# debbiemarkslab/BEAR

Measured on AMD Instinct MI355X. Metric: k-mer contexts/sec (DM-marginal+grad h), k=13, higher is better.
Workload: dtype f64

## Files before the change

### bear_amd/csrc/bear_common.h

```cpp
#pragma once
#include <hip/hip_runtime.h>
#include <math.h>
#include <stdint.h>
#include <string.h>

#include "../../include/bear_hip.h"
#include "bear_release_guard.h"
#include "bear_math.h"

#define BEAR_THREADS 256
#define BEAR_TILE_ROWS 1024
#define BEAR_ROWS_PER_THREAD (BEAR_TILE_ROWS / BEAR_THREADS)
#define BEAR_MAX_OUT 4

extern __attribute__((visibility("hidden"))) thread_local int g_last_hip_error;

#define HIP_TRY(expr)                      \
  do {                                     \
    hipError_t _e = (expr);                \
    if (_e != hipSuccess) {                \
      g_last_hip_error = (int)_e;          \
      return BEAR_ERR_HIP;                 \
    }                                      \
  } while (0)

struct bear_params;
struct bear_ws {
  int device;
  int num_cu;
  int max_blocks;
  double *partials;
  double *logtab;
  unsigned long long *dbg;
  double *eval_partials;
  double *eval_out;
  int eval_blocks;
  double *lin_partials;
  double *lin_accum;
  unsigned long long *arrive;
  unsigned epoch;
  double *cnn_partials;
  size_t cnn_partials_cap;
};

struct bear_params {
  double inv_h;
  double eps;
  double E;
  double tauE;
  double tau;
  double V;
  double nw;
};

__device__ __forceinline__ void bear_store_agent(double *p, double v) {
  __hip_atomic_store(p, v, __ATOMIC_RELAXED, __HIP_MEMORY_SCOPE_AGENT);
}

__device__ __forceinline__ void bear_wave_store_rows5(double *R, const double (&f)[5], double *__restrict__ dst, uint64_t i0,
                                                      uint32_t valid, uint32_t lane) {
#pragma unroll
  for (int b = 0; b < 5; ++b) R[lane * 5u + b] = f[b];
  __builtin_amdgcn_fence(__ATOMIC_RELEASE, "wavefront");
  __builtin_amdgcn_wave_barrier();
  const uint32_t n16 = (valid * 5u) >> 1;
  typedef double bear_v2d __attribute__((ext_vector_type(2)));
  bear_v2d *out = reinterpret_cast<bear_v2d *>(dst + i0 * 5u);
  const bear_v2d *src = reinterpret_cast<const bear_v2d *>(R);
  for (uint32_t k = lane; k < n16; k += 64u) __builtin_nontemporal_store(src[k], out + k);
  if ((valid & 1u) && lane == 0) dst[(i0 + valid) * 5u - 1u] = R[valid * 5u - 1u];
  __builtin_amdgcn_fence(__ATOMIC_ACQUIRE, "wavefront");
  __builtin_amdgcn_wave_barrier();
}

__device__ __forceinline__ void bear_wave_load_rows5(double *R, const double *__restrict__ src, uint64_t i0, uint32_t valid,
                                                     uint32_t lane, double (&f)[5]) {
  typedef double bear_v2d __attribute__((ext_vector_type(2)));
  const uint32_t n16 = (valid * 5u) >> 1;
  const bear_v2d *in = reinterpret_cast<const bear_v2d *>(src + i0 * 5u);
  bear_v2d *dst = reinterpret_cast<bear_v2d *>(R);
  for (uint32_t k = lane; k < n16; k += 64u) dst[k] = __builtin_nontemporal_load(in + k);
  if ((valid & 1u) && lane == 0) R[valid * 5u - 1u] = src[(i0 + valid) * 5u - 1u];
  __builtin_amdgcn_fence(__ATOMIC_RELEASE, "wavefront");
  __builtin_amdgcn_wave_barrier();
  const uint32_t row = lane < valid ? lane : valid - 1u;
#pragma unroll
  for (int b = 0; b < 5; ++b) f[b] = R[row * 5u + b];
  __builtin_amdgcn_fence(__ATOMIC_ACQUIRE, "wavefront");
  __builtin_amdgcn_wave_barrier();
}

template <int NOUT, bool AGENT = false>
__device__ __forceinline__ void block_store_partials(double (&acc)[NOUT], double *partials) {
  __shared__ double red[16][BEAR_MAX_OUT];
  const int lane = threadIdx.x & 63, wave = threadIdx.x >> 6;
#pragma unroll
  for (int k = 0; k < NOUT; ++k) {
    double v = bear_wave_sum(acc[k]);
    if (lane == 0) red[wave][k] = v;
  }
  __syncthreads();
  if (threadIdx.x < NOUT) {
    double s = 0.0;
#pragma unroll
    for (int w = 0; w < (int)(blockDim.x >> 6); ++w) s += red[w][threadIdx.x];
    if (AGENT) bear_store_agent(&partials[(size_t)blockIdx.x * BEAR_MAX_OUT + threadIdx.x], s);
    else partials[(size_t)blockIdx.x * BEAR_MAX_OUT + threadIdx.x] = s;
  }
}

#define BEAR_THETA_NET 1
#define BEAR_THETA_REF 2
struct bear_arrival {
  unsigned long long *word;
  unsigned epoch;
};
struct bear_step_io {
  const double *theta;
  int kind;
  unsigned epoch;
  double *out;
  unsigned long long *arrive_word;
  __host__ __device__ bear_arrival arrive() const { return bear_arrival{arrive_word, epoch}; }
};
static_assert(sizeof(bear_step_io) == 32, "bear_step_io: kernel-argument size");

__device__ __forceinline__ double bear_uniform_f64(double v) {
  const unsigned long long b = (unsigned long long)__double_as_longlong(v);
  const unsigned lo = (unsigned)__builtin_amdgcn_readfirstlane((int)(unsigned)b);
  const unsigned hi = (unsigned)__builtin_amdgcn_readfirstlane((int)(unsigned)(b >> 32));
  return __longlong_as_double((long long)(((unsigned long long)hi << 32) | lo));
}

__device__ __forceinline__ bear_params bear_params_of(const bear_params &arg, const bear_step_io &io) {
  if (!io.theta) return arg;
  bear_params p;
  p.eps = arg.eps;
  p.inv_h = bear_uniform_f64(1.0 / exp(io.theta[0]));
  p.E = p.tauE = p.tau = p.V = p.nw = 0.0;
  if (io.kind == BEAR_THETA_REF) {
    const double tau = exp(io.theta[1]), nw = exp(io.theta[2]);
    const double E = exp(-tau);
    p.E = bear_uniform_f64(E);
    p.tauE = bear_uniform_f64(tau * E);
    p.tau = bear_uniform_f64(tau);
    p.V = bear_uniform_f64(1.0 / (nw + 1.0));
    p.nw = bear_uniform_f64(nw);
  }
  return p;
}

#define BEAR_ARRIVE_SUBS 16
#define BEAR_ARRIVE_STRIDE 16
#define BEAR_ARRIVE_WORDS ((BEAR_ARRIVE_SUBS + 1) * BEAR_ARRIVE_STRIDE)
__device__ __forceinline__ bool bear_arrive_count(unsigned long long *word, unsigned long long tag, unsigned expected) {
  __hip_atomic_fetch_max(word, tag, __ATOMIC_RELAXED, __HIP_MEMORY_SCOPE_AGENT);
  return __hip_atomic_fetch_add(word, 1ull, __ATOMIC_RELAXED, __HIP_MEMORY_SCOPE_AGENT) == tag + (expected - 1u);
}
__device__ __forceinline__ bool bear_arrive_last(const bear_arrival &arrive) {
  __shared__ unsigned s_last;
  asm volatile("s_waitcnt vmcnt(0)" ::: "memory");
  __syncthreads();
  if (threadIdx.x == 0) {
    const unsigned long long tag = (unsigned long long)arrive.epoch << 24;
    const unsigned sub = blockIdx.x % BEAR_ARRIVE_SUBS, grid = gridDim.x;
    const unsigned in_sub = (grid - sub + BEAR_ARRIVE_SUBS - 1u) / BEAR_ARRIVE_SUBS;
    const unsigned subs = grid < BEAR_ARRIVE_SUBS ? grid : BEAR_ARRIVE_SUBS;
    bool last = bear_arrive_count(arrive.word + (1u + sub) * BEAR_ARRIVE_STRIDE, tag, in_sub);
    if (last) last = bear_arrive_count(arrive.word, tag, subs);
    s_last = last ? 1u : 0u;
  }
  __syncthreads();
  if (!s_last) return false;
  __builtin_amdgcn_fence(__ATOMIC_ACQUIRE, "agent");
  return true;
}

__device__ __forceinline__ void bear_arrive_reset(const bear_arrival &arrive) {
#pragma unroll
  for (int k = 0; k <= BEAR_ARRIVE_SUBS; ++k)
    __hip_atomic_store(arrive.word + k * BEAR_ARRIVE_STRIDE, 0ull, __ATOMIC_RELAXED, __HIP_MEMORY_SCOPE_AGENT);
}

__device__ __forceinline__ void bear_finalize_in_block(const double *partials, int n_out, double *out, const bear_arrival &arrive, bool accumulate = false) {
  __shared__ double fred[4][BEAR_MAX_OUT];
  const int n_blocks = (int)gridDim.x;
  if (threadIdx.x < 256) {
    double acc[BEAR_MAX_OUT] = {0.0, 0.0, 0.0, 0.0};
    for (int b = threadIdx.x; b < n_blocks; b += 256)
#pragma unroll
      for (int k = 0; k < BEAR_MAX_OUT; ++k)
        if (k < n_out) acc[k] += partials[(size_t)b * BEAR_MAX_OUT + k];
    const int lane = threadIdx.x & 63, wave = threadIdx.x >> 6;
#pragma unroll
    for (int k = 0; k < BEAR_MAX_OUT; ++k) {
      double v = bear_wave_sum(acc[k]);
      if (lane == 0) fred[wave][k] = v;
    }
  }
  __syncthreads();
  if ((int)threadIdx.x < n_out) {
    const double v = (fred[0][threadIdx.x] + fred[1][threadIdx.x]) + (fred[2][threadIdx.x] + fred[3][threadIdx.x]);
    out[threadIdx.x] = accumulate ? out[threadIdx.x] + v : v;
  }
  if (threadIdx.x == 0) bear_arrive_reset(arrive);
}

struct bear_apply_io {
  double *theta;
  double *m, *v;
  double *t_state;
  double *loss_buf;
  unsigned long long loss_cap;
  double lr, scale;
  int n_theta, train_ar;
};

__device__ __forceinline__ void bear_adam_update(const bear_apply_io &A, const double *packed, int tid, int n_threads) {
  const double t0 = A.t_state[0], t = t0 + 1.0;
  const double b1 = 0.9, b2 = 0.999, aeps = 1e-7;
  const double lr_t = A.lr * sqrt(1.0 - pow(b2, t)) / (1.0 - pow(b1, t));
  for (int k = tid; k < A.n_theta; k += n_threads) {
    if (A.train_ar && k == 0) continue;
    const double g = A.scale * packed[1 + k];
    const double mk = b1 * A.m[k] + (1.0 - b1) * g, vk = b2 * A.v[k] + (1.0 - b2) * g * g;
    A.m[k] = mk;
    A.v[k] = vk;
    A.theta[k] -= lr_t * mk / (sqrt(vk) + aeps);
  }
  if (tid == 0) {
    const unsigned long long step = (unsigned long long)t0;
    if (A.loss_buf && step < A.loss_cap) A.loss_buf[step] = -A.scale * packed[0];
  }
  __syncthreads();
  if (tid == 0) A.t_state[0] = t;
}

__device__ __forceinline__ void bear_apply_in_block(const bear_apply_io &A, const double *packed) {
  if (!A.theta) return;
  __threadfence_block();
  __syncthreads();
  bear_adam_update(A, packed, (int)threadIdx.x, (int)blockDim.x);
}

template <int NOUT>
__device__ __forceinline__ void block_finish(double (&acc)[NOUT], double *partials, const bear_step_io &io) {
  if (!io.out) {
    block_store_partials<NOUT>(acc, partials);
    return;
  }
  block_store_partials<NOUT, true>(acc, partials);
  if (bear_arrive_last(io.arrive())) bear_finalize_in_block(partials, NOUT, io.out, io.arrive());
}
template <int NOUT>
__device__ __forceinline__ void block_finish(double (&acc)[NOUT], double *partials, const bear_step_io &io, const bear_apply_io &apply) {
  if (!io.out) {
    block_store_partials<NOUT>(acc, partials);
    return;
  }
  block_store_partials<NOUT, true>(acc, partials);
  if (bear_arrive_last(io.arrive())) {
    bear_finalize_in_block(partials, NOUT, io.out, io.arrive());
    bear_apply_in_block(apply, io.out);
  }
}
```

### bear_amd/csrc/bear_hip.hip

```cpp
#include "bear_host.h"
#include "kernels_finalize.h"
#include "kernels_rows.h"
#include "kernels_sorted.h"
#include "kernels_plan.h"
#include "kernels_synth.h"
#include "kernels_refmix.h"
#include "kernels_mixplan.h"
#include "kernels_sample.h"
#include "kernels_shuffle.h"
#include "kernels_refplan.h"

#ifdef PLN_STAMPS
#define PLN_DBG_ARG , ws->dbg
#else
#define PLN_DBG_ARG
#endif

thread_local int g_last_hip_error = 0;

extern "C" {

int bear_abi_version(void) { return BEAR_ABI_VERSION; }

const char *bear_strerror(int status) {
  switch (status) {
    case BEAR_OK: return "ok";
    case BEAR_ERR_INVALID_ARG: return "invalid argument (null or misaligned pointer, bad flag)";
    case BEAR_ERR_NO_DEVICE: return "no usable HIP device";
    case BEAR_ERR_WRONG_DEVICE: return "current HIP device differs from the workspace device";
    case BEAR_ERR_HIP: return "HIP runtime call failed (see bear_last_hip_error)";
    case BEAR_ERR_NOMEM: return "out of memory";
    case BEAR_ERR_IO: return "file could not be opened or read";
    case BEAR_ERR_PARSE: return "malformed count-table row";
    default: return "unknown bear status";
  }
}

int bear_last_hip_error(void) { return g_last_hip_error; }

static int dm_kernels_setup() {
  int st = allow_dynamic_lds({BEAR_KFN(dm_prior_sorted_kernel<0>), BEAR_KFN(dm_prior_sorted_kernel<1>), BEAR_KFN(dm_prior_sorted_kernel<9>)},
                             sizeof(srt_lds_n));
  if (st == BEAR_OK) st = allow_dynamic_lds({BEAR_KFN(dm_ref_sorted_kernel)}, sizeof(srt_lds_r));
  if (st == BEAR_OK)
    st = allow_dynamic_lds({BEAR_KFN(dm_prior_plan_kernel<false, false>), BEAR_KFN(dm_prior_plan_kernel<true, false>),
                            BEAR_KFN(dm_prior_plan_kernel<true, true>)},
                           sizeof(pln_lds_n));
  if (st == BEAR_OK)
    st = allow_dynamic_lds({BEAR_KFN(dm_prior_plan_grad_kernel<false, false>), BEAR_KFN(dm_prior_plan_grad_kernel<true, true>),
                            BEAR_KFN(dm_refmix_plan_grad_kernel<false>), BEAR_KFN(dm_refmix_plan_grad_kernel<true>)},
                           sizeof(pln_lds_g));
  if (st == BEAR_OK) st = allow_dynamic_lds({BEAR_KFN(dm_prior_plan_grad_inplace_kernel)}, sizeof(pln_lds_gi));
  if (st == BEAR_OK) st = allow_dynamic_lds({BEAR_KFN(dm_ref_plan_kernel<false>), BEAR_KFN(dm_ref_plan_kernel<true>)}, sizeof(pln_lds_r));
  return st;
}

static void ws_release(bear_ws *ws) {
  (void)hipFree(ws->partials);
  (void)hipFree(ws->logtab);
  (void)hipFree(ws->dbg);
  (void)hipFree(ws->eval_partials);
  (void)hipFree(ws->eval_out);
  (void)hipFree(ws->lin_partials);
  (void)hipFree(ws->lin_accum);
  (void)hipFree(ws->cnn_partials);
  (void)hipFree(ws->arrive);
  delete ws;
}

static int ws_setup(bear_ws *ws) {
  HIP_TRY(hipMalloc(&ws->partials, sizeof(double) * BEAR_MAX_OUT * (size_t)ws->max_blocks));
  HIP_TRY(hipMalloc(&ws->logtab, sizeof(double) * 2 * BEAR_LOGTAB_N));
  HIP_TRY(hipMalloc(&ws->dbg, sizeof(unsigned long long) * 48 * (size_t)ws->max_blocks));
  HIP_TRY(hipMalloc(&ws->arrive, sizeof(unsigned long long) * BEAR_ARRIVE_WORDS));
  HIP_TRY(hipMemset(ws->arrive, 0, sizeof(unsigned long long) * BEAR_ARRIVE_WORDS));
  double tab[2 * BEAR_LOGTAB_N];
  for (int i = 0; i < BEAR_LOGTAB_N; ++i) {
    const double r = 1.0 / ((BEAR_LOGTAB_N + i + 0.5) / (2.0 * BEAR_LOGTAB_N));
    tab[2 * i] = r;
    tab[2 * i + 1] = -log(r);
  }
  HIP_TRY(hipMemcpy(ws->logtab, tab, sizeof(tab), hipMemcpyHostToDevice));
  int st = dm_kernels_setup();
  if (st == BEAR_OK) st = linear_ws_setup(ws);
  if (st == BEAR_OK) st = cnn_ws_setup(ws);
  if (st == BEAR_OK) st = eval_ws_setup(ws);
  return st;
}

int bear_ws_create(int device, bear_ws **out) {
  if (!out) return BEAR_ERR_INVALID_ARG;
  *out = nullptr;
  int count = 0;
  if (hipGetDeviceCount(&count) != hipSuccess || count <= 0) return BEAR_ERR_NO_DEVICE;
  if (device < 0 || device >= count) return BEAR_ERR_INVALID_ARG;
  int prev = 0;
  HIP_TRY(hipGetDevice(&prev));
  HIP_TRY(hipSetDevice(device));
  hipDeviceProp_t prop;
  const hipError_t e = hipGetDeviceProperties(&prop, device);
  bear_ws *ws = e == hipSuccess ? new (std::nothrow) bear_ws() : nullptr;
  int st = ws ? BEAR_OK : BEAR_ERR_NOMEM;
  if (e != hipSuccess) {
    g_last_hip_error = (int)e;
    st = BEAR_ERR_HIP;
  }
  if (ws) {
    ws->device = device;
    ws->num_cu = prop.multiProcessorCount;
    ws->max_blocks = ws->num_cu * 8;
    ws->eval_blocks = ws->num_cu * 8;
    st = ws_setup(ws);
    if (st != BEAR_OK) {
      ws_release(ws);
      ws = nullptr;
    }
  }
  (void)hipSetDevice(prev);
  *out = ws;
  return st;
}

int bear_ws_destroy(bear_ws *ws) {
  if (!ws) return BEAR_OK;
  int prev = 0;
  (void)hipGetDevice(&prev);
  (void)hipSetDevice(ws->device);
  ws_release(ws);
  (void)hipSetDevice(prev);
  return BEAR_OK;
}

int bear_deterministic_build(void) {
#ifdef BEAR_DET_BUILD
  return 1;
#else
  return 0;
#endif
}

static int grid_rows(const bear_ws *ws, uint64_t n_rows) { return grid_capped((n_rows + BEAR_TILE_ROWS - 1) / BEAR_TILE_ROWS, ws_blocks(ws, 2)); }
static int grid_sorted(const bear_ws *ws, uint64_t n_rows) { return grid_capped((n_rows + SRT_TILE - 1) / SRT_TILE, ws_blocks(ws, 2)); }
static int grid_dense(const bear_ws *ws, uint64_t n_rows) {
  return grid_capped((n_rows + DPR_TILE_ROWS - 1) / DPR_TILE_ROWS, ws_blocks(ws, DPR_BLOCKS_PER_CU));
}

int bear_dm_prior_f64(bear_ws *ws, const uint32_t *counts, const double *prior, uint64_t n_rows,
                      double h_signed, double eps, int train_ar, double *out, double *grad_prior,
                      void *stream) {
  int st = check_ws(ws);
  if (st != BEAR_OK) return st;
  if (!out || (n_rows && (!counts || !prior))) return BEAR_ERR_INVALID_ARG;
  if (misaligned(counts) || misaligned(prior) || misaligned(grad_prior) || (reinterpret_cast<uintptr_t>(out) & 7u))
    return BEAR_ERR_INVALID_ARG;
  hipStream_t s = static_cast<hipStream_t>(stream);
  bear_params prm;
  memset(&prm, 0, sizeof(prm));
  prm.inv_h = 1.0 / exp(h_signed);
  prm.eps = eps;
  int grid = grid_rows(ws, n_rows);
  if (!train_ar && !grad_prior) {
    grid = grid_sorted(ws, n_rows);
    const char *dbg = getenv("BEAR_DEBUG_STOP");
    const int stop = dbg ? atoi(dbg) : 0;
    const double2 *lt = reinterpret_cast<const double2 *>(ws->logtab);
    if (stop == 1)
      hipLaunchKernelGGL(dm_prior_sorted_kernel<1>, dim3(grid), dim3(SRT_THREADS), sizeof(srt_lds_n), s, counts, prior, n_rows, prm, lt, ws->partials, ws->dbg);
    else if (stop == 9)
      hipLaunchKernelGGL(dm_prior_sorted_kernel<9>, dim3(grid), dim3(SRT_THREADS), sizeof(srt_lds_n), s, counts, prior, n_rows, prm, lt, ws->partials, ws->dbg);
    else
      hipLaunchKernelGGL(dm_prior_sorted_kernel<0>, dim3(grid), dim3(SRT_THREADS), sizeof(srt_lds_n), s, counts, prior, n_rows, prm, lt, ws->partials, ws->dbg);
  } else {
#define PRIOR_LAUNCH(AR, GRAD)                                                                                                          \
  hipLaunchKernelGGL((dm_prior_kernel<AR, GRAD>), dim3(grid), dim3(BEAR_THREADS), 0, s, counts, prior, n_rows, prm, grad_prior, \
                     reinterpret_cast<const double2 *>(ws->logtab), ws->partials)
    BEAR_DISPATCH_2(train_ar, grad_prior, PRIOR_LAUNCH);
#undef PRIOR_LAUNCH
  }
  HIP_TRY(hipGetLastError());
  hipLaunchKernelGGL(finalize_kernel, dim3(1), dim3(256), 0, s, ws->partials, grid, 2, out);
  HIP_TRY(hipGetLastError());
  return BEAR_OK;
}

int bear_dm_ref_f64(bear_ws *ws, const uint32_t *train, const uint32_t *ref, uint64_t n_rows,
                    double h_signed, double tau_signed, double nu_signed, double eps, int train_ar,
                    double *out, void *stream) {
  int st = check_ws(ws);
  if (st != BEAR_OK) return st;
  if (!out || (n_rows && (!train || !ref))) return BEAR_ERR_INVALID_ARG;
  if (misaligned(train) || misaligned(ref) || (reinterpret_cast<uintptr_t>(out) & 7u)) return BEAR_ERR_INVALID_ARG;
  hipStream_t s = static_cast<hipStream_t>(stream);
  bear_params prm;
  const double tau = exp(tau_signed), nw = exp(nu_signed);
  prm.inv_h = 1.0 / exp(h_signed);
  prm.eps = eps;
  prm.E = exp(-tau);
  prm.tauE = tau * prm.E;
  prm.tau = tau;
  prm.V = 1.0 / (nw + 1.0);
  prm.nw = nw;
  int grid = grid_rows(ws, n_rows);
  if (train_ar) {
    hipLaunchKernelGGL((dm_ref_kernel<true>), dim3(grid), dim3(BEAR_THREADS), 0, s, train, ref, n_rows, prm, reinterpret_cast<const double2 *>(ws->logtab), ws->partials);
  } else if (getenv("BEAR_ROWS_KERNEL")) {
    hipLaunchKernelGGL((dm_ref_kernel<false>), dim3(grid), dim3(BEAR_THREADS), 0, s, train, ref, n_rows, prm, reinterpret_cast<const double2 *>(ws->logtab), ws->partials);
  } else {
    grid = grid_sorted(ws, n_rows);
    hipLaunchKernelGGL(dm_ref_sorted_kernel, dim3(grid), dim3(SRT_THREADS), sizeof(srt_lds_r), s, train, ref, n_rows, prm,
                       reinterpret_cast<const double2 *>(ws->logtab), ws->partials);
  }
  HIP_TRY(hipGetLastError());
  hipLaunchKernelGGL(finalize_kernel, dim3(1), dim3(256), 0, s, ws->partials, grid, 4, out);
  HIP_TRY(hipGetLastError());
  return BEAR_OK;
}

static void plan_free(bear_plan *p) {
  if (!p) return;
  (void)hipFree(p->tiles);
  (void)hipFree(p->stream);
  (void)hipFree(p->heavy_col);
  (void)hipFree(p->heavy_row);
  (void)hipFree(p->heavy_stop);
  (void)hipFree(p->hist);
  (void)hipFree(p->live);
  for (int k = 0; k < p->n_cnn_levels; ++k) bear_level_free(&p->cnn_levels[k]);
  for (int k = 0; k <= CNN_MAX_LAG; ++k)
    for (int q = 0; q < p->n_cnn_win[k]; ++q) bear_window_free(&p->cnn_win[k][q]);
  (void)hipFree(p->live2);
  (void)hipFree(p->tiles_p);
  (void)hipFree(p->tiles_u);
  (void)hipFree(p->ref_items);
  (void)hipFree(p->hist0_base);
  (void)hipFree(p->heavy0);
  (void)hipFree(p->sum0);
  delete p;
}

int bear_plan_create(bear_ws *ws, const uint32_t *counts, uint64_t n_rows, int ncol, bear_plan **out) {
  if (!out) return BEAR_ERR_INVALID_ARG;
  *out = nullptr;
  int st = check_ws(ws);
  if (st != BEAR_OK) return st;
  if ((ncol != 4 && ncol != 5) || (n_rows && !counts) || misaligned(counts)) return BEAR_ERR_INVALID_ARG;
  bear_plan *p = new (std::nothrow) bear_plan();
  if (!p) return BEAR_ERR_NOMEM;
  memset(p, 0, sizeof(*p));
  p->device = ws->device;
  p->ncol = ncol;
  p->n_rows = n_rows;
  p->counts = counts;
  hipError_t e = hipMalloc(&p->hist, sizeof(unsigned long long) * (2 * SRT_NKEY + PLN_NBIG + 1));
  if (e == hipSuccess) e = hipMemset(p->hist, 0, sizeof(unsigned long long) * (2 * SRT_NKEY + PLN_NBIG + 1));
  if (e != hipSuccess) {
    g_last_hip_error = (int)e;
    plan_free(p);
    return BEAR_ERR_HIP;
  }
  if (n_rows == 0) {
    *out = p;
    return BEAR_OK;
  }
  const uint64_t n_quads = (n_rows + PLN_QUAD - 1) / PLN_QUAD;
  uint8_t *d_quad = nullptr, *h_quad = nullptr;
  unsigned long long *d_cnt = nullptr;
  std::vector<pln_tile> tiles;
  e = hipMalloc(&d_quad, 3 * n_quads);
  if (e == hipSuccess) e = hipMalloc(&d_cnt, sizeof(unsigned long long) * 9);
  if (e == hipSuccess) e = hipMemset(d_cnt, 0, sizeof(unsigned long long) * 9);
  if (e == hipSuccess) {
    const int grid = grid_capped((n_quads + 255) / 256, (uint64_t)ws->num_cu * 8);
    hipLaunchKernelGGL(plan_scan_kernel, dim3(grid), dim3(256), 0, 0, counts, n_rows, ncol, d_quad, d_cnt, p->hist);
    e = hipGetLastError();
  }
  unsigned long long h_cnt[3] = {0, 0, 0}, h_total[3] = {0, 0, 0};
  if (e == hipSuccess) e = hipMemcpy(h_cnt, d_cnt, sizeof(h_cnt), hipMemcpyDeviceToHost);
  if (e == hipSuccess) e = hipMemcpy(h_total, d_cnt + 6, sizeof(h_total), hipMemcpyDeviceToHost);
  for (int k = 0; k < 3; ++k) p->count_total[k] = p->count_bound[k] = (double)h_total[k];
  uint64_t off16 = 0, n_tiles = 0;
  const char *cut_env = getenv("BEAR_PLAN_CUT");
  const bool host_cut = cut_env && cut_env[0] == 'h';
  if (e == hipSuccess && host_cut) {
    h_quad = (uint8_t *)malloc(3 * n_quads);
    if (!h_quad) e = hipErrorOutOfMemory;
    if (e == hipSuccess) e = hipMemcpy(h_quad, d_quad, 3 * n_quads, hipMemcpyDeviceToHost);
  }
  if (e == hipSuccess && host_cut) {
    uint64_t q = 0;
    while (q < n_quads) {
      uint32_t items = 0, rows = 0, hcol = 0, hrow = 0;
      const uint64_t q0 = q;
      while (q < n_quads && rows + PLN_QUAD <= PLN_RMAX && items + h_quad[q] <= PLN_NI_CUT) {
        items += h_quad[q];
        hcol += h_quad[n_quads + q];
        hrow += h_quad[2 * n_quads + q];
        rows += PLN_QUAD;
        ++q;
      }
      pln_tile ti;
      memset(&ti, 0, sizeof(ti));
      ti.row0 = q0 * PLN_QUAD;
      if (ti.row0 + rows > n_rows) rows = (uint32_t)(n_rows - ti.row0);
      const uint32_t hc = hcol < PLN_HCAP ? hcol : PLN_HCAP;
      const uint32_t hr = ncol == 5 ? (hrow < PLN_HCAP ? hrow : PLN_HCAP) : 0u;
      ti.rows_items = (rows << 16) | items;
      ti.off16 = (uint32_t)off16;
      ti.hc_hr = (hc << 16) | hr;
      ti.blk16 = pln_block_layout(rows, items, hc, hr).end / 16;
      off16 += ti.blk16;
      if (off16 > 0xffffffffull) {
        e = hipErrorOutOfMemory;
        break;
      }
      tiles.push_back(ti);
    }
    n_tiles = tiles.size();
  }
  free(h_quad);
  if (e == hipSuccess && !host_cut) {
    const uint32_t chunk = plan_cut_chunk(n_quads);
    const uint64_t n_chunks = (n_quads + chunk - 1) / chunk;
    uint32_t *d_walk = nullptr;
    uint16_t *d_step = nullptr;
    uint64_t *d_entry = nullptr;
    unsigned long long *d_meta = nullptr, h_meta[3] = {0, 0, 0};
    e = hipMalloc(&d_walk, sizeof(uint32_t) * n_chunks * PLN_CUT_SPAN);
    if (e == hipSuccess) e = hipMalloc(&d_step, sizeof(uint16_t) * n_quads);
    if (e == hipSuccess) e = hipMalloc(&d_entry, sizeof(uint64_t) * 2 * n_chunks);
    if (e == hipSuccess) e = hipMalloc(&d_meta, sizeof(h_meta));
    if (e == hipSuccess) e = hipMemset(d_meta, 0, sizeof(h_meta));
    if (e == hipSuccess) {
      const uint64_t wb = (n_chunks * PLN_CUT_SPAN + 255) / 256;
      hipLaunchKernelGGL(plan_cut_step_kernel, dim3((unsigned)((n_chunks + 255) / 256)), dim3(256), 0, 0, d_quad, n_quads, n_chunks, chunk, d_step);
      hipLaunchKernelGGL(plan_cut_walk_kernel, dim3((unsigned)wb), dim3(256), 0, 0, d_step, n_quads, n_chunks, chunk, d_walk);
      hipLaunchKernelGGL(plan_cut_chain_kernel, dim3(1), dim3(1), 0, 0, d_walk, n_chunks, chunk, d_entry, d_entry + n_chunks, d_meta);
      e = hipGetLastError();
    }
    if (e == hipSuccess) e = hipMemcpy(h_meta, d_meta, sizeof(unsigned long long), hipMemcpyDeviceToHost);
    n_tiles = h_meta[0];
    if (e == hipSuccess) e = hipMalloc(&p->tiles, sizeof(pln_tile) * (n_tiles + PLN_DESC_PAD));
    if (e == hipSuccess) e = hipMemset(p->tiles, 0, sizeof(pln_tile) * (n_tiles + PLN_DESC_PAD));
    if (e == hipSuccess) {
      hipLaunchKernelGGL(plan_cut_write_kernel, dim3((unsigned)((n_chunks + 255) / 256)), dim3(256), 0, 0, d_quad, n_quads, n_rows, ncol,
                         n_chunks, chunk, d_entry, d_entry + n_chunks, p->tiles);
      hipLaunchKernelGGL(plan_cut_offsets_kernel, dim3(1), dim3(1024), 0, 0, p->tiles, n_tiles, d_meta);
      e = hipGetLastError();
    }
    if (e == hipSuccess) e = hipMemcpy(h_meta, d_meta, sizeof(h_meta), hipMemcpyDeviceToHost);
    if (e == hipSuccess && h_meta[2]) e = hipErrorOutOfMemory;
    off16 = h_meta[1];
    (void)hipFree(d_walk);
    (void)hipFree(d_step);
    (void)hipFree(d_entry);
    (void)hipFree(d_meta);
  }
  (void)hipFree(d_quad);
  p->n_tiles = n_tiles;
  const uint64_t stream_bytes = off16 * 16 + 1024;
  for (int k = 0; k < 3; ++k) p->n_heavy[k] = h_cnt[k];
  if (host_cut) {
    if (e == hipSuccess) e = hipMalloc(&p->tiles, sizeof(pln_tile) * (tiles.size() + PLN_DESC_PAD));
    if (e == hipSuccess) e = hipMemset(p->tiles, 0, sizeof(pln_tile) * (tiles.size() + PLN_DESC_PAD));
    if (e == hipSuccess) e = hipMemcpy(p->tiles, tiles.data(), sizeof(pln_tile) * tiles.size(), hipMemcpyHostToDevice);
  }
  if (e == hipSuccess) e = hipMalloc(&p->stream, stream_bytes);
  if (e == hipSuccess) e = hipMemset(p->stream, 0, stream_bytes);
  if (e == hipSuccess && h_cnt[0]) e = hipMalloc(&p->heavy_col, sizeof(pln_heavy_col) * h_cnt[0]);
  if (e == hipSuccess && h_cnt[1]) e = hipMalloc(&p->heavy_row, sizeof(pln_heavy_row) * h_cnt[1]);
  if (e == hipSuccess && h_cnt[2]) e = hipMalloc(&p->heavy_stop, sizeof(uint64_t) * h_cnt[2]);
  if (e == hipSuccess) {
    const uint64_t nt = n_tiles;
    const int grid = grid_capped(nt, (uint64_t)ws->num_cu * 2);
    hipLaunchKernelGGL(plan_fill_kernel, dim3(grid), dim3(1024), 0, 0, counts, n_rows, ncol, p->tiles, nt, p->stream,
                       p->heavy_col, p->heavy_row, p->heavy_stop, d_cnt + 3);
    e = hipGetLastError();
  }
  const uint64_t live_bytes = ncol == 5 ? sizeof(uint16_t) * PLN_LIVE_STRIDE * (n_tiles + 1) : 0;
  if (e == hipSuccess && live_bytes) e = hipMalloc(&p->live, live_bytes);
  if (e == hipSuccess && live_bytes) e = hipMemset(p->live, 0, live_bytes);
  if (e == hipSuccess && live_bytes) {
    const uint64_t nt = n_tiles;
    const int grid = grid_capped(nt, (uint64_t)ws->num_cu * 2);
    hipLaunchKernelGGL(plan_live_kernel, dim3(grid), dim3(1024), 0, 0, p->tiles, nt, p->stream, p->live);
    e = hipGetLastError();
  }
  if (e == hipSuccess) e = hipDeviceSynchronize();
  unsigned long long h_used[3] = {0, 0, 0};
  if (e == hipSuccess) e = hipMemcpy(h_used, d_cnt + 3, sizeof(h_used), hipMemcpyDeviceToHost);
  for (int k = 0; k < 3; ++k) p->n_heavy[k] = h_used[k];
#ifdef BEAR_DET_BUILD
  const uint64_t sort_from = 2;
#else
  const uint64_t sort_from = 1u << 16;
#endif
  if (e == hipSuccess) {
    int cst = h_used[0] >= sort_from ? bear_canonical_order(p->heavy_col, h_used[0], 16, 0) : BEAR_OK;
    if (cst == BEAR_OK && h_used[1] >= sort_from) cst = bear_canonical_order(p->heavy_row, h_used[1], 16, 0);
    if (cst == BEAR_OK && h_used[2] >= sort_from) cst = bear_canonical_order(p->heavy_stop, h_used[2], 8, 0);
    if (cst != BEAR_OK) e = cst == BEAR_ERR_NOMEM ? hipErrorOutOfMemory : hipErrorUnknown;
  }
  p->n_live_rows = n_rows;
  if (e == hipSuccess && ncol == 5) {
    unsigned long long h_hist[SRT_NKEY];
    e = hipMemcpy(h_hist, p->hist, sizeof(h_hist), hipMemcpyDeviceToHost);
    unsigned long long live_rows = h_cnt[1];
    for (int k = 0; k < SRT_NKEY; ++k) live_rows += h_hist[k];
    p->n_live_rows = live_rows;
  }
  (void)hipFree(d_cnt);
  if (e != hipSuccess) {
    g_last_hip_error = (int)e;
    plan_free(p);
    return e == hipErrorOutOfMemory ? BEAR_ERR_NOMEM : BEAR_ERR_HIP;
  }
  p->bytes = stream_bytes + live_bytes + sizeof(pln_tile) * n_tiles + sizeof(pln_heavy_col) * h_cnt[0] +
             sizeof(pln_heavy_row) * h_cnt[1] + sizeof(uint64_t) * h_cnt[2];
  *out = p;
  return BEAR_OK;
}

int bear_plan_destroy(bear_plan *plan) {
  if (!plan) return BEAR_OK;
  int prev = 0;
  (void)hipGetDevice(&prev);
  (void)hipSetDevice(plan->device);
  plan_free(plan);
  (void)hipSetDevice(prev);
  return BEAR_OK;
}

uint64_t bear_plan_bytes(const bear_plan *plan) { return plan ? plan->bytes : 0; }

#define PLAN_ROWS 15
static bool plan_is_rows(const bear_plan *p) { return p->ncol == PLAN_ROWS; }
int bear_plan_create_auto(bear_ws *ws, const uint32_t *counts, uint64_t n_rows, int *rowwise, bear_plan **out) {
  if (rowwise) *rowwise = 0;
  int st = bear_plan_create(ws, counts, n_rows, 5, out);
  if (st != BEAR_OK) return st;
  bear_plan *p = *out;
  const double cells = p->count_total[1], listed = (double)p->n_heavy[0];
  if (!(cells > 0.0) || listed * 2.0 <= cells) return BEAR_OK;
  (void)hipFree(p->tiles);
  (void)hipFree(p->stream);
  (void)hipFree(p->heavy_col);
  (void)hipFree(p->heavy_row);
  (void)hipFree(p->heavy_stop);
  (void)hipFree(p->live);
  p->tiles = nullptr;
  p->stream = nullptr;
  p->heavy_col = nullptr;
  p->heavy_row = nullptr;
  p->heavy_stop = nullptr;
  p->live = nullptr;
  p->n_tiles = 0;
  p->n_heavy[0] = p->n_heavy[1] = p->n_heavy[2] = 0;
  p->ncol = PLAN_ROWS;
  p->bytes = sizeof(unsigned long long) * (2 * SRT_NKEY + PLN_NBIG + 1);
  if (rowwise) *rowwise = 1;
  return BEAR_OK;
}
static int launch_prior_rows(bear_ws *ws, const bear_plan *plan, const double *prior, const bear_params &prm, const double *theta,
                             int train_ar, double *out, double *grad_prior, hipStream_t s) {
  const int grid = grid_dense(ws, plan->n_rows);
  const double2 *lt = reinterpret_cast<const double2 *>(ws->logtab);
  const bear_step_io io = ws_io(ws, theta, BEAR_THETA_NET, out);
#define ROWS_LAUNCH(AR, GRAD) \
  hipLaunchKernelGGL((dm_prior_rows_kernel<AR, GRAD>), dim3(grid), dim3(BEAR_THREADS), 0, s, plan->counts, prior, plan->n_rows, prm, grad_prior, lt, \
                     ws->partials, io)
  BEAR_DISPATCH_2(train_ar, grad_prior, ROWS_LAUNCH);
#undef ROWS_LAUNCH
  HIP_TRY(hipGetLastError());
  return BEAR_OK;
}

uint64_t bear_plan_tile_count(const bear_plan *plan) { return plan ? plan->n_tiles : 0; }

int bear_plan_tile_info(const bear_plan *plan, uint64_t first, uint64_t count, uint64_t *row0, uint32_t *rows, uint32_t *items,
                        uint64_t *stream_offset) {
  if (!plan || first + count > plan->n_tiles || (count && (!row0 || !rows || !items || !stream_offset))) return BEAR_ERR_INVALID_ARG;
  if (!count) return BEAR_OK;
  std::vector<pln_tile> h(count);
  int prev = 0;
  (void)hipGetDevice(&prev);
  (void)hipSetDevice(plan->device);
  const hipError_t e = hipMemcpy(h.data(), plan->tiles + first, sizeof(pln_tile) * count, hipMemcpyDeviceToHost);
  (void)hipSetDevice(prev);
  if (e != hipSuccess) {
    g_last_hip_error = (int)e;
    return BEAR_ERR_HIP;
  }
  for (uint64_t k = 0; k < count; ++k) {
    row0[k] = h[k].row0;
    rows[k] = h[k].rows_items >> 16;
    items[k] = h[k].rows_items & 0xffffu;
    stream_offset[k] = (uint64_t)h[k].off16 * 16;
  }
  return BEAR_OK;
}

int bear_plan_create_ref(bear_ws *ws, const uint32_t *train, const uint32_t *ref, uint64_t n_rows, bear_plan **out) {
  if (!out) return BEAR_ERR_INVALID_ARG;
  *out = nullptr;
  if ((n_rows && !ref) || misaligned(ref)) return BEAR_ERR_INVALID_ARG;
  bear_plan *p = nullptr;
  int st = bear_plan_create(ws, train, n_rows, 4, &p);
  if (st != BEAR_OK) return st;
  p->ref = ref;
  if (p->count_total[1] > 0.0 && (double)p->n_heavy[0] * 2.0 > p->count_total[1]) {
    (void)hipFree(p->tiles);
    (void)hipFree(p->stream);
    (void)hipFree(p->heavy_col);
    (void)hipFree(p->heavy_row);
    (void)hipFree(p->heavy_stop);
    p->tiles = nullptr;
    p->stream = nullptr;
    p->heavy_col = nullptr;
    p->heavy_row = nullptr;
    p->heavy_stop = nullptr;
    p->n_tiles = 0;
    p->n_heavy[0] = p->n_heavy[1] = p->n_heavy[2] = 0;
    p->rows_ref = 1;
    p->bytes = sizeof(unsigned long long) * (2 * SRT_NKEY + PLN_NBIG + 1);
    *out = p;
    return BEAR_OK;
  }
  unsigned long long *d_meta = nullptr;
  hipError_t e = hipMalloc(&d_meta, sizeof(unsigned long long) * 72);
  if (e == hipSuccess) e = hipMemset(d_meta, 0, sizeof(unsigned long long) * 72);
  if (e == hipSuccess) e = hipMalloc(&p->sum0, sizeof(double));
  if (e == hipSuccess) e = hipMemset(p->sum0, 0, sizeof(double));
  p->hist0_base = d_meta;
  unsigned long long h_meta[72];
  memset(h_meta, 0, sizeof(h_meta));
  const int grid = grid_capped((n_rows + 1023) / 1024, (uint64_t)ws->num_cu * 8);
  if (e == hipSuccess && n_rows) {
    hipLaunchKernelGGL(rpl_build_kernel, dim3(grid), dim3(256), 0, 0, train, ref, n_rows, 0, d_meta, d_meta + 32, d_meta + 64, p->sum0,
                       static_cast<rpl_item *>(nullptr), static_cast<uint32_t *>(nullptr));
    e = hipGetLastError();
    if (e == hipSuccess) e = hipMemcpy(h_meta, d_meta, sizeof(h_meta), hipMemcpyDeviceToHost);
  }
  if (e == hipSuccess) {
    unsigned long long run = 0, cur[RPL_NKEY];
    for (int k = 0; k < RPL_NKEY; ++k) {
      cur[k] = run;
      run += h_meta[k];
    }
    p->n_ref_items = run;
    p->n_heavy0 = h_meta[64];
    if (run) e = hipMalloc(&p->ref_items, sizeof(rpl_item) * run);
    if (e == hipSuccess && p->n_heavy0) e = hipMalloc(&p->heavy0, sizeof(uint32_t) * p->n_heavy0);
    if (e == hipSuccess) e = hipMemcpy(d_meta, cur, sizeof(cur), hipMemcpyHostToDevice);
    if (e == hipSuccess) e = hipMemset(d_meta + 64, 0, sizeof(unsigned long long));
    if (e == hipSuccess && n_rows && (run || p->n_heavy0)) {
      hipLaunchKernelGGL(rpl_build_kernel, dim3(grid), dim3(256), 0, 0, train, ref, n_rows, 1, d_meta, d_meta + 32, d_meta + 64, p->sum0,
                         p->ref_items, p->heavy0);
      e = hipGetLastError();
    }
    if (e == hipSuccess) e = hipDeviceSynchronize();
#ifdef BEAR_DET_BUILD
    for (int k = 0; k < RPL_NKEY && e == hipSuccess; ++k)
      if (bear_canonical_order(p->ref_items + cur[k], h_meta[k], 16, 0) != BEAR_OK) e = hipErrorUnknown;
    if (e == hipSuccess && bear_canonical_order(p->heavy0, p->n_heavy0, 4, 0) != BEAR_OK) e = hipErrorUnknown;
#endif
  }
  if (e != hipSuccess) {
    g_last_hip_error = (int)e;
    plan_free(p);
    return e == hipErrorOutOfMemory ? BEAR_ERR_NOMEM : BEAR_ERR_HIP;
  }
  p->hist0 = d_meta + 32;
  p->bytes += sizeof(rpl_item) * p->n_ref_items + sizeof(uint32_t) * p->n_heavy0 + sizeof(unsigned long long) * 72;
  *out = p;
  return BEAR_OK;
}

static int launch_prior_plan(bear_ws *ws, const bear_plan *plan, const double *prior, uint64_t n_rows, const bear_params &prm,
                             const double *theta, int train_ar, int prior_normalized, double *out, hipStream_t s) {
  const int grid = grid_plan(ws, plan->n_tiles);
  const double2 *lt = reinterpret_cast<const double2 *>(ws->logtab);
  const bear_step_io io = ws_io(ws, theta, BEAR_THETA_NET, out);
  if (train_ar)
    hipLaunchKernelGGL((dm_prior_plan_kernel<true, true>), dim3(grid), dim3(PLN_THREADS), sizeof(pln_lds_n), s, prior, n_rows, prm,
                       plan_view(plan), lt, ws->partials, io PLN_DBG_ARG);
  else if (prior_normalized)
    hipLaunchKernelGGL((dm_prior_plan_kernel<true, false>), dim3(grid), dim3(PLN_THREADS), sizeof(pln_lds_n), s, prior, n_rows, prm,
                       plan_view(plan), lt, ws->partials, io PLN_DBG_ARG);
  else
    hipLaunchKernelGGL((dm_prior_plan_kernel<false, false>), dim3(grid), dim3(PLN_THREADS), sizeof(pln_lds_n), s, prior, n_rows, prm,
                       plan_view(plan), lt, ws->partials, io PLN_DBG_ARG);
  HIP_TRY(hipGetLastError());
  return BEAR_OK;
}

int bear_dm_prior_plan_f64(bear_ws *ws, const bear_plan *plan, const uint32_t *counts, const double *prior,
                           uint64_t n_rows, double h_signed, double eps, int train_ar, int prior_normalized,
                           double *out, void *stream) {
  int st = check_ws(ws);
  if (st != BEAR_OK) return st;
  if (!plan || !out || (n_rows && (!counts || !prior))) return BEAR_ERR_INVALID_ARG;
  if ((plan->ncol != 5 && !plan_is_rows(plan)) || plan->n_rows != n_rows || plan->counts != counts || plan->device != ws->device)
    return BEAR_ERR_INVALID_ARG;
  if (misaligned(prior) || (reinterpret_cast<uintptr_t>(out) & 7u)) return BEAR_ERR_INVALID_ARG;
  bear_params prm;
  memset(&prm, 0, sizeof(prm));
  prm.inv_h = 1.0 / exp(h_signed);
  prm.eps = eps;
  if (plan_is_rows(plan)) return launch_prior_rows(ws, plan, prior, prm, nullptr, train_ar, out, nullptr, static_cast<hipStream_t>(stream));
  return launch_prior_plan(ws, plan, prior, n_rows, prm, nullptr, train_ar, prior_normalized, out, static_cast<hipStream_t>(stream));
}

int launch_prior_plan_grad(bear_ws *ws, const bear_plan *plan, const double *prior, const bear_params &prm,
                                  const double *theta, int train_ar, int prior_normalized, double *out, double *grad_prior,
                                  hipStream_t s) {
  const int grid = grid_plan(ws, plan->n_tiles);
  const double2 *lt = reinterpret_cast<const double2 *>(ws->logtab);
  const pln_view pv = plan_view(plan);
  const bear_step_io io = ws_io(ws, theta, BEAR_THETA_NET, out);
  if (train_ar)
    hipLaunchKernelGGL((dm_prior_plan_grad_kernel<true, true>), dim3(grid), dim3(PLN_THREADS), sizeof(pln_lds_g), s, prior, prm, pv, lt,
                       grad_prior, ws->partials, io);
  else if (prior_normalized)
    hipLaunchKernelGGL(dm_prior_plan_grad_inplace_kernel, dim3(grid), dim3(PLN_THREADS), sizeof(pln_lds_gi), s, prior, prm, pv, lt,
                       grad_prior, ws->partials, io);
  else
    hipLaunchKernelGGL((dm_prior_plan_grad_kernel<false, false>), dim3(grid), dim3(PLN_THREADS), sizeof(pln_lds_g), s, prior, prm, pv, lt,
                       grad_prior, ws->partials, io);
  HIP_TRY(hipGetLastError());
  auto fixup_grid = [&](uint64_t nh) { return grid_capped((nh + 255) / 256, (uint64_t)ws->num_cu * 8); };
#define FIXUP(NORM, AR, ROWS, N) \
  hipLaunchKernelGGL((dm_prior_grad_fixup_kernel<NORM, AR, ROWS>), dim3(fixup_grid(N)), dim3(256), 0, s, prior, prm, pv, lt, grad_prior, io)
  if (pv.n_heavy_row && !train_ar) {
    if (prior_normalized) FIXUP(true, false, true, pv.n_heavy_row);
    else FIXUP(false, false, true, pv.n_heavy_row);
  }
  if (pv.n_heavy_col) {
    if (train_ar) FIXUP(true, true, false, pv.n_heavy_col);
    else if (prior_normalized) FIXUP(true, false, false, pv.n_heavy_col);
    else FIXUP(false, false, false, pv.n_heavy_col);
  }
#undef FIXUP
  HIP_TRY(hipGetLastError());
  return BEAR_OK;
}

int bear_dm_prior_plan_grad_f64(bear_ws *ws, const bear_plan *plan, const uint32_t *counts, const double *prior,
                                uint64_t n_rows, double h_signed, double eps, int train_ar, int prior_normalized,
                                double *out, double *grad_prior, void *stream) {
  int st = check_ws(ws);
  if (st != BEAR_OK) return st;
  if (!plan || !out || !grad_prior || (n_rows && (!counts || !prior))) return BEAR_ERR_INVALID_ARG;
  if ((plan->ncol != 5 && !plan_is_rows(plan)) || plan->n_rows != n_rows || plan->counts != counts || plan->device != ws->device)
    return BEAR_ERR_INVALID_ARG;
  if (misaligned(prior) || misaligned(grad_prior) || (reinterpret_cast<uintptr_t>(out) & 7u)) return BEAR_ERR_INVALID_ARG;
  bear_params prm;
  memset(&prm, 0, sizeof(prm));
  prm.inv_h = 1.0 / exp(h_signed);
  prm.eps = eps;
  if (plan_is_rows(plan)) return launch_prior_rows(ws, plan, prior, prm, nullptr, train_ar, out, grad_prior, static_cast<hipStream_t>(stream));
  return launch_prior_plan_grad(ws, plan, prior, prm, nullptr, train_ar, prior_normalized, out, grad_prior,
                                static_cast<hipStream_t>(stream));
}

int bear_dm_prior_plan_dev_f64(bear_ws *ws, const bear_plan *plan, const uint32_t *counts, const double *prior, uint64_t n_rows,
                               const double *h_signed_dev, double eps, int train_ar, int prior_normalized, double *out,
                               double *grad_prior, void *stream) {
  int st = check_ws(ws);
  if (st != BEAR_OK) return st;
  if (!plan || !out || !h_signed_dev || (n_rows && (!counts || !prior))) return BEAR_ERR_INVALID_ARG;
  if ((plan->ncol != 5 && !plan_is_rows(plan)) || plan->n_rows != n_rows || plan->counts != counts || plan->device != ws->device)
    return BEAR_ERR_INVALID_ARG;
  if (misaligned(prior) || misaligned(grad_prior) || (reinterpret_cast<uintptr_t>(out) & 7u)) return BEAR_ERR_INVALID_ARG;
  hipStream_t s = static_cast<hipStream_t>(stream);
  bear_params only_eps;
  memset(&only_eps, 0, sizeof(only_eps));
  only_eps.eps = eps;
  if (plan_is_rows(plan)) return launch_prior_rows(ws, plan, prior, only_eps, h_signed_dev, train_ar, out, grad_prior, s);
  if (grad_prior) return launch_prior_plan_grad(ws, plan, prior, only_eps, h_signed_dev, train_ar, prior_normalized, out, grad_prior, s);
  return launch_prior_plan(ws, plan, prior, n_rows, only_eps, h_signed_dev, train_ar, prior_normalized, out, s);
}

int bear_dm_refmix_plan_grad_f64(bear_ws *ws, const bear_plan *plan, const uint32_t *counts, const double *net_rows,
                                 const double *ref_rows, uint64_t n_rows, const double *h_signed_dev, const double *tau_signed_dev,
                                 const double *net_weight_signed_dev, double eps, int train_ar, double *out, double *grad_net_rows,
                                 void *stream) {
  int st = check_ws(ws);
  if (st != BEAR_OK) return st;
  if (!plan || !out || !h_signed_dev || !tau_signed_dev || !net_weight_signed_dev) return BEAR_ERR_INVALID_ARG;
  if (n_rows && (!counts || !net_rows || !ref_rows || !grad_net_rows)) return BEAR_ERR_INVALID_ARG;
  if (plan->ncol != 5 || plan->n_rows != n_rows || plan->counts != counts || plan->device != ws->device) return BEAR_ERR_INVALID_ARG;
  if (misaligned(net_rows) || misaligned(ref_rows) || misaligned(grad_net_rows) || misaligned8(out) || misaligned8(h_signed_dev) ||
      misaligned8(tau_signed_dev) || misaligned8(net_weight_signed_dev) || !(eps >= 0.0))
    return BEAR_ERR_INVALID_ARG;
  hipStream_t s = static_cast<hipStream_t>(stream);
  const int grid = grid_plan(ws, plan->n_tiles);
  const double2 *lt = reinterpret_cast<const double2 *>(ws->logtab);
  const pln_view pv = plan_view(plan);
  const bear_step_io io = ws_io(ws, nullptr, BEAR_THETA_REF, out);
  if (train_ar)
    hipLaunchKernelGGL(dm_refmix_plan_grad_kernel<true>, dim3(grid), dim3(PLN_THREADS), sizeof(pln_lds_g), s, net_rows, ref_rows,
                       h_signed_dev, tau_signed_dev, net_weight_signed_dev, eps, pv, lt, grad_net_rows, ws->partials, io);
  else
    hipLaunchKernelGGL(dm_refmix_plan_grad_kernel<false>, dim3(grid), dim3(PLN_THREADS), sizeof(pln_lds_g), s, net_rows, ref_rows,
                       h_signed_dev, tau_signed_dev, net_weight_signed_dev, eps, pv, lt, grad_net_rows, ws->partials, io);
  HIP_TRY(hipGetLastError());
  if (pv.n_heavy_col + pv.n_heavy_row) {
    const uint64_t nh = pv.n_heavy_col + pv.n_heavy_row;
    const int g2 = grid_capped((nh + 255) / 256, (uint64_t)ws->num_cu * 4);
    if (train_ar)
      hipLaunchKernelGGL(dm_refmix_fixup_kernel<true>, dim3(g2), dim3(256), 0, s, net_rows, ref_rows, h_signed_dev, tau_signed_dev,
                         net_weight_signed_dev, eps, pv, lt, grad_net_rows);
    else
      hipLaunchKernelGGL(dm_refmix_fixup_kernel<false>, dim3(g2), dim3(256), 0, s, net_rows, ref_rows, h_signed_dev, tau_signed_dev,
                         net_weight_signed_dev, eps, pv, lt, grad_net_rows);
    HIP_TRY(hipGetLastError());
  }
  return BEAR_OK;
}


static int launch_ref_plan(bear_ws *ws, const bear_plan *plan, const uint32_t *ref, uint64_t n_rows, const bear_params &prm,
                           const double *theta, int train_ar, double *out, hipStream_t s, const bear_apply_io &apply = NO_APPLY) {
  const double2 *lt = reinterpret_cast<const double2 *>(ws->logtab);
  const bear_step_io io = ws_io(ws, theta, BEAR_THETA_REF, out);
  int grid;
  if (plan->rows_ref) {
    if (plan->ref != ref) return BEAR_ERR_INVALID_ARG;
    grid = grid_dense(ws, n_rows);
    if (train_ar)
      hipLaunchKernelGGL(dm_ref_rows_kernel<true>, dim3(grid), dim3(BEAR_THREADS), 0, s, plan->counts, ref, n_rows, prm, lt, ws->partials, io, apply);
    else
      hipLaunchKernelGGL(dm_ref_rows_kernel<false>, dim3(grid), dim3(BEAR_THREADS), 0, s, plan->counts, ref, n_rows, prm, lt, ws->partials, io, apply);
  } else if (plan->ref) {
    if (plan->ref != ref) return BEAR_ERR_INVALID_ARG;
    rpl_view rv;
    rv.items = plan->ref_items;
    rv.n_items = plan->n_ref_items;
    rv.hist0 = plan->hist0;
    rv.heavy0 = plan->heavy0;
    rv.n_heavy0 = plan->n_heavy0;
    rv.sum0 = plan->sum0;
    const uint64_t units = (plan->n_ref_items + 63) / 64, want = (units + 3) / 4 + 2, cap = (uint64_t)ws->num_cu * (units > 131072 ? 6 : 4);
    grid = grid_capped(want, cap);
    if (train_ar)
      hipLaunchKernelGGL(dm_ref_items_kernel<true>, dim3(grid), dim3(256), 0, s, prm, rv, plan_view(plan), lt, ws->partials, io, apply);
    else
      hipLaunchKernelGGL(dm_ref_items_kernel<false>, dim3(grid), dim3(256), 0, s, prm, rv, plan_view(plan), lt, ws->partials, io, apply);
  } else {
    grid = grid_plan(ws, plan->n_tiles);
    if (train_ar)
      hipLaunchKernelGGL(dm_ref_plan_kernel<true>, dim3(grid), dim3(PLN_THREADS), sizeof(pln_lds_r), s, ref, n_rows, prm, plan_view(plan), lt,
                         ws->partials, io, apply);
    else
      hipLaunchKernelGGL(dm_ref_plan_kernel<false>, dim3(grid), dim3(PLN_THREADS), sizeof(pln_lds_r), s, ref, n_rows, prm, plan_view(plan), lt,
                         ws->partials, io, apply);
  }
  HIP_TRY(hipGetLastError());
  (void)grid;
  return BEAR_OK;
}

int bear_dm_ref_plan_f64(bear_ws *ws, const bear_plan *plan, const uint32_t *train, const uint32_t *ref,
                         uint64_t n_rows, double h_signed, double tau_signed, double nu_signed, double eps,
                         int train_ar, double *out, void *stream) {
  int st = check_ws(ws);
  if (st != BEAR_OK) return st;
  if (!plan || !out || (n_rows && (!train || !ref))) return BEAR_ERR_INVALID_ARG;
  if (plan->ncol != 4 || plan->n_rows != n_rows || plan->counts != train || plan->device != ws->device)
    return BEAR_ERR_INVALID_ARG;
  if (misaligned(ref) || (reinterpret_cast<uintptr_t>(out) & 7u)) return BEAR_ERR_INVALID_ARG;
  hipStream_t s = static_cast<hipStream_t>(stream);
  bear_params prm;
  const double tau = exp(tau_signed), nw = exp(nu_signed);
  prm.inv_h = 1.0 / exp(h_signed);
  prm.eps = eps;
  prm.E = exp(-tau);
  prm.tauE = tau * prm.E;
  prm.tau = tau;
  prm.V = 1.0 / (nw + 1.0);
  prm.nw = nw;
  return launch_ref_plan(ws, plan, ref, n_rows, prm, nullptr, train_ar, out, s);
}

int bear_ref_train_reduce_f64(bear_ws *ws, const bear_plan *plan, const uint32_t *train, const uint32_t *ref, uint64_t n_rows,
                              const double *theta, double eps, int train_ar, double *packed, void *stream) {
  int st = check_ws(ws);
  if (st != BEAR_OK) return st;
  if (!plan || !packed || !theta || !n_rows || !train || !ref) return BEAR_ERR_INVALID_ARG;
  if (plan->ncol != 4 || plan->n_rows != n_rows || plan->counts != train || plan->device != ws->device)
    return BEAR_ERR_INVALID_ARG;
  if (misaligned(ref) || (reinterpret_cast<uintptr_t>(packed) & 7u)) return BEAR_ERR_INVALID_ARG;
  hipStream_t s = static_cast<hipStream_t>(stream);
  bear_params only_eps;
  memset(&only_eps, 0, sizeof(only_eps));
  only_eps.eps = eps;
  return launch_ref_plan(ws, plan, ref, n_rows, only_eps, theta, train_ar, packed, s);
}

int bear_ref_train_step_f64(bear_ws *ws, const bear_plan *plan, const uint32_t *train, const uint32_t *ref, uint64_t n_rows,
                            double *theta, double *adam_m, double *adam_v, double *adam_t, double eps, int train_ar,
                            double learning_rate, double scale, double *out, double *loss_buf, uint64_t loss_cap, void *stream) {
  if (!adam_m || !adam_v || !adam_t) return BEAR_ERR_INVALID_ARG;
  if (two_launch_step()) {
    int st = bear_ref_train_reduce_f64(ws, plan, train, ref, n_rows, theta, eps, train_ar, out, stream);
    if (st != BEAR_OK) return st;
    return launch_train_apply(theta, 3, out, adam_m, adam_v, adam_t, learning_rate, scale, train_ar, loss_buf, loss_cap,
                              static_cast<hipStream_t>(stream));
  }
  int st = check_ws(ws);
  if (st != BEAR_OK) return st;
  if (!plan || !out || !theta || !n_rows || !train || !ref) return BEAR_ERR_INVALID_ARG;
  if (plan->ncol != 4 || plan->n_rows != n_rows || plan->counts != train || plan->device != ws->device) return BEAR_ERR_INVALID_ARG;
  if (misaligned(ref) || (reinterpret_cast<uintptr_t>(out) & 7u)) return BEAR_ERR_INVALID_ARG;
  bear_params only_eps;
  memset(&only_eps, 0, sizeof(only_eps));
  only_eps.eps = eps;
  return launch_ref_plan(ws, plan, ref, n_rows, only_eps, theta, train_ar, out, static_cast<hipStream_t>(stream),
                         make_apply(theta, 3, adam_m, adam_v, adam_t, learning_rate, scale, train_ar, loss_buf, loss_cap));
}

int bear_dm_items_f64(bear_ws *ws, const double *x, const uint32_t *c, uint64_t n, int path, double *D, double *P,
                      void *stream) {
  int st = check_ws(ws);
  if (st != BEAR_OK) return st;
  if (n == 0) return BEAR_OK;
  if (!x || !c || !D || !P || path < 0 || path > 2) return BEAR_ERR_INVALID_ARG;
  uint64_t blocks = (n + 255) / 256;
  if (blocks > 0x7fffffffull) return BEAR_ERR_INVALID_ARG;
  hipLaunchKernelGGL(dm_items_kernel, dim3((unsigned)blocks), dim3(256), 0, static_cast<hipStream_t>(stream), x, c, n, path,
                     reinterpret_cast<const double2 *>(ws->logtab), D, P);
  HIP_TRY(hipGetLastError());
  return BEAR_OK;
}

int bear_plan_count_total(const bear_plan *plan, double *total, double *bound) {
  if (!plan) return BEAR_ERR_INVALID_ARG;
  for (int k = 0; k < 3; ++k) {
    if (total) total[k] = plan->count_total[k];
    if (bound) bound[k] = plan->count_bound[k];
  }
  return BEAR_OK;
}

int bear_plan_set_count_bound(bear_plan *plan, const double *bound) {
  if (!plan || !bound) return BEAR_ERR_INVALID_ARG;
  for (int k = 0; k < 3; ++k)
    if (!(bound[k] >= plan->count_total[k]) || !(bound[k] < 0x1p50)) return BEAR_ERR_INVALID_ARG;
  for (int k = 0; k < 3; ++k) plan->count_bound[k] = bound[k];
  return BEAR_OK;
}

static int refmix_grid(const bear_ws *ws, uint64_t n_rows) { return grid_capped((n_rows + RMX_THREADS - 1) / RMX_THREADS, ws_blocks(ws, 2)); }

int bear_ref_mix_forward_f64(bear_ws *ws, const double *net_rows, const double *ref_rows, uint64_t n_rows, const double *tau_signed,
                             const double *net_weight_signed, double *prior, void *stream) {
  int st = check_ws(ws);
  if (st != BEAR_OK) return st;
  if (!tau_signed || !net_weight_signed || misaligned8(tau_signed) || misaligned8(net_weight_signed)) return BEAR_ERR_INVALID_ARG;
  if (n_rows == 0) return BEAR_OK;
  if (!net_rows || !ref_rows || !prior || misaligned(net_rows) || misaligned(ref_rows) || misaligned(prior)) return BEAR_ERR_INVALID_ARG;
  hipLaunchKernelGGL(ref_mix_forward_kernel, dim3(refmix_grid(ws, n_rows)), dim3(RMX_THREADS), 0, static_cast<hipStream_t>(stream),
                     net_rows, ref_rows, tau_signed, net_weight_signed, n_rows, prior);
  HIP_TRY(hipGetLastError());
  return BEAR_OK;
}

int bear_ref_mix_backward_f64(bear_ws *ws, const double *net_rows, const double *ref_rows, const double *grad_prior, uint64_t n_rows,
                              const double *tau_signed, const double *net_weight_signed, double *grad_net_rows, double *grad_scalars,
                              void *stream) {
  int st = check_ws(ws);
  if (st != BEAR_OK) return st;
  if (!tau_signed || !net_weight_signed || !grad_scalars || misaligned8(tau_signed) || misaligned8(net_weight_signed) ||
      misaligned8(grad_scalars))
    return BEAR_ERR_INVALID_ARG;
  hipStream_t s = static_cast<hipStream_t>(stream);
  if (n_rows == 0) {
    HIP_TRY(hipMemsetAsync(grad_scalars, 0, 2 * sizeof(double), s));
    return BEAR_OK;
  }
  if (!net_rows || !ref_rows || !grad_prior || !grad_net_rows || misaligned(net_rows) || misaligned(ref_rows) ||
      misaligned(grad_prior) || misaligned(grad_net_rows))
    return BEAR_ERR_INVALID_ARG;
  hipLaunchKernelGGL(ref_mix_backward_kernel, dim3(refmix_grid(ws, n_rows)), dim3(RMX_THREADS), 0, s, net_rows, ref_rows, grad_prior,
                     tau_signed, net_weight_signed, n_rows, grad_net_rows, ws->partials, ws_arrival(ws), grad_scalars);
  HIP_TRY(hipGetLastError());
  return BEAR_OK;
}

int bear_debug_read_timing(bear_ws *ws, unsigned long long *host, int n_words) {
  if (!ws || !host) return BEAR_ERR_INVALID_ARG;
  HIP_TRY(hipDeviceSynchronize());
  HIP_TRY(hipMemcpy(host, ws->dbg, sizeof(unsigned long long) * (size_t)n_words, hipMemcpyDeviceToHost));
  return BEAR_OK;
}

int bear_debug_occupancy(int which) {
  int nb = -1;
  hipError_t e = which == 0
      ? hipOccupancyMaxActiveBlocksPerMultiprocessor(&nb, dm_prior_sorted_kernel<0>, SRT_THREADS, sizeof(srt_lds_n))
      : hipOccupancyMaxActiveBlocksPerMultiprocessor(&nb, dm_ref_sorted_kernel, SRT_THREADS, sizeof(srt_lds_r));
  return e == hipSuccess ? nb : -1000 - (int)e;
}

int bear_log_gamma_f64(const double *conc, uint64_t n, uint64_t n_samples, uint64_t seed, double *out, void *stream) {
  if (n == 0 || n_samples == 0) return BEAR_OK;
  if (!conc || !out) return BEAR_ERR_INVALID_ARG;
  if (n_samples > (~0ull) / n) return BEAR_ERR_INVALID_ARG;
  const uint64_t total = n * n_samples;
  uint64_t blocks = (total + SMP_THREADS - 1) / SMP_THREADS;
  if (blocks > 65536) blocks = 65536;
  hipLaunchKernelGGL(log_gamma_kernel, dim3((unsigned)blocks), dim3(SMP_THREADS), 0, static_cast<hipStream_t>(stream), conc, n,
                     n_samples, seed, out);
  HIP_TRY(hipGetLastError());
  return BEAR_OK;
}

static int logdir_sample_launch(const uint32_t *counts, const double *prior, uint64_t n_rows, int width, const double *h,
                                int n_h, int with_ar, const double *van, int n_van, int mc_samples, int map, uint64_t seed,
                                uint64_t row_base, double *out, void *stream) {
  if (n_h < 0 || n_van < 0 || n_h + n_van > SMP_MAX_MODELS || (n_h && !h) || (n_van && !van)) return BEAR_ERR_INVALID_ARG;
  if (with_ar && !map) return BEAR_ERR_INVALID_ARG;
  if (map) mc_samples = 1;
  if (mc_samples <= 0) return BEAR_ERR_INVALID_ARG;
  const int M = (with_ar ? 1 : 0) + n_h + n_van;
  if (n_rows == 0 || M == 0) return BEAR_OK;
  if (!out || ((n_h || with_ar) && !prior)) return BEAR_ERR_INVALID_ARG;
  smp_args A;
  memset(&A, 0, sizeof(A));
  A.n_h = n_h;
  A.n_van = n_van;
  A.arm = with_ar ? 1 : 0;
  A.has_counts = counts ? 1 : 0;
  A.has_prior = prior ? 1 : 0;
  A.map = map ? 1 : 0;
  A.mc = (uint32_t)mc_samples;
  A.seed = seed;
  A.row_base = row_base;
  for (int j = 0; j < n_h; ++j) {
    if (!(h[j] > 0.0)) return BEAR_ERR_INVALID_ARG;
    A.w[j] = 1.0 / h[j];
  }
  for (int k = 0; k < n_van; ++k) A.w[n_h + k] = van[k];
  const uint64_t per_row = (uint64_t)M * (uint64_t)mc_samples;
  if (per_row > 0xffffffffull || n_rows > (~0ull) / ((uint64_t)width * per_row)) return BEAR_ERR_INVALID_ARG;
  uint64_t blocks = (n_rows * per_row + SMP_THREADS - 1) / SMP_THREADS;
  if (blocks > 65536) blocks = 65536;
  hipStream_t s = static_cast<hipStream_t>(stream);
  if (width == 21)
    hipLaunchKernelGGL(logdir_sample_kernel<21>, dim3((unsigned)blocks), dim3(SMP_THREADS), 0, s, counts, prior, n_rows, A, out);
  else
    hipLaunchKernelGGL(logdir_sample_kernel<5>, dim3((unsigned)blocks), dim3(SMP_THREADS), 0, s, counts, prior, n_rows, A, out);
  HIP_TRY(hipGetLastError());
  return BEAR_OK;
}

int bear_logdir_sample_f64(const uint32_t *counts, const double *prior, uint64_t n_rows, const double *h, int n_h,
                           int with_ar, const double *van, int n_van, int mc_samples, int map, uint64_t seed,
                           uint64_t row_base, double *out, void *stream) {
  return logdir_sample_launch(counts, prior, n_rows, 5, h, n_h, with_ar, van, n_van, mc_samples, map, seed, row_base, out, stream);
}

int bear_logdir_sample_wide_f64(const uint32_t *counts, const double *prior, uint64_t n_rows, int width, const double *h,
                                int n_h, int with_ar, const double *van, int n_van, int mc_samples, int map, uint64_t seed,
                                uint64_t row_base, double *out, void *stream) {
  if (!wide_width_ok(width)) return BEAR_ERR_INVALID_ARG;
  return logdir_sample_launch(counts, prior, n_rows, width, h, n_h, with_ar, van, n_van, mc_samples, map, seed, row_base, out,
                              stream);
}

int bear_shuffle_rows(const void *src, void *dst, uint64_t n_rows, uint32_t row_bytes, uint64_t seed, void *stream) {
  if (n_rows == 0 || row_bytes == 0) return BEAR_OK;
  if (!src || !dst || src == dst) return BEAR_ERR_INVALID_ARG;
  if (n_rows > (1ull << 62) / row_bytes) return BEAR_ERR_INVALID_ARG;
  const uint32_t hb = shf_half_bits(n_rows);
  const bool words = (row_bytes % 4 == 0) && ((reinterpret_cast<uintptr_t>(src) | reinterpret_cast<uintptr_t>(dst)) % 4 == 0);
  const uint64_t total = words ? n_rows * (row_bytes / 4) : n_rows * (uint64_t)row_bytes;
  uint64_t blocks = (total + 255) / 256;
  if (blocks > 1u << 20) blocks = 1u << 20;
  if (words)
    hipLaunchKernelGGL(shuffle_words_kernel, dim3((unsigned)blocks), dim3(256), 0, static_cast<hipStream_t>(stream),
                       static_cast<const uint32_t *>(src), static_cast<uint32_t *>(dst), n_rows, row_bytes / 4, hb, seed);
  else
    hipLaunchKernelGGL(shuffle_bytes_kernel, dim3((unsigned)blocks), dim3(256), 0, static_cast<hipStream_t>(stream),
                       static_cast<const uint8_t *>(src), static_cast<uint8_t *>(dst), n_rows, row_bytes, hb, seed);
  HIP_TRY(hipGetLastError());
  return BEAR_OK;
}

uint64_t bear_shuffle_source_row(uint64_t i, uint64_t n_rows, uint64_t seed) {
  return (n_rows == 0 || i >= n_rows) ? i : shf_perm(i, n_rows, shf_half_bits(n_rows), seed);
}

int bear_stream_read(bear_ws *ws, const void *src, uint64_t n_bytes, void *stream) {
  int st = check_ws(ws);
  if (st != BEAR_OK) return st;
  if (!src || misaligned(src)) return BEAR_ERR_INVALID_ARG;
  hipLaunchKernelGGL(stream_read_kernel, dim3(ws->num_cu * 16), dim3(256), 0, static_cast<hipStream_t>(stream),
                     static_cast<const uint4 *>(src), n_bytes / 16, reinterpret_cast<uint32_t *>(ws->dbg));
  HIP_TRY(hipGetLastError());
  return BEAR_OK;
}

int bear_synth_counts_u32(uint64_t seed, uint64_t row0, uint64_t n_rows, int dense, uint32_t *train,
                          uint32_t *test, uint32_t *ref, void *stream) {
  if (n_rows == 0) return BEAR_OK;
  if (!train && !test && !ref) return BEAR_ERR_INVALID_ARG;
  uint64_t blocks = (n_rows + 255) / 256;
  if (blocks > 0x7fffffffull) return BEAR_ERR_INVALID_ARG;
  hipLaunchKernelGGL(synth_counts_kernel, dim3((unsigned)blocks), dim3(256), 0, static_cast<hipStream_t>(stream), seed, row0, n_rows, dense, train, test, ref);
  HIP_TRY(hipGetLastError());
  return BEAR_OK;
}

int bear_synth_prior_f64(uint64_t seed, uint64_t row0, uint64_t n_rows, double *prior, void *stream) {
  if (n_rows == 0) return BEAR_OK;
  if (!prior) return BEAR_ERR_INVALID_ARG;
  uint64_t blocks = (n_rows + 255) / 256;
  if (blocks > 0x7fffffffull) return BEAR_ERR_INVALID_ARG;
  hipLaunchKernelGGL(synth_prior_kernel, dim3((unsigned)blocks), dim3(256), 0, static_cast<hipStream_t>(stream), seed, row0, n_rows, prior);
  HIP_TRY(hipGetLastError());
  return BEAR_OK;
}

}
```

### bear_amd/csrc/kernels_plan.h

```cpp
#pragma once
#include "plan_common.h"

__global__ __launch_bounds__(256) void plan_scan_kernel(const uint32_t *__restrict__ counts, uint64_t n_rows, int ncol,
                                                        uint8_t *__restrict__ quad_light,
                                                        unsigned long long *__restrict__ heavy_counts,
                                                        unsigned long long *__restrict__ hist) {
  __shared__ uint32_t s_heavy[3];
  __shared__ uint32_t s_hist[2 * SRT_NKEY];
  __shared__ uint32_t s_big[PLN_NBIG + 1];
  __shared__ unsigned long long s_total, s_cells;
  __shared__ uint32_t s_cmax;
  unsigned long long my_total = 0ull;
  uint32_t my_cells = 0u, my_cmax = 0u;
  if (threadIdx.x == 0) {
    s_total = s_cells = 0ull;
    s_cmax = 0u;
  }
  if (threadIdx.x < 3) s_heavy[threadIdx.x] = 0;
  if (threadIdx.x < 2 * SRT_NKEY) s_hist[threadIdx.x] = 0;
  for (uint32_t k = threadIdx.x; k <= PLN_NBIG; k += 256) s_big[k] = 0;
  __syncthreads();
  const uint64_t n_quads = (n_rows + PLN_QUAD - 1) / PLN_QUAD;
  for (uint64_t g = (uint64_t)blockIdx.x * 256 + threadIdx.x; g < n_quads; g += (uint64_t)gridDim.x * 256) {
    uint32_t light = 0, qhc = 0, qhr = 0;
    for (uint64_t r = PLN_QUAD * g; r < PLN_QUAD * g + PLN_QUAD && r < n_rows; ++r) {
      uint32_t nsat = 0, hcol = 0;
#pragma unroll
      for (int b = 0; b < 5; ++b) {
        const uint32_t c = counts[r * 5 + b];
        const uint32_t s = nsat + c;
        nsat = s < nsat ? 0xffffffffu : s;
        my_total += c;
        my_cells += c != 0u;
        my_cmax = c > my_cmax ? c : my_cmax;
        if (b < ncol) {
          light += (c != 0 && c <= SRT_CL);
          hcol += (c > SRT_CL);
        }
      }
      qhc += hcol;
      qhr += nsat > SRT_CL;
      if (hcol) atomicAdd(&s_heavy[0], hcol);
      if (nsat > SRT_CL) {
        atomicAdd(&s_heavy[1], 1u);
        if (nsat <= PLN_NBIG) atomicAdd(&s_big[nsat], 1u);
      } else if (nsat != 0) atomicAdd(&s_hist[nsat - 1], 1u);
      const uint32_t c4 = counts[r * 5 + 4];
      if (ncol == 4 && c4 > SRT_CL) atomicAdd(&s_heavy[2], 1u);
      else if (ncol == 4 && c4 != 0) atomicAdd(&s_hist[SRT_NKEY + c4 - 1], 1u);
    }
    quad_light[g] = (uint8_t)light;
    quad_light[n_quads + g] = (uint8_t)qhc;
    quad_light[2 * n_quads + g] = (uint8_t)qhr;
  }
  if (my_total) {
    atomicAdd(&s_total, my_total);
    atomicAdd(&s_cells, (unsigned long long)my_cells);
    atomicMax(&s_cmax, my_cmax);
  }
  __syncthreads();
  if (threadIdx.x == 0 && s_total) {
    atomicAdd(&heavy_counts[6], s_total);
    atomicAdd(&heavy_counts[7], s_cells);
    atomicMax(&heavy_counts[8], (unsigned long long)s_cmax);
  }
  if (threadIdx.x < 3 && s_heavy[threadIdx.x]) atomicAdd(&heavy_counts[threadIdx.x], (unsigned long long)s_heavy[threadIdx.x]);
  if (threadIdx.x < 2 * SRT_NKEY && s_hist[threadIdx.x]) atomicAdd(&hist[threadIdx.x], (unsigned long long)s_hist[threadIdx.x]);
  for (uint32_t k = threadIdx.x; k <= PLN_NBIG; k += 256)
    if (s_big[k]) atomicAdd(&hist[2 * SRT_NKEY + k], (unsigned long long)s_big[k]);
}

#define PLN_CUT_CHUNK_MAX 8192
static inline uint32_t plan_cut_chunk(uint64_t n_quads) { return n_quads <= 50000000ull ? 2048u : (uint32_t)PLN_CUT_CHUNK_MAX; }
#define PLN_CUT_SPAN (PLN_RMAX / PLN_QUAD)

__device__ __forceinline__ uint64_t plan_cut_one(const uint8_t *__restrict__ quad, uint64_t n_quads, uint64_t q0, uint32_t *items,
                                                 uint32_t *hcol, uint32_t *hrow) {
  uint32_t it = 0, hc = 0, hr = 0, rows = 0;
  uint64_t q = q0;
  while (q < n_quads && rows + PLN_QUAD <= PLN_RMAX && it + quad[q] <= PLN_NI_CUT) {
    it += quad[q];
    if (hcol) {
      hc += quad[n_quads + q];
      hr += quad[2 * n_quads + q];
    }
    rows += PLN_QUAD;
    ++q;
  }
  *items = it;
  if (hcol) {
    *hcol = hc;
    *hrow = hr;
  }
  return q;
}
__global__ __launch_bounds__(256) void plan_cut_step_kernel(const uint8_t *__restrict__ quad, uint64_t n_quads, uint64_t n_chunks,
                                                            uint32_t chunk, uint16_t *__restrict__ step) {
  const uint64_t k = (uint64_t)blockIdx.x * 256 + threadIdx.x;
  if (k >= n_chunks) return;
  const uint64_t q0 = k * chunk, q_end = q0 + chunk < n_quads ? q0 + chunk : n_quads;
  uint64_t r = q0;
  uint32_t items = 0;
  for (uint64_t q = q0; q < q_end; ++q) {
    if (r < q) {
      r = q;
      items = 0;
    }
    while (r < n_quads && (uint32_t)(r - q + 1) * PLN_QUAD <= PLN_RMAX && items + quad[r] <= PLN_NI_CUT) items += quad[r++];
    step[q] = (uint16_t)(r - q);
    items -= quad[q];
  }
}
__global__ __launch_bounds__(256) void plan_cut_walk_kernel(const uint16_t *__restrict__ step, uint64_t n_quads, uint64_t n_chunks,
                                                            uint32_t chunk, uint32_t *__restrict__ walk) {
  const uint64_t id = (uint64_t)blockIdx.x * 256 + threadIdx.x;
  if (id >= n_chunks * PLN_CUT_SPAN) return;
  const uint64_t k = id / PLN_CUT_SPAN, j = id - k * PLN_CUT_SPAN, end = (k + 1) * chunk;
  uint64_t q = k * chunk + j;
  uint32_t cnt = 0;
  while (q < end && q < n_quads) {
    q += step[q];
    ++cnt;
  }
  walk[id] = (uint32_t)(q >= end ? q - end : 0) | (cnt << 16);
}
static_assert(PLN_CUT_CHUNK_MAX < 65536 && PLN_CUT_SPAN < 65536 && PLN_CUT_SPAN <= 2048, "walk table: 16-bit fields; a tile is shorter than a chunk");
__global__ void plan_cut_chain_kernel(const uint32_t *__restrict__ walk, uint64_t n_chunks, uint32_t chunk, uint64_t *__restrict__ entry,
                                      uint64_t *__restrict__ base, unsigned long long *__restrict__ meta) {
  if (blockIdx.x || threadIdx.x) return;
  uint64_t j = 0, tiles = 0;
  for (uint64_t k = 0; k < n_chunks; ++k) {
    entry[k] = k * chunk + j;
    base[k] = tiles;
    const uint32_t w = walk[k * PLN_CUT_SPAN + j];
    tiles += w >> 16;
    j = w & 0xffffu;
  }
  meta[0] = tiles;
}
__global__ __launch_bounds__(256) void plan_cut_write_kernel(const uint8_t *__restrict__ quad, uint64_t n_quads, uint64_t n_rows, int ncol,
                                                             uint64_t n_chunks, uint32_t chunk, const uint64_t *__restrict__ entry,
                                                             const uint64_t *__restrict__ base, pln_tile *__restrict__ tiles) {
  const uint64_t k = (uint64_t)blockIdx.x * 256 + threadIdx.x;
  if (k >= n_chunks) return;
  const uint64_t end = (k + 1) * chunk;
  uint64_t q = entry[k], t = base[k];
  while (q < end && q < n_quads) {
    uint32_t items, hcol, hrow;
    const uint64_t q1 = plan_cut_one(quad, n_quads, q, &items, &hcol, &hrow);
    pln_tile ti;
    ti.row0 = q * PLN_QUAD;
    uint32_t rows = (uint32_t)(q1 - q) * PLN_QUAD;
    if (ti.row0 + rows > n_rows) rows = (uint32_t)(n_rows - ti.row0);
    const uint32_t hc = hcol < PLN_HCAP ? hcol : PLN_HCAP;
    const uint32_t hr = ncol == 5 ? (hrow < PLN_HCAP ? hrow : PLN_HCAP) : 0u;
    ti.rows_items = (rows << 16) | items;
    ti.off16 = 0;
    ti.hc_hr = (hc << 16) | hr;
    ti.blk16 = pln_block_layout(rows, items, hc, hr).end / 16;
    ti.pad = 0;
    tiles[t++] = ti;
    q = q1;
  }
}
__global__ __launch_bounds__(1024) void plan_cut_offsets_kernel(pln_tile *__restrict__ tiles, uint64_t n_tiles,
                                                                unsigned long long *__restrict__ meta) {
  __shared__ unsigned long long part[1024];
  const uint64_t per = (n_tiles + 1023) / 1024, lo = per * threadIdx.x, hi = lo + per < n_tiles ? lo + per : n_tiles;
  unsigned long long s = 0;
  for (uint64_t t = lo; t < hi; ++t) s += tiles[t].blk16;
  part[threadIdx.x] = s;
  __syncthreads();
  if (threadIdx.x == 0) {
    unsigned long long run = 0;
    for (int k = 0; k < 1024; ++k) {
      const unsigned long long v = part[k];
      part[k] = run;
      run += v;
    }
    meta[1] = run;
    meta[2] = run > 0xffffffffull ? 1ull : 0ull;
  }
  __syncthreads();
  unsigned long long off = part[threadIdx.x];
  for (uint64_t t = lo; t < hi; ++t) {
    tiles[t].off16 = (uint32_t)off;
    off += tiles[t].blk16;
  }
}

__global__ __launch_bounds__(1024) void plan_fill_kernel(const uint32_t *__restrict__ counts, uint64_t n_rows, int ncol,
                                                         const pln_tile *__restrict__ tiles, uint64_t n_tiles,
                                                         unsigned char *__restrict__ stream,
                                                         pln_heavy_col *__restrict__ heavy_col,
                                                         pln_heavy_row *__restrict__ heavy_row,
                                                         uint64_t *__restrict__ heavy_stop,
                                                         unsigned long long *__restrict__ cursors) {
  constexpr int RPT = (PLN_RMAX + 1023) / 1024;
  __shared__ uint32_t hist[SRT_NHIST];
  __shared__ uint32_t offs[SRT_NHIST];
  __shared__ uint32_t scan[16];
  __shared__ uint16_t sorted[PLN_NI + 64];
  __shared__ uint32_t s_hc, s_hr;
#ifdef BEAR_DET_BUILD
  __shared__ uint32_t comp[PLN_NI];
  static_assert((PLN_NI & (PLN_NI - 1)) == 0 && PLN_NI <= 2048, "bitonic sort over the tile's items: PLN_NI / 2 pairs, at most one per thread");
  __shared__ unsigned long long hkey[PLN_HCAP], htmp[PLN_HCAP];
#endif
  const uint32_t tid = threadIdx.x, rep = tid & (SRT_REP - 1);
  for (uint64_t t = blockIdx.x; t < n_tiles; t += gridDim.x) {
    const pln_tile ti = tiles[t];
    const uint32_t rows = ti.rows_items >> 16, n_light = ti.rows_items & 0xffffu;
    const uint32_t hc_cap = ti.hc_hr >> 16, hr_cap = ti.hc_hr & 0xffffu;
    const pln_layout L = pln_block_layout(rows, n_light, hc_cap, hr_cap);
    unsigned char *blk = stream + (size_t)ti.off16 * 16;
    uint16_t *E = reinterpret_cast<uint16_t *>(blk);
    uint8_t *nrow = blk + L.nrow;
    uint16_t *items = reinterpret_cast<uint16_t *>(blk + L.items);
    uint16_t *hoff = reinterpret_cast<uint16_t *>(blk + L.hoff);
    uint32_t *hcnt = reinterpret_cast<uint32_t *>(blk + L.hcnt);
    uint16_t *hrow = reinterpret_cast<uint16_t *>(blk + L.hrow);
    double *hn = reinterpret_cast<double *>(blk + L.hn);
    if (tid < SRT_NHIST) hist[tid] = 0;
    if (tid == 0) {
      s_hc = 0;
      s_hr = 0;
    }
    __syncthreads();
#ifdef BEAR_DET_BUILD
    uint32_t det_hc[RPT], det_hr[RPT];
    {
      uint32_t base_c = 0, base_r = 0;
#pragma unroll
      for (int k = 0; k < RPT; ++k) {
        const uint32_t lr = tid + 1024u * k;
        uint32_t nc = 0, nr = 0;
        if (lr < rows) {
          double n = 0.0;
          for (int b = 0; b < 5; ++b) {
            const uint32_t cv = counts[(ti.row0 + lr) * 5 + b];
            n += (double)cv;
            nc += (b < ncol && cv > SRT_CL) ? 1u : 0u;
          }
          nr = n > (double)SRT_CL ? 1u : 0u;
        }
        const uint32_t packed = nc | (nr << 16);
        const int lane = tid & 63, wave = tid >> 6;
        uint32_t incl = packed;
#pragma unroll
        for (int off = 1; off < 64; off <<= 1) {
          const uint32_t o = (uint32_t)__shfl_up((int)incl, off, 64);
          if (lane >= off) incl += o;
        }
        __syncthreads();
        if (lane == 63) scan[wave] = incl;
        __syncthreads();
        uint32_t before = 0, total = 0;
        for (int w = 0; w < 16; ++w) {
          if (w < wave) before += scan[w];
          total += scan[w];
        }
        const uint32_t excl = before + incl - packed;
        det_hc[k] = base_c + (excl & 0xffffu);
        det_hr[k] = base_r + (excl >> 16);
        base_c += total & 0xffffu;
        base_r += total >> 16;
      }
      __syncthreads();
      if (tid == 0) {
        s_hc = base_c;
        s_hr = base_r;
      }
    }
#endif
    uint32_t c[RPT][5], rank[RPT][5];
#pragma unroll
    for (int k = 0; k < RPT; ++k) {
      const uint32_t lr = tid + 1024u * k;
#pragma unroll
      for (int b = 0; b < 5; ++b) {
        c[k][b] = 0;
        rank[k][b] = 0;
      }
      if (lr < rows) {
        const uint64_t r = ti.row0 + lr;
        double n = 0.0;
#pragma unroll
        for (int b = 0; b < 5; ++b) {
          c[k][b] = counts[r * 5 + b];
          n += (double)c[k][b];
        }
        nrow[lr] = n < 1.0 ? (uint8_t)0 : (n <= (double)SRT_CL ? (uint8_t)n : (uint8_t)255);
        if (n > (double)SRT_CL) {
#ifdef BEAR_DET_BUILD
          const uint32_t k2 = hr_cap ? det_hr[k] : 0xffffffffu;
#else
          const uint32_t k2 = hr_cap ? atomicAdd(&s_hr, 1u) : 0xffffffffu;
#endif
          if (k2 < hr_cap) {
            hrow[k2] = (uint16_t)lr;
            hn[k2] = n;
          } else {
            const unsigned long long q = atomicAdd(&cursors[1], 1ull);
            heavy_row[q].row = r;
            heavy_row[q].n = n;
          }
        }
        if (ncol == 4 && c[k][4] > SRT_CL) heavy_stop[atomicAdd(&cursors[2], 1ull)] = c[k][4];
#pragma unroll
        for (int b = 0; b < 5; ++b) {
          if (b >= ncol) c[k][b] = 0;
          if (c[k][b] > SRT_CL) {
#ifdef BEAR_DET_BUILD
            const uint32_t k2 = hc_cap ? det_hc[k]++ : 0xffffffffu;
#else
            const uint32_t k2 = hc_cap ? atomicAdd(&s_hc, 1u) : 0xffffffffu;
#endif
            if (k2 < hc_cap) {
              hoff[k2] = (uint16_t)(lr * 5 + b);
              hcnt[k2] = c[k][b];
            } else {
              const unsigned long long q = atomicAdd(&cursors[0], 1ull);
              heavy_col[q].off = r * 5 + b;
              heavy_col[q].c = c[k][b];
            }
            c[k][b] = 0;
          }
          if (c[k][b] != 0) rank[k][b] = atomicAdd(&hist[(c[k][b] - 1) * SRT_REP + rep], 1u);
        }
      } else if (lr < ((rows + 15u) & ~15u)) {
        nrow[lr] = 0;
      }
    }
    __syncthreads();
    {
      const uint32_t v = tid < SRT_NHIST ? hist[tid] : 0u;
      const int lane = tid & 63, wave = tid >> 6;
      uint32_t incl = v;
#pragma unroll
      for (int off = 1; off < 64; off <<= 1) {
        uint32_t o = (uint32_t)__shfl_up((int)incl, off, 64);
        if (lane >= off) incl += o;
      }
      if (lane == 63) scan[wave] = incl;
      __syncthreads();
      uint32_t base = 0;
      for (int w = 0; w < wave; ++w) base += scan[w];
      if (tid < SRT_NHIST) offs[tid] = base + incl - v;
    }
    __syncthreads();
    if (tid < 30) E[tid] = (uint16_t)(tid < SRT_CL ? offs[tid * SRT_REP] : n_light);
    if (tid == 30) E[30] = (uint16_t)hc_cap;
    if (tid == 31) E[31] = (uint16_t)hr_cap;
#pragma unroll
    for (int k = 0; k < RPT; ++k)
#pragma unroll
      for (int b = 0; b < 5; ++b)
        if (c[k][b] != 0) sorted[offs[(c[k][b] - 1) * SRT_REP + rep] + rank[k][b]] = (uint16_t)((tid + 1024u * k) * 5 + b);
    __syncthreads();
#ifdef BEAR_DET_BUILD
    {
      for (uint32_t i = tid; i < PLN_NI; i += 1024) {
        uint32_t key = 0;
        for (uint32_t q = 1; q < SRT_CL; ++q) key += offs[q * SRT_REP] <= i ? 1u : 0u;
        comp[i] = i < n_light ? (key << 16) | sorted[i] : 0xffffffffu;
      }
      __syncthreads();
      for (uint32_t size = 2; size <= PLN_NI; size <<= 1)
        for (uint32_t stride = size >> 1; stride > 0; stride >>= 1) {
          const uint32_t lo = 2u * tid - (tid & (stride - 1u)), hi = lo + stride;
          if (tid < PLN_NI / 2) {
            const bool up = (lo & size) == 0u;
            const uint32_t a = comp[lo], bq = comp[hi];
            if ((a > bq) == up) {
              comp[lo] = bq;
              comp[hi] = a;
            }
          }
          __syncthreads();
        }
      for (uint32_t i = tid; i < n_light; i += 1024) sorted[i] = (uint16_t)(comp[i] & 0xffffu);
      __syncthreads();
      const uint32_t nhc = s_hc < hc_cap ? s_hc : hc_cap, nhr = s_hr < hr_cap ? s_hr : hr_cap;
      if (tid < nhc) hkey[tid] = ((unsigned long long)hoff[tid] << 32) | hcnt[tid];
      __syncthreads();
      if (tid < nhc) {
        uint32_t r = 0;
        for (uint32_t q = 0; q < nhc; ++q) r += hkey[q] < hkey[tid] ? 1u : 0u;
        htmp[r] = hkey[tid];
      }
      __syncthreads();
      if (tid < nhc) {
        hoff[tid] = (uint16_t)(htmp[tid] >> 32);
        hcnt[tid] = (uint32_t)htmp[tid];
      }
      __syncthreads();
      if (tid < nhr) hkey[tid] = ((unsigned long long)hrow[tid] << 48) | tid;
      if (tid < nhr) htmp[tid] = (unsigned long long)__double_as_longlong(hn[tid]);
      __syncthreads();
      uint32_t r = 0;
      unsigned long long mine = 0ull, myn = 0ull;
      if (tid < nhr) {
        for (uint32_t q = 0; q < nhr; ++q) r += hkey[q] < hkey[tid] ? 1u : 0u;
        mine = hkey[tid];
        myn = htmp[tid];
      }
      __syncthreads();
      if (tid < nhr) {
        hrow[r] = (uint16_t)(mine >> 48);
        hn[r] = __longlong_as_double((long long)myn);
      }
      __syncthreads();
    }
#endif
    const uint32_t padded = (n_light + 63u) & ~63u;
    for (uint32_t i = tid; i < padded; i += 1024) items[i] = i < n_light ? sorted[i] : (uint16_t)PLN_SENTINEL;
    __syncthreads();
  }
}

__global__ __launch_bounds__(1024) void plan_live_kernel(const pln_tile *__restrict__ tiles, uint64_t n_tiles,
                                                         const unsigned char *__restrict__ stream, uint16_t *__restrict__ live) {
  constexpr int RPT = (PLN_RMAX + 1023) / 1024;
  __shared__ uint32_t cnt[RPT * 16];
  const uint32_t tid = threadIdx.x, lane = tid & 63, wave = tid >> 6;
  for (uint64_t t = blockIdx.x; t < n_tiles; t += gridDim.x) {
    const pln_tile ti = tiles[t];
    const uint32_t rows = ti.rows_items >> 16;
    const uint8_t *nrow = stream + (size_t)ti.off16 * 16 + 64;
    uint16_t *out = live + t * PLN_LIVE_STRIDE;
    unsigned long long mask[RPT];
#pragma unroll
    for (int k = 0; k < RPT; ++k) {
      const uint32_t lr = tid + 1024u * k;
      mask[k] = __builtin_amdgcn_ballot_w64(lr < rows && nrow[lr] != 0);
      if (lane == 0) cnt[k * 16 + wave] = (uint32_t)__builtin_popcountll(mask[k]);
    }
    __syncthreads();
    uint32_t total = 0;
#pragma unroll
    for (int k = 0; k < RPT; ++k) {
      uint32_t base = total;
      for (int w = 0; w < 16; ++w) {
        const uint32_t c = cnt[k * 16 + w];
        if (w < (int)wave) base += c;
        total += c;
      }
      if ((mask[k] >> lane) & 1ull) out[1 + base + (uint32_t)__builtin_popcountll(mask[k] & ((1ull << lane) - 1ull))] = (uint16_t)(tid + 1024u * k);
    }
    if (tid == 0) out[0] = (uint16_t)total;
    __syncthreads();
  }
}

template <bool NORM, bool AR>
__global__ __launch_bounds__(PLN_THREADS, 4) void dm_prior_plan_kernel(const double *__restrict__ prior,
                                                                                    uint64_t n_rows, bear_params prm_arg,
                                                                                    pln_view pv,
                                                                                    const double2 *__restrict__ logtab_g,
                                                                                    double *__restrict__ partials,
                                                                                    const bear_step_io io
#ifdef PLN_STAMPS
                                                                                    , unsigned long long *__restrict__ dbg
#endif
                                                                                    ) {
  extern __shared__ __attribute__((aligned(16))) unsigned char srt_smem[];
  pln_lds_n &S = *reinterpret_cast<pln_lds_n *>(srt_smem);
  const bear_params prm = bear_params_of(prm_arg, io);
  const uint32_t tid = threadIdx.x, lane = tid & 63, wave = srt_uniform(tid >> 6);
  const double u = prm.inv_h, eps = prm.eps, eps5 = 5.0 * prm.eps;
  double acc[2] = {0.0, 0.0};

  if (tid < BEAR_LOGTAB_N) S.logtab[tid] = logtab_g[tid];
  if (tid < SRT_NKEY) {
    const bear_dp o = srt_general_fast(u + eps5, (double)(tid + 1), logtab_g);
    S.tabD[tid] = o.D;
    S.tabP[tid] = o.P;
  }
  if (tid < PLN_NBUF) {
    S.buf[tid].pri[PLN_SENTINEL] = 1.0;
    S.ticket[tid] = PLN_TICKET_START(PLN_WAVES - PLN_DMA_WAVES);
    S.sum_fail[tid] = 0xffffffffu;
  }

  const bool dma_wave = wave >= PLN_WAVES - PLN_DMA_WAVES;
  const uint32_t dw = wave - (PLN_WAVES - PLN_DMA_WAVES);
  constexpr bool GEN = !NORM && !AR;
  constexpr bool NT = GEN && PLN_GEN_NT;
  auto stage = [&](const pln_tile &ti, uint32_t b, bool with_nrow) {
    const uint32_t rows = ti.rows_items >> 16;
    if (rows == 0) return;
    const uint32_t pbytes = (rows * 40u) & ~15u, bbytes = ti.blk16 * 16u;
    const unsigned char *psrc = reinterpret_cast<const unsigned char *>(prior + ti.row0 * 5);
    const unsigned char *bsrc = pv.stream + (size_t)ti.off16 * 16;
    if (GEN && dw == 0 && lane == 0) S.nrow_in[b] = with_nrow ? 1u : 0u;
    if (!GEN || with_nrow) {
      for (uint32_t pc = dw; (pc << 10) < bbytes; pc += PLN_DMA_WAVES) pln_dma_piece<NT>(S.buf[b].blk, bsrc, bbytes, pc, lane);
    } else {
      const uint32_t items0 = pln_block_layout(rows, ti.rows_items & 0xffffu, ti.hc_hr >> 16, ti.hc_hr & 0xffffu).items;
      if (dw == PLN_DMA_WAVES - 1) pln_dma_piece<NT>(S.buf[b].blk, bsrc, 64u, 0u, lane);
      for (uint32_t pc = dw; (pc << 10) < bbytes - items0; pc += PLN_DMA_WAVES)
        pln_dma_piece<NT>(S.buf[b].blk + items0, bsrc + items0, bbytes - items0, pc, lane);
    }
    for (uint32_t pc = dw; (pc << 10) < pbytes; pc += PLN_DMA_WAVES) pln_dma_piece<NT>(S.buf[b].pri, psrc, pbytes, pc, lane);
    if (dw == 0 && ((rows * 40u) & 15u)) {
      const __attribute__((address_space(4))) double *tail =
          (const __attribute__((address_space(4))) double *)(uintptr_t)(prior + (ti.row0 + rows) * 5 - 1);
      const double v = *tail;
      if (lane == 0) S.buf[b].pri[rows * 5 - 1] = v;
    }
  };

  constexpr uint32_t PF_INSTR = (NORM || AR || PLN_GEN_PREFETCH) ? PLN_PREFETCH_KIB / 8u : 0u;
  auto prefetch_behind = [&](const pln_tile &ti) -> uint32_t {
    const uint32_t rows = ti.rows_items >> 16;
    if (PF_INSTR == 0 || rows == 0) return 0u;
    const uint64_t end_bytes = n_rows * 40ull, base = (ti.row0 + rows) * 40ull;
    const uint32_t m = srt_uniform((uint32_t)(uintptr_t)S.pf_scratch);
    uint32_t issued = 0;
    for (uint32_t k = dw; k < PF_INSTR; k += PLN_DMA_WAVES) {
      uint64_t off = base + ((uint64_t)(k * 64u + lane) << 7);
      if (off + 4u > end_bytes) off = end_bytes - 4u;
      const unsigned char *g = reinterpret_cast<const unsigned char *>(prior) + off;
      uint32_t keep_m0;
      asm volatile("s_mov_b32 %0, m0\n\ts_mov_b32 m0, %2\n\ts_nop 0\n\tglobal_load_lds_dword %1, off\n\ts_mov_b32 m0, %0"
                   : "=&s"(keep_m0)
                   : "v"(g), "s"(m)
                   : "memory");
      ++issued;
    }
    return issued;
  };
  uint32_t pf_young = 0;
#ifdef PLN_STAMPS
  unsigned long long tph[8] = {0, 0, 0, 0, 0, 0, 0, 0}, t_prev = __builtin_amdgcn_s_memtime();
  int prev_kind = 0;
#define PLN_STAMP(k)                                              \
  {                                                               \
    const unsigned long long now = __builtin_amdgcn_s_memtime();  \
    tph[k] += now - t_prev;                                       \
    t_prev = now;                                                 \
  }
#else
#define PLN_STAMP(k)
#endif
  static_assert(PLN_NBUF == 2, "the DMA-wave protocol below is written for a two-slot ring");
  const uint64_t G = gridDim.x;
  const uint64_t first = (pv.n_tiles * (uint64_t)blockIdx.x) / G, count = (pv.n_tiles * ((uint64_t)blockIdx.x + 1)) / G - first;
  auto fetch_desc = [&](uint64_t j0) {
    if (dw == 0 && j0 < count)
      pln_dma_piece(S.desc[(j0 >> 5) & 1u], pv.tiles + first + j0, PLN_DESC_CHUNK * (uint32_t)sizeof(pln_tile), 0u, lane);
  };
  if (dma_wave) {
    __builtin_amdgcn_s_setprio(3);
    fetch_desc(0);
    fetch_desc(PLN_DESC_CHUNK);
    srt_wait_dma();
  }
  __syncthreads();
  pln_tile cur = pln_desc(S.desc, 0, count), nxt = pln_desc(S.desc, 1, count);
  if (dma_wave) stage(cur, 0, !PLN_GEN_NROW_ON_DEMAND);
  uint32_t slot = 0;
  for (uint64_t j = 0; j < count; ++j) {
#ifdef PLN_STAMPS
    PLN_STAMP(prev_kind)
    prev_kind = 4;
#endif
    if (dma_wave) pln_wait_all_but(pf_young);
    PLN_STAMP(1)
    srt_sync();
    PLN_STAMP(2)
    const pln_tile nn = pln_desc(S.desc, j + 2, count);
    if (dma_wave) {
      if ((j & (PLN_DESC_CHUNK - 1)) == 0 && j != 0) fetch_desc(j + PLN_DESC_CHUNK);
      stage(nxt, slot ^ 1u, !GEN || !PLN_GEN_NROW_ON_DEMAND || srt_uniform(S.sum_fail[slot ^ 1u]) == (uint32_t)j);
      pf_young = prefetch_behind(nxt);
      cur = nxt;
      nxt = nn;
      slot ^= 1u;
      continue;
    }
    PLN_STAMP(3)

    const pln_buf_n &B = S.buf[slot];
    const uint32_t rows = cur.rows_items >> 16, n_light = cur.rows_items & 0xffffu;
    const uint32_t hc = cur.hc_hr >> 16, hr = cur.hc_hr & 0xffffu;
    const pln_layout L = pln_block_layout(rows, n_light, hc, hr);
    const uint16_t *E = reinterpret_cast<const uint16_t *>(B.blk);
    const uint8_t *nrow = B.blk + L.nrow;
    const uint16_t *items = reinterpret_cast<const uint16_t *>(B.blk + L.items);
    if (tid == 0) S.ticket[(slot + 1) % PLN_NBUF] = PLN_TICKET_START(PLN_WAVES - PLN_DMA_WAVES);
    const uint32_t n_hcu = (hc + 63u) >> 6, n_hru = AR ? 0u : (hr + 63u) >> 6, n_heavy = n_hcu + n_hru;
    const uint32_t n_units = (n_light + 63u) >> 6;
    const uint32_t n_work = n_heavy + n_units;
    static_assert(PLN_CHUNK == 128, "two adjacent contexts per lane");
    for (uint32_t c = wave; GEN && c * PLN_CHUNK < rows; c += PLN_WAVES - PLN_DMA_WAVES) {
      const uint32_t row0c = c * PLN_CHUNK + 2u * lane;
      const uint32_t rr = row0c < rows ? row0c : 0u;
      const double2 *src = reinterpret_cast<const double2 *>(&B.pri[rr * 5]);
      const double2 v0 = src[0], v1 = src[1], v2 = src[2], v3 = src[3], v4 = src[4];
      const double S5[2] = {((v0.x + v0.y) + (v1.x + v1.y)) + v2.x, ((v2.y + v3.x) + (v3.y + v4.x)) + v4.y};
      bool bad[2];
#pragma unroll
      for (int q = 0; q < 2; ++q) bad[q] = row0c + q < rows && !(__builtin_fabs(S5[q] - 1.0) <= SRT_SUM1_TOL);
      if (__builtin_amdgcn_ballot_w64(bad[0] || bad[1])) {
        if (lane == 0) S.sum_fail[slot] = (uint32_t)(j + 1);
        uint32_t nn_[2];
        if (!PLN_GEN_NROW_ON_DEMAND || srt_uniform(S.nrow_in[slot])) {
#pragma unroll
          for (int q = 0; q < 2; ++q) nn_[q] = bad[q] ? (uint32_t)nrow[rr + q] : 0u;
        } else {
          const uint8_t *g = pv.stream + (size_t)cur.off16 * 16 + L.nrow;
#pragma unroll
          for (int q = 0; q < 2; ++q) nn_[q] = bad[q] ? (uint32_t)g[rr + q] : 0u;
        }
#pragma unroll
        for (int q = 0; q < PLN_CHUNK / 64; ++q) {
          const uint32_t own = nn_[q] == 255u ? 0u : nn_[q];
          if (__builtin_amdgcn_ballot_w64(own != 0)) {
            uint32_t cm = own;
#pragma unroll
            for (int off = 32; off > 0; off >>= 1) {
              const uint32_t o2 = (uint32_t)__shfl_xor((int)cm, off, 64);
              cm = o2 > cm ? o2 : cm;
            }
            const double xa[1] = {own ? __builtin_fma(S5[q], u, eps5) : 1.0};
            const uint32_t ca[1] = {own};
            bear_dp o[1];
            srt_light<1>(xa, ca, 0u, srt_uniform(cm), S.logtab, o);
            if (own) {
              acc[0] += S.tabD[own - 1] - o[0].D;
              acc[1] = __builtin_fma(xa[0] - eps5, o[0].P, __builtin_fma(-u, S.tabP[own - 1], acc[1]));
            }
          }
        }
      }
    }
    PLN_FOR_UNITS_F(w, &S.ticket[slot], n_work, wave, PLN_WAVES - PLN_DMA_WAVES) {
#ifdef PLN_STAMPS
      {
        const unsigned long long now = __builtin_amdgcn_s_memtime();
        tph[prev_kind] += now - t_prev;
        t_prev = now;
        prev_kind = w < n_heavy ? 5 : 6;
      }
#endif
      if (w < n_hcu) {
        const uint32_t i = w * 64u + lane;
        if (i < hc) {
          const uint32_t off = reinterpret_cast<const uint16_t *>(B.blk + L.hoff)[i];
          const double cnt = (double)reinterpret_cast<const uint32_t *>(B.blk + L.hcnt)[i];
          if (AR) {
            acc[0] = __builtin_fma(cnt, bear_log_tab(B.pri[off] + eps, S.logtab), acc[0]);
          } else {
            const double x = __builtin_fma(B.pri[off], u, eps);
            const bear_dp o = srt_general_fast(x, cnt, S.logtab);
            acc[0] += o.D;
            acc[1] = __builtin_fma(eps - x, o.P, acc[1]);
          }
        }
        continue;
      }
      if (w < n_heavy) {
        const uint32_t i = (w - n_hcu) * 64u + lane;
        if (i < hr) {
          const double *f = &B.pri[(uint32_t)reinterpret_cast<const uint16_t *>(B.blk + L.hrow)[i] * 5u];
          const double A = NORM ? u + eps5 : __builtin_fma(((f[0] + f[1]) + (f[2] + f[3])) + f[4], u, eps5);
          const bear_dp o = srt_general_fast(A, reinterpret_cast<const double *>(B.blk + L.hn)[i], S.logtab);
          acc[0] -= o.D;
          acc[1] = __builtin_fma(A - eps5, o.P, acc[1]);
        }
        continue;
      }
      {
        const uint32_t un = n_heavy + n_units - 1u - w;
        uint32_t cmin, cmax;
        const uint32_t ci[1] = {pln_unit_counts(E, n_light, un, lane, &cmin, &cmax)};
        const uint32_t off = items[un * 64u + lane];
        if (AR) {
          acc[0] = __builtin_fma((double)ci[0], bear_log_tab(B.pri[off] + eps, S.logtab), acc[0]);
          continue;
        }
        const double x[1] = {__builtin_fma(B.pri[off], u, eps)};
        bear_dp o[1];
        srt_light<1>(x, ci, cmin, cmax, S.logtab, o);
        acc[0] += o[0].D;
        acc[1] = __builtin_fma(eps - x[0], o[0].P, acc[1]);
        continue;
      }
    }
    cur = nxt;
    nxt = nn;
    slot ^= 1u;
  }
  srt_wait_dma();
#ifdef PLN_STAMPS
  if (lane == 0 && dbg) {
    for (int k = 0; k < 8; ++k) dbg[((size_t)blockIdx.x * PLN_WAVES + wave) * 8 + k] = tph[k];
  }
#endif
  const uint64_t gtid = (uint64_t)blockIdx.x * PLN_THREADS + tid, gsz = (uint64_t)gridDim.x * PLN_THREADS;
  for (uint64_t i = gtid; i < pv.n_heavy_col; i += gsz) {
    const pln_heavy_col h = pv.heavy_col[i];
    if (AR) {
      acc[0] = __builtin_fma((double)h.c, bear_log_tab(prior[h.off] + eps, S.logtab), acc[0]);
      continue;
    }
    const double x = __builtin_fma(prior[h.off], u, eps);
    const bear_dp o = srt_general_fast(x, (double)h.c, S.logtab);
    acc[0] += o.D;
    acc[1] = __builtin_fma(eps - x, o.P, acc[1]);
  }
  for (uint64_t i = gtid; !AR && i < pv.n_heavy_row; i += gsz) {
    const pln_heavy_row h = pv.heavy_row[i];
    const double *f = prior + h.row * 5;
    const double A = __builtin_fma(((f[0] + f[1]) + (f[2] + f[3])) + f[4], u, eps5);
    const bear_dp o = srt_general_fast(A, h.n, S.logtab);
    acc[0] -= o.D;
    acc[1] = __builtin_fma(A - eps5, o.P, acc[1]);
  }
  if (!AR && blockIdx.x == 0 && tid < SRT_CL) {
    const double m = (double)pv.hist[tid];
    acc[0] -= m * S.tabD[tid];
    acc[1] = __builtin_fma(u * m, S.tabP[tid], acc[1]);
  }
  __syncthreads();
  block_finish<2>(acc, partials, io);
}

struct pln_buf_r {
  uint32_t ref[PLN_RMAX * 5 + 4];
  __attribute__((aligned(16))) unsigned char blk[PLN_BLOCK_MAX];
};
#define PLN_RSLOT 3
struct pln_lds_r {
  pln_buf_r buf[PLN_RSLOT];
  double2 logtab[BEAR_LOGTAB_N];
  double tabD[2][SRT_NKEY];
  double tabP[2][SRT_NKEY];
  uint32_t meta[PLN_RSLOT][2];
  uint32_t ticket[PLN_RSLOT];
  uint32_t landed[PLN_RSLOT];
  uint32_t left[PLN_RSLOT];
};

template <bool AR>
__global__ __launch_bounds__(PLN_THREADS, 4) void dm_ref_plan_kernel(const uint32_t *__restrict__ ref,
                                                                                  uint64_t n_rows, bear_params prm_arg,
                                                                                  pln_view pv,
                                                                                  const double2 *__restrict__ logtab_g,
                                                                                  double *__restrict__ partials,
                                                                                  const bear_step_io io, const bear_apply_io apply) {
  extern __shared__ __attribute__((aligned(16))) unsigned char srt_smem[];
  pln_lds_r &S = *reinterpret_cast<pln_lds_r *>(srt_smem);
  const bear_params prm = bear_params_of(prm_arg, io);
  const uint32_t tid = threadIdx.x, lane = tid & 63, wave = srt_uniform(tid >> 6);
  const double u = prm.inv_h, eps = prm.eps;
  const double A = u + 5.0 * eps;
  const double x4 = prm.nw * prm.V * u + eps;
  const double VU = prm.V * u;
  const double tau = prm.tau;
  const double w2c = tau * (eps + 0.25 * VU);
  const double nwV = prm.nw * prm.V;
  double acc[4] = {0.0, 0.0, 0.0, 0.0};

  if (tid < BEAR_LOGTAB_N) S.logtab[tid] = logtab_g[tid];
  if (tid < 2 * SRT_NKEY) {
    const int which = tid / SRT_NKEY, j = tid % SRT_NKEY;
    const bear_dp o = srt_general_fast(which ? x4 : A, (double)(j + 1), logtab_g);
    S.tabD[which][j] = o.D;
    S.tabP[which][j] = o.P;
  }
  if (tid < PLN_RSLOT) {
    S.landed[tid] = S.left[tid] = 0u;
    S.ticket[tid] = PLN_TICKET_START(PLN_WAVES - PLN_DMA_WAVES);
  }
  if (tid < 4 * PLN_RSLOT) S.buf[tid >> 2].ref[PLN_SENTINEL + (tid & 3)] = 0;

  const bool dma_wave = wave >= PLN_WAVES - PLN_DMA_WAVES;
  const uint32_t dw = wave - (PLN_WAVES - PLN_DMA_WAVES);
  constexpr uint32_t CWAVES = PLN_WAVES - PLN_DMA_WAVES;
  auto stage = [&](const pln_tile &ti, uint32_t b) {
    const uint32_t rows = ti.rows_items >> 16;
    const uint32_t rbytes = rows * 20u, rb16 = rbytes & ~15u, bbytes = ti.blk16 * 16u;
    const unsigned char *rsrc = reinterpret_cast<const unsigned char *>(ref + ti.row0 * 5);
    const unsigned char *bsrc = pv.stream + (size_t)ti.off16 * 16;
    for (uint32_t pc = 0; (pc << 10) < bbytes; ++pc) pln_dma_piece(S.buf[b].blk, bsrc, bbytes, pc, lane);
    for (uint32_t pc = 0; (pc << 10) < rb16; ++pc) pln_dma_piece(S.buf[b].ref, rsrc, rb16, pc, lane);
    if (rbytes & 15u) {
      const uint32_t w0 = rb16 >> 2, nw = (rbytes & 15u) >> 2;
      const __attribute__((address_space(4))) uint32_t *tail =
          (const __attribute__((address_space(4))) uint32_t *)(uintptr_t)(ref + ti.row0 * 5 + w0);
      const uint32_t v0 = tail[0], v1 = nw > 1 ? tail[1] : 0u, v2 = nw > 2 ? tail[2] : 0u;
      if (lane == 0) {
        S.buf[b].ref[w0] = v0;
        if (nw > 1) S.buf[b].ref[w0 + 1] = v1;
        if (nw > 2) S.buf[b].ref[w0 + 2] = v2;
      }
    }
    if (lane == 0) {
      S.meta[b][0] = ti.rows_items;
      S.meta[b][1] = ti.hc_hr;
      S.ticket[b] = PLN_TICKET_START(PLN_WAVES - PLN_DMA_WAVES);
    }
  };
  auto alpha_from = [&](double rb, double R) {
    const double dev = __builtin_fma(rb + eps, bear_rcp(R), -0.25);
    return __builtin_fma(__builtin_fma(prm.E, dev, 0.25), VU, eps);
  };
  auto accumulate = [&](double x, const bear_dp &o) {
    const double w1 = eps - x;
    acc[0] += o.D;
    acc[1] = __builtin_fma(w1, o.P, acc[1]);
    acc[2] = __builtin_fma(__builtin_fma(-tau, x, w2c), o.P, acc[2]);
    acc[3] = __builtin_fma(nwV * w1, o.P, acc[3]);
  };
  auto accumulate_ar = [&](double rb, double R, double c) {
    const double dev = __builtin_fma(rb + eps, bear_rcp(R), -0.25);
    const double f = __builtin_fma(prm.E, dev, 0.25) * prm.V;
    const double p = f + eps;
    const double dLdf = c * bear_rcp(p);
    acc[0] = __builtin_fma(c, bear_log_tab(p, S.logtab), acc[0]);
    acc[2] = __builtin_fma(dLdf, -prm.tauE * dev * prm.V, acc[2]);
    acc[3] = __builtin_fma(dLdf, -nwV * f, acc[3]);
  };

  const uint64_t G = gridDim.x;
  const uint64_t first = (pv.n_tiles * (uint64_t)blockIdx.x) / G, count = (pv.n_tiles * ((uint64_t)blockIdx.x + 1)) / G - first;
  __syncthreads();
  if (dma_wave) {
    __builtin_amdgcn_s_setprio(3);
    pln_tile ti = pln_load_tile(pv, dw < count ? first + dw : pv.n_tiles);
    for (uint64_t j = dw; j < count; j += PLN_DMA_WAVES) {
      const uint32_t b = (uint32_t)(j % PLN_RSLOT), gen = (uint32_t)(j / PLN_RSLOT);
      const pln_tile ti_next = pln_load_tile(pv, j + PLN_DMA_WAVES < count ? first + j + PLN_DMA_WAVES : pv.n_tiles);
      while (pln_peek(&S.left[b]) < CWAVES * gen) __builtin_amdgcn_s_sleep(1);
      stage(ti, b);
      srt_wait_dma();
      asm volatile("s_waitcnt lgkmcnt(0)" ::: "memory");
      if (lane == 0) atomicAdd(&S.landed[b], 1u);
      ti = ti_next;
    }
  }
  for (uint64_t j = 0; !dma_wave && j < count; ++j) {
    const uint32_t slot = (uint32_t)(j % PLN_RSLOT), gen = (uint32_t)(j / PLN_RSLOT);
    while (pln_peek(&S.landed[slot]) < gen + 1u) __builtin_amdgcn_s_sleep(1);
    const pln_buf_r &B = S.buf[slot];
    const uint32_t rows_items = srt_uniform(S.meta[slot][0]), hc_hr = srt_uniform(S.meta[slot][1]);
    const uint32_t rows = rows_items >> 16, n_light = rows_items & 0xffffu;
    const uint32_t hc = hc_hr >> 16;
    const pln_layout L = pln_block_layout(rows, n_light, hc, hc_hr & 0xffffu);
    const uint16_t *E = reinterpret_cast<const uint16_t *>(B.blk);
    const uint16_t *items = reinterpret_cast<const uint16_t *>(B.blk + L.items);
    const uint32_t n_hcu = (hc + 63u) >> 6;
    const uint32_t n_units = (n_light + 63u) >> 6;
    PLN_FOR_UNITS_F(w, &S.ticket[slot], n_hcu + n_units, wave, CWAVES) {
      if (w < n_hcu) {
        const uint32_t i = w * 64u + lane;
        if (i < hc) {
          const uint32_t off = reinterpret_cast<const uint16_t *>(B.blk + L.hoff)[i];
          const uint32_t *rr = &B.ref[((off * 52429u) >> 18) * 5u];
          const double R = (double)(((uint64_t)rr[0] + rr[1]) + ((uint64_t)rr[2] + rr[3])) + 4.0 * eps;
          const double cnt = (double)reinterpret_cast<const uint32_t *>(B.blk + L.hcnt)[i];
          if (AR) {
            accumulate_ar((double)B.ref[off], R, cnt);
          } else {
            const double x = alpha_from((double)B.ref[off], R);
            accumulate(x, srt_general_fast(x, cnt, S.logtab));
          }
        }
        continue;
      }
      const uint32_t un = n_hcu + n_units - 1u - w;
      uint32_t cmin, cmax;
      const uint32_t ci[1] = {pln_unit_counts(E, n_light, un, lane, &cmin, &cmax)};
      const uint32_t off = items[un * 64u + lane];
      const uint32_t *rr = &B.ref[((off * 52429u) >> 18) * 5u];
      const double R = (double)(((uint64_t)rr[0] + rr[1]) + ((uint64_t)rr[2] + rr[3])) + 4.0 * eps;
      if (AR) {
        accumulate_ar((double)B.ref[off], R, (double)ci[0]);
        continue;
      }
      const double x[1] = {alpha_from((double)B.ref[off], R)};
      bear_dp o[1];
      srt_light<1>(x, ci, cmin, cmax, S.logtab, o);
      accumulate(x[0], o[0]);
    }
    asm volatile("s_waitcnt lgkmcnt(0)" ::: "memory");
    if (lane == 0) atomicAdd(&S.left[slot], 1u);
  }
  srt_wait_dma();
  const uint64_t gtid = (uint64_t)blockIdx.x * PLN_THREADS + tid, gsz = (uint64_t)gridDim.x * PLN_THREADS;
  for (uint64_t i = gtid; i < pv.n_heavy_col; i += gsz) {
    const pln_heavy_col h = pv.heavy_col[i];
    const uint32_t *rr = ref + (h.off / 5) * 5;
    const double R = (double)(((uint64_t)rr[0] + rr[1]) + ((uint64_t)rr[2] + rr[3])) + 4.0 * eps;
    if (AR) {
      accumulate_ar((double)ref[h.off], R, (double)h.c);
      continue;
    }
    const double x = alpha_from((double)ref[h.off], R);
    accumulate(x, srt_general_fast(x, (double)h.c, S.logtab));
  }
  if (AR) {
    const double f4 = nwV, p4 = f4 + eps;
    double c4sum = 0.0;
    if (blockIdx.x == 0 && tid < SRT_CL) c4sum = (double)(tid + 1) * (double)pv.hist[SRT_NKEY + tid];
    for (uint64_t i = gtid; i < pv.n_heavy_stop; i += gsz) c4sum += (double)pv.heavy_stop[i];
    acc[0] = __builtin_fma(c4sum, bear_log_tab(p4, S.logtab), acc[0]);
    acc[3] = __builtin_fma(c4sum * bear_rcp(p4), nwV * (1.0 - f4), acc[3]);
    __syncthreads();
    block_finish<4>(acc, partials, io, apply);
    return;
  }
  for (uint64_t i = gtid; i < pv.n_heavy_row; i += gsz) {
    const double n = pv.heavy_row[i].n;
    if (pln_in_big_hist(pv, n)) continue;
    const bear_dp o = srt_general_fast(A, n, S.logtab);
    acc[0] -= o.D;
    acc[1] = __builtin_fma(u, o.P, acc[1]);
  }
  pln_big_totals(pv, A, u, gtid, gsz, S.logtab, acc[0], acc[1]);
  for (uint64_t i = gtid; i < pv.n_heavy_stop; i += gsz) {
    const bear_dp o = srt_general_fast(x4, (double)pv.heavy_stop[i], S.logtab);
    acc[0] += o.D;
    acc[1] = __builtin_fma(eps - x4, o.P, acc[1]);
    acc[3] = __builtin_fma(VU * nwV, o.P, acc[3]);
  }
  if (blockIdx.x == 0 && tid < SRT_CL) {
    const double mn = (double)pv.hist[tid], m4 = (double)pv.hist[SRT_NKEY + tid];
    acc[0] -= mn * S.tabD[0][tid];
    acc[1] = __builtin_fma(u * mn, S.tabP[0][tid], acc[1]);
    const double P4 = m4 * S.tabP[1][tid];
    acc[0] += m4 * S.tabD[1][tid];
    acc[1] = __builtin_fma(eps - x4, P4, acc[1]);
    acc[3] = __builtin_fma(VU * nwV, P4, acc[3]);
  }
  __syncthreads();
  block_finish<4>(acc, partials, io, apply);
}

struct pln_lds_g {
  double pri[PLN_RMAX * 5 + 2];
  double grad[PLN_RMAX * 5 + 2];
  __attribute__((aligned(16))) unsigned char blk[PLN_BLOCK_MAX];
  double2 logtab[BEAR_LOGTAB_N];
  double tabD[SRT_NKEY];
  double tabP[SRT_NKEY];
  uint32_t ticket;
  __attribute__((aligned(16))) uint32_t pf_scratch[64];
};
static_assert(sizeof(pln_lds_g) <= 158 * 1024, "gradient-row kernel: LDS budget");

__device__ __forceinline__ void pln_touch_lines(uint32_t *scratch, const void *src, uint32_t bytes, uint32_t k, uint32_t lane) {
  const uint32_t off = (k * 64u + lane) << 7;
  if (off < bytes) {
    const unsigned char *g = static_cast<const unsigned char *>(src) + off;
    const uint32_t m = srt_uniform((uint32_t)(uintptr_t)scratch);
    uint32_t keep_m0;
    asm volatile("s_mov_b32 %0, m0\n\ts_mov_b32 m0, %2\n\ts_nop 0\n\tglobal_load_lds_dword %1, off\n\ts_mov_b32 m0, %0"
                 : "=&s"(keep_m0)
                 : "v"(g), "s"(m)
                 : "memory");
  }
}

template <bool NORM, bool AR>
__global__ __launch_bounds__(PLN_THREADS, 4) void dm_prior_plan_grad_kernel(const double *__restrict__ prior,
                                                                                         bear_params prm_arg, pln_view pv,
                                                                                         const double2 *__restrict__ logtab_g,
                                                                                         double *__restrict__ grad_out,
                                                                                         double *__restrict__ partials,
                                                                                         const bear_step_io io) {
  extern __shared__ __attribute__((aligned(16))) unsigned char srt_smem[];
  pln_lds_g &S = *reinterpret_cast<pln_lds_g *>(srt_smem);
  const bear_params prm = bear_params_of(prm_arg, io);
  const uint32_t tid = threadIdx.x, lane = tid & 63, wave = srt_uniform(tid >> 6);
  const double u = prm.inv_h, eps = prm.eps, eps5 = 5.0 * prm.eps;
  double acc[2] = {0.0, 0.0};
  if (tid < BEAR_LOGTAB_N) S.logtab[tid] = logtab_g[tid];
  if (tid < SRT_NKEY) {
    const bear_dp o = srt_general_fast(u + eps5, (double)(tid + 1), logtab_g);
    S.tabD[tid] = o.D;
    S.tabP[tid] = o.P;
  }
  if (tid == 0) {
    S.pri[PLN_SENTINEL] = 1.0;
    S.ticket = PLN_TICKET_START(PLN_WAVES);
  }
  pln_tile nxt = pln_load_tile(pv, blockIdx.x);
  for (uint64_t t = blockIdx.x; t < pv.n_tiles; t += gridDim.x) {
    const pln_tile cur = nxt;
    const uint32_t rows = cur.rows_items >> 16, n_light = cur.rows_items & 0xffffu;
    const uint32_t hc = cur.hc_hr >> 16, hr = cur.hc_hr & 0xffffu;
    const pln_layout L = pln_block_layout(rows, n_light, hc, hr);
    __syncthreads();
    {
      const uint32_t pbytes = rows * 40u;
      pln_dma(S.pri, prior + cur.row0 * 5, pbytes & ~15u, wave, lane, 0);
      if (pbytes & 15u) {
        const __attribute__((address_space(4))) double *tail =
            (const __attribute__((address_space(4))) double *)(uintptr_t)(prior + (cur.row0 + rows) * 5 - 1);
        const double v = *tail;
        if (tid == 0) S.pri[rows * 5 - 1] = v;
      }
      pln_dma(S.blk, pv.stream + (size_t)cur.off16 * 16, cur.blk16 * 16u, wave, lane, (pbytes + 1023u) >> 10);
    }
    if (tid == 0) S.ticket = PLN_TICKET_START(PLN_WAVES);
    nxt = pln_load_tile(pv, t + gridDim.x);
    srt_wait_dma();
    srt_sync();
    const uint16_t *E = reinterpret_cast<const uint16_t *>(S.blk);
    const uint8_t *nrow = S.blk + L.nrow;
    const uint16_t *items = reinterpret_cast<const uint16_t *>(S.blk + L.items);
    for (uint32_t row = tid; AR && row < rows; row += PLN_THREADS) {
#pragma unroll
      for (int b = 0; b < 5; ++b) S.grad[row * 5 + b] = 0.0;
    }
    for (uint32_t row = tid; !AR && row < rows; row += PLN_THREADS) {
      double f[5];
#pragma unroll
      for (int b = 0; b < 5; ++b) f[b] = S.pri[row * 5 + b];
      const double S5 = ((f[0] + f[1]) + (f[2] + f[3])) + f[4];
      uint32_t n = nrow[row];
      if (n == 255u) n = 0u;
      const bool shared = NORM || __builtin_fabs(S5 - 1.0) <= SRT_SUM1_TOL;
      double Pn = 0.0;
      if (n != 0 && shared) {
        Pn = S.tabP[n - 1];
        acc[0] -= S.tabD[n - 1];
        acc[1] = __builtin_fma(u, Pn, acc[1]);
      }
      if (n != 0 && !shared) {
        const double A = __builtin_fma(S5, u, eps5);
        const bear_dp o = srt_general_fast(A, (double)n, S.logtab);
        Pn = o.P;
        acc[0] -= o.D;
        acc[1] = __builtin_fma(A - eps5, o.P, acc[1]);
      }
      const double base = -u * Pn;
#pragma unroll
      for (int b = 0; b < 5; ++b) S.grad[row * 5 + b] = base;
    }
    srt_sync();
    for (uint32_t i = tid; !AR && i < hr; i += PLN_THREADS) {
      const uint32_t row = reinterpret_cast<const uint16_t *>(S.blk + L.hrow)[i];
      const double *f = &S.pri[row * 5u];
      const double A = NORM ? u + eps5 : __builtin_fma(((f[0] + f[1]) + (f[2] + f[3])) + f[4], u, eps5);
      const bear_dp o = srt_general_fast(A, reinterpret_cast<const double *>(S.blk + L.hn)[i], S.logtab);
      acc[0] -= o.D;
      acc[1] = __builtin_fma(A - eps5, o.P, acc[1]);
#pragma unroll
      for (int b = 0; b < 5; ++b) S.grad[row * 5 + b] = -u * o.P;
    }
    srt_sync();
    if (!AR && wave < 10u) {
      const pln_tile &nx = nxt;
      const uint32_t nrows = nx.rows_items >> 16;
      if (wave < 9u) pln_touch_lines(S.pf_scratch, prior + nx.row0 * 5, nrows * 40u, wave, lane);
      else pln_touch_lines(S.pf_scratch, pv.stream + (size_t)nx.off16 * 16, nx.blk16 * 16u, 0u, lane);
    }
    const uint32_t n_hcu = (hc + 63u) >> 6, n_units = (n_light + 63u) >> 6;
    PLN_FOR_UNITS_F(w, &S.ticket, n_hcu + n_units, wave, PLN_WAVES) {
      if (w < n_hcu) {
        const uint32_t i = w * 64u + lane;
        if (i < hc) {
          const uint32_t off = reinterpret_cast<const uint16_t *>(S.blk + L.hoff)[i];
          const double cnt = (double)reinterpret_cast<const uint32_t *>(S.blk + L.hcnt)[i];
          if (AR) {
            const double pp = S.pri[off] + eps;
            acc[0] = __builtin_fma(cnt, bear_log_tab(pp, S.logtab), acc[0]);
            S.grad[off] = cnt * bear_rcp(pp);
          } else {
            const double x = __builtin_fma(S.pri[off], u, eps);
            const bear_dp o = srt_general_fast(x, cnt, S.logtab);
            acc[0] += o.D;
            acc[1] = __builtin_fma(eps - x, o.P, acc[1]);
            S.grad[off] = __builtin_fma(u, o.P, S.grad[off]);
          }
        }
        continue;
      }
      const uint32_t un = n_hcu + n_units - 1u - w;
      uint32_t cmin, cmax;
      const uint32_t ci[1] = {pln_unit_counts(E, n_light, un, lane, &cmin, &cmax)};
      const uint32_t off = items[un * 64u + lane];
      if (AR) {
        const double pp = S.pri[off] + eps;
        acc[0] = __builtin_fma((double)ci[0], bear_log_tab(pp, S.logtab), acc[0]);
        if (ci[0] != 0) S.grad[off] = (double)ci[0] * bear_rcp(pp);
        continue;
      }
      const double x[1] = {__builtin_fma(S.pri[off], u, eps)};
      bear_dp o[1];
      srt_light<1>(x, ci, cmin, cmax, S.logtab, o);
      acc[0] += o[0].D;
      acc[1] = __builtin_fma(eps - x[0], o[0].P, acc[1]);
      if (ci[0] != 0) S.grad[off] = __builtin_fma(u, o[0].P, S.grad[off]);
    }
    __syncthreads();
    {
      const uint32_t n_dw = rows * 10u;
      const uint4 *src = reinterpret_cast<const uint4 *>(S.grad);
      uint4 *dst = reinterpret_cast<uint4 *>(grad_out + cur.row0 * 5);
      for (uint32_t i = tid; i < (n_dw >> 2); i += PLN_THREADS) dst[i] = src[i];
      if ((n_dw & 3u) && tid == 0) grad_out[(cur.row0 + rows) * 5 - 1] = S.grad[rows * 5 - 1];
    }
  }
  __syncthreads();
  const uint64_t gtid = (uint64_t)blockIdx.x * PLN_THREADS + tid, gsz = (uint64_t)gridDim.x * PLN_THREADS;
  for (uint64_t i = gtid; i < pv.n_heavy_col; i += gsz) {
    const pln_heavy_col h = pv.heavy_col[i];
    if (AR) {
      acc[0] = __builtin_fma((double)h.c, bear_log_tab(prior[h.off] + eps, S.logtab), acc[0]);
      continue;
    }
    const double x = __builtin_fma(prior[h.off], u, eps);
    const bear_dp o = srt_general_fast(x, (double)h.c, S.logtab);
    acc[0] += o.D;
    acc[1] = __builtin_fma(eps - x, o.P, acc[1]);
  }
  for (uint64_t i = gtid; !AR && i < pv.n_heavy_row; i += gsz) {
    const pln_heavy_row h = pv.heavy_row[i];
    const double *f = prior + h.row * 5;
    const double A = NORM ? u + eps5 : __builtin_fma(((f[0] + f[1]) + (f[2] + f[3])) + f[4], u, eps5);
    const bear_dp o = srt_general_fast(A, h.n, S.logtab);
    acc[0] -= o.D;
    acc[1] = __builtin_fma(A - eps5, o.P, acc[1]);
  }
  __syncthreads();
  block_finish<2>(acc, partials, io);
}

struct pln_lds_gi {
  double pri[2][PLN_RMAX * 5 + 2];
  __attribute__((aligned(16))) unsigned char blk[2][PLN_BLOCK_MAX];
  double2 logtab[BEAR_LOGTAB_N];
  double tabD[SRT_NKEY];
  double tabP[SRT_NKEY];
  uint32_t ticket[2];
};
static_assert(sizeof(pln_lds_gi) <= 158 * 1024, "in-place gradient kernel: LDS budget");

__global__ __launch_bounds__(PLN_THREADS, 4) void dm_prior_plan_grad_inplace_kernel(const double *__restrict__ prior,
                                                                                                 bear_params prm_arg, pln_view pv,
                                                                                                 const double2 *__restrict__ logtab_g,
                                                                                                 double *__restrict__ grad_out,
                                                                                                 double *__restrict__ partials,
                                                                                                 const bear_step_io io) {
  extern __shared__ __attribute__((aligned(16))) unsigned char srt_smem[];
  pln_lds_gi &S = *reinterpret_cast<pln_lds_gi *>(srt_smem);
  const bear_params prm = bear_params_of(prm_arg, io);
  const uint32_t tid = threadIdx.x, lane = tid & 63, wave = srt_uniform(tid >> 6);
  const double u = prm.inv_h, eps = prm.eps, eps5 = 5.0 * prm.eps;
  double acc[2] = {0.0, 0.0};
  if (tid < BEAR_LOGTAB_N) S.logtab[tid] = logtab_g[tid];
  if (tid < SRT_NKEY) {
    const bear_dp o = srt_general_fast(u + eps5, (double)(tid + 1), logtab_g);
    S.tabD[tid] = o.D;
    S.tabP[tid] = o.P;
  }
  if (tid == 0) {
    S.pri[0][PLN_SENTINEL] = 1.0;
    S.pri[1][PLN_SENTINEL] = 1.0;
    S.ticket[0] = PLN_TICKET_START(PLN_WAVES);
    S.ticket[1] = PLN_TICKET_START(PLN_WAVES);
  }
  auto stage = [&](const pln_tile &ti, uint32_t b) {
    const uint32_t rows = ti.rows_items >> 16;
    if (rows == 0) return;
    const uint32_t pbytes = rows * 40u;
    pln_dma(S.pri[b], prior + ti.row0 * 5, pbytes & ~15u, wave, lane, 0);
    if (pbytes & 15u) {
      const __attribute__((address_space(4))) double *tail =
          (const __attribute__((address_space(4))) double *)(uintptr_t)(prior + (ti.row0 + rows) * 5 - 1);
      const double v = *tail;
      if (tid == 0) S.pri[b][rows * 5 - 1] = v;
    }
    pln_dma(S.blk[b], pv.stream + (size_t)ti.off16 * 16, ti.blk16 * 16u, wave, lane, (pbytes + 1023u) >> 10);
  };
  pln_tile cur = pln_load_tile(pv, blockIdx.x);
  stage(cur, 0);
  uint32_t b = 0;
  for (uint64_t t = blockIdx.x; t < pv.n_tiles; t += gridDim.x, b ^= 1u) {
    const pln_tile nxt = pln_load_tile(pv, t + gridDim.x);
    const uint32_t rows = cur.rows_items >> 16, n_light = cur.rows_items & 0xffffu;
    const uint32_t hc = cur.hc_hr >> 16, hr = cur.hc_hr & 0xffffu;
    const pln_layout L = pln_block_layout(rows, n_light, hc, hr);
    srt_wait_dma();
    srt_sync();
    stage(nxt, b ^ 1u);
    if (tid == 0) S.ticket[b ^ 1u] = PLN_TICKET_START(PLN_WAVES);
    double *P = S.pri[b];
    const unsigned char *blk = S.blk[b];
    const uint16_t *E = reinterpret_cast<const uint16_t *>(blk);
    const uint8_t *nrow = blk + L.nrow;
    const uint16_t *items = reinterpret_cast<const uint16_t *>(blk + L.items);
    const uint32_t n_hcu = (hc + 63u) >> 6, n_units = (n_light + 63u) >> 6;
    PLN_FOR_UNITS_F(w, &S.ticket[b], n_hcu + n_units, wave, PLN_WAVES) {
      if (w < n_hcu) {
        const uint32_t i = w * 64u + lane;
        if (i < hc) {
          const uint32_t off = reinterpret_cast<const uint16_t *>(blk + L.hoff)[i];
          const double cnt = (double)reinterpret_cast<const uint32_t *>(blk + L.hcnt)[i];
          const double x = __builtin_fma(P[off], u, eps);
          const bear_dp o = srt_general_fast(x, cnt, S.logtab);
          acc[0] += o.D;
          acc[1] = __builtin_fma(eps - x, o.P, acc[1]);
          P[off] = -(u * o.P);
        }
        continue;
      }
      const uint32_t un = n_hcu + n_units - 1u - w;
      uint32_t cmin, cmax;
      const uint32_t ci[1] = {pln_unit_counts(E, n_light, un, lane, &cmin, &cmax)};
      const uint32_t off = items[un * 64u + lane];
      const double x[1] = {__builtin_fma(P[off], u, eps)};
      bear_dp o[1];
      srt_light<1>(x, ci, cmin, cmax, S.logtab, o);
      acc[0] += o[0].D;
      acc[1] = __builtin_fma(eps - x[0], o[0].P, acc[1]);
      if (ci[0] != 0) P[off] = -(u * o[0].P);
    }
    srt_sync();
    for (uint32_t row = tid; row < rows; row += PLN_THREADS) {
      double base = 0.0;
      uint32_t n = nrow[row];
      if (n == 255u) n = 0u;
      if (n != 0) {
        const double Pn = S.tabP[n - 1];
        acc[0] -= S.tabD[n - 1];
        acc[1] = __builtin_fma(u, Pn, acc[1]);
        base = -u * Pn;
      }
#pragma unroll
      for (int c = 0; c < 5; ++c) {
        const double v = P[row * 5 + c];
        P[row * 5 + c] = (v < 0.0 ? -v : 0.0) + base;
      }
    }
    srt_sync();
    for (uint32_t i = tid; i < hr; i += PLN_THREADS) {
      const uint32_t row = reinterpret_cast<const uint16_t *>(blk + L.hrow)[i];
      const bear_dp o = srt_general_fast(u + eps5, reinterpret_cast<const double *>(blk + L.hn)[i], S.logtab);
      acc[0] -= o.D;
      acc[1] = __builtin_fma(u, o.P, acc[1]);
#pragma unroll
      for (int c = 0; c < 5; ++c) P[row * 5 + c] -= u * o.P;
    }
    srt_sync();
    {
      const uint32_t n_dw = rows * 10u;
      const uint4 *src = reinterpret_cast<const uint4 *>(P);
      uint4 *dst = reinterpret_cast<uint4 *>(grad_out + cur.row0 * 5);
      for (uint32_t i = tid; i < (n_dw >> 2); i += PLN_THREADS) dst[i] = src[i];
      if ((n_dw & 3u) && tid == 0) grad_out[(cur.row0 + rows) * 5 - 1] = P[rows * 5 - 1];
    }
    cur = nxt;
  }
  srt_wait_dma();
  __syncthreads();
  const uint64_t gtid = (uint64_t)blockIdx.x * PLN_THREADS + tid, gsz = (uint64_t)gridDim.x * PLN_THREADS;
  for (uint64_t i = gtid; i < pv.n_heavy_col; i += gsz) {
    const pln_heavy_col h = pv.heavy_col[i];
    const double x = __builtin_fma(prior[h.off], u, eps);
    const bear_dp o = srt_general_fast(x, (double)h.c, S.logtab);
    acc[0] += o.D;
    acc[1] = __builtin_fma(eps - x, o.P, acc[1]);
  }
  for (uint64_t i = gtid; i < pv.n_heavy_row; i += gsz) {
    const bear_dp o = srt_general_fast(u + eps5, pv.heavy_row[i].n, S.logtab);
    acc[0] -= o.D;
    acc[1] = __builtin_fma(u, o.P, acc[1]);
  }
  __syncthreads();
  block_finish<2>(acc, partials, io);
}

template <bool NORM, bool AR, bool ROWS>
__global__ __launch_bounds__(256) void dm_prior_grad_fixup_kernel(const double *__restrict__ prior, bear_params prm_arg, pln_view pv,
                                                                   const double2 *__restrict__ logtab_g,
                                                                   double *__restrict__ grad_out,
                                                                   const bear_step_io io) {
  const bear_params prm = bear_params_of(prm_arg, io);
  __shared__ double2 logtab[BEAR_LOGTAB_N];
  if (threadIdx.x < BEAR_LOGTAB_N) logtab[threadIdx.x] = logtab_g[threadIdx.x];
  __syncthreads();
  const double u = prm.inv_h, eps = prm.eps, eps5 = 5.0 * prm.eps;
  const uint64_t gtid = (uint64_t)blockIdx.x * 256 + threadIdx.x, gsz = (uint64_t)gridDim.x * 256;
  for (uint64_t i = gtid; !ROWS && i < pv.n_heavy_col; i += gsz) {
    const pln_heavy_col h = pv.heavy_col[i];
    if (AR) {
      grad_out[h.off] += (double)h.c * bear_rcp(prior[h.off] + eps);
      continue;
    }
    const double x = __builtin_fma(prior[h.off], u, eps);
    const bear_dp o = srt_general_fast(x, (double)h.c, logtab);
    grad_out[h.off] += u * o.P;
  }
  for (uint64_t i = gtid; ROWS && !AR && i < pv.n_heavy_row; i += gsz) {
    const pln_heavy_row h = pv.heavy_row[i];
    const double *f = prior + h.row * 5;
    const double A = NORM ? u + eps5 : __builtin_fma(((f[0] + f[1]) + (f[2] + f[3])) + f[4], u, eps5);
    const bear_dp o = srt_general_fast(A, h.n, logtab);
    for (int b = 0; b < 5; ++b) grad_out[h.row * 5 + b] -= u * o.P;
  }
}
```

Before: 141.8 billion.

## Rebuild plan creation with pooled scratch, parallel tile cut, and fused live pass

```diff
diff --git a/bear_amd/csrc/bear_common.h b/bear_amd/csrc/bear_common.h
--- a/bear_amd/csrc/bear_common.h
+++ b/bear_amd/csrc/bear_common.h
@@ -41,6 +41,8 @@
   unsigned epoch;
   double *cnn_partials;
   size_t cnn_partials_cap;
+  void *plan_scratch;
+  size_t plan_scratch_cap;
 };
 
 struct bear_params {
diff --git a/bear_amd/csrc/bear_hip.hip b/bear_amd/csrc/bear_hip.hip
--- a/bear_amd/csrc/bear_hip.hip
+++ b/bear_amd/csrc/bear_hip.hip
@@ -65,6 +65,7 @@
   (void)hipFree(ws->lin_accum);
   (void)hipFree(ws->cnn_partials);
   (void)hipFree(ws->arrive);
+  (void)hipFree(ws->plan_scratch);
   delete ws;
 }
 
@@ -238,6 +239,19 @@
   delete p;
 }
 
+static hipError_t plan_scratch(bear_ws *ws, size_t bytes, unsigned char **out) {
+  if (bytes > ws->plan_scratch_cap) {
+    (void)hipFree(ws->plan_scratch);
+    ws->plan_scratch = nullptr;
+    ws->plan_scratch_cap = 0;
+    const hipError_t e = hipMalloc(&ws->plan_scratch, bytes);
+    if (e != hipSuccess) return e;
+    ws->plan_scratch_cap = bytes;
+  }
+  *out = static_cast<unsigned char *>(ws->plan_scratch);
+  return hipSuccess;
+}
+
 int bear_plan_create(bear_ws *ws, const uint32_t *counts, uint64_t n_rows, int ncol, bear_plan **out) {
   if (!out) return BEAR_ERR_INVALID_ARG;
   *out = nullptr;
@@ -252,43 +266,66 @@
   p->n_rows = n_rows;
   p->counts = counts;
   hipError_t e = hipMalloc(&p->hist, sizeof(unsigned long long) * (2 * SRT_NKEY + PLN_NBIG + 1));
-  if (e == hipSuccess) e = hipMemset(p->hist, 0, sizeof(unsigned long long) * (2 * SRT_NKEY + PLN_NBIG + 1));
+  if (e == hipSuccess) e = hipMemsetAsync(p->hist, 0, sizeof(unsigned long long) * (2 * SRT_NKEY + PLN_NBIG + 1), 0);
   if (e != hipSuccess) {
     g_last_hip_error = (int)e;
     plan_free(p);
     return BEAR_ERR_HIP;
   }
   if (n_rows == 0) {
+    e = hipStreamSynchronize(0);
+    if (e != hipSuccess) {
+      g_last_hip_error = (int)e;
+      plan_free(p);
+      return BEAR_ERR_HIP;
+    }
     *out = p;
     return BEAR_OK;
   }
   const uint64_t n_quads = (n_rows + PLN_QUAD - 1) / PLN_QUAD;
-  uint8_t *d_quad = nullptr, *h_quad = nullptr;
-  unsigned long long *d_cnt = nullptr;
-  std::vector<pln_tile> tiles;
-  e = hipMalloc(&d_quad, 3 * n_quads);
-  if (e == hipSuccess) e = hipMalloc(&d_cnt, sizeof(unsigned long long) * 9);
-  if (e == hipSuccess) e = hipMemset(d_cnt, 0, sizeof(unsigned long long) * 9);
+  const uint64_t n_chunks = (n_quads + PLN_CUT_CHUNK - 1) / PLN_CUT_CHUNK;
+  const uint64_t n_maps1 = (n_chunks + PLN_CUT_FAN - 1) / PLN_CUT_FAN, n_maps2 = (n_maps1 + PLN_CUT_FAN - 1) / PLN_CUT_FAN;
+  const uint64_t max_tiles = plan_cut_max_tiles(n_quads);
+  enum { HDR_CNT = 0, HDR_META = 9, HDR_WORDS = 64 };
+  static_assert(HDR_META + 3 + SRT_NKEY <= HDR_WORDS, "header of the plan scratch");
+  size_t at = 0;
+  auto piece = [&at](size_t bytes) {
+    const size_t here = at;
+    at += (bytes + 255) & ~(size_t)255;
+    return here;
+  };
+  const size_t o_hdr = piece(sizeof(unsigned long long) * HDR_WORDS);
+  const size_t o_quad = piece(3 * n_quads);
+  const size_t o_step = piece(sizeof(uint16_t) * n_quads);
+  const size_t o_ent = piece(sizeof(uint64_t) * 2 * (n_chunks + n_maps1 + n_maps2));
+  const size_t o_map1 = piece(sizeof(uint64_t) * n_maps1 * PLN_CUT_SPAN);
+  const size_t o_map2 = piece(sizeof(uint64_t) * n_maps2 * PLN_CUT_SPAN);
+  const size_t walk_bytes = sizeof(uint32_t) * n_chunks * PLN_CUT_SPAN, desc_bytes = sizeof(pln_tile) * max_tiles;
+  const size_t o_walk = piece(walk_bytes > desc_bytes ? walk_bytes : desc_bytes);
+  unsigned char *scratch = nullptr;
+  e = plan_scratch(ws, at, &scratch);
+  unsigned long long *d_hdr = reinterpret_cast<unsigned long long *>(scratch + o_hdr), *d_cnt = d_hdr + HDR_CNT, *d_meta = d_hdr + HDR_META;
+  uint8_t *d_quad = scratch + o_quad;
+  if (e == hipSuccess) e = hipMemsetAsync(d_hdr, 0, sizeof(unsigned long long) * HDR_WORDS, 0);
   if (e == hipSuccess) {
     const int grid = grid_capped((n_quads + 255) / 256, (uint64_t)ws->num_cu * 8);
     hipLaunchKernelGGL(plan_scan_kernel, dim3(grid), dim3(256), 0, 0, counts, n_rows, ncol, d_quad, d_cnt, p->hist);
     e = hipGetLastError();
   }
-  unsigned long long h_cnt[3] = {0, 0, 0}, h_total[3] = {0, 0, 0};
-  if (e == hipSuccess) e = hipMemcpy(h_cnt, d_cnt, sizeof(h_cnt), hipMemcpyDeviceToHost);
-  if (e == hipSuccess) e = hipMemcpy(h_total, d_cnt + 6, sizeof(h_total), hipMemcpyDeviceToHost);
-  for (int k = 0; k < 3; ++k) p->count_total[k] = p->count_bound[k] = (double)h_total[k];
+  unsigned long long h_hdr[HDR_META + 3 + SRT_NKEY];
+  memset(h_hdr, 0, sizeof(h_hdr));
   uint64_t off16 = 0, n_tiles = 0;
   const char *cut_env = getenv("BEAR_PLAN_CUT");
   const bool host_cut = cut_env && cut_env[0] == 'h';
-  if (e == hipSuccess && host_cut) {
-    h_quad = (uint8_t *)malloc(3 * n_quads);
-    if (!h_quad) e = hipErrorOutOfMemory;
+  std::vector<pln_tile> tiles;
+  if (host_cut) {
+    uint8_t *h_quad = e == hipSuccess ? (uint8_t *)malloc(3 * n_quads) : nullptr;
+    if (e == hipSuccess && !h_quad) e = hipErrorOutOfMemory;
     if (e == hipSuccess) e = hipMemcpy(h_quad, d_quad, 3 * n_quads, hipMemcpyDeviceToHost);
-  }
-  if (e == hipSuccess && host_cut) {
+    if (e == hipSuccess) e = hipMemcpy(h_hdr, d_hdr, sizeof(unsigned long long) * HDR_META, hipMemcpyDeviceToHost);
+    if (e == hipSuccess) e = hipMemcpy(h_hdr + HDR_META + 3, p->hist, sizeof(unsigned long long) * SRT_NKEY, hipMemcpyDeviceToHost);
     uint64_t q = 0;
-    while (q < n_quads) {
+    while (e == hipSuccess && q < n_quads) {
       uint32_t items = 0, rows = 0, hcol = 0, hrow = 0;
       const uint64_t q0 = q;
       while (q < n_quads && rows + PLN_QUAD <= PLN_RMAX && items + h_quad[q] <= PLN_NI_CUT) {
@@ -316,76 +353,60 @@
       tiles.push_back(ti);
     }
     n_tiles = tiles.size();
-  }
-  free(h_quad);
-  if (e == hipSuccess && !host_cut) {
-    const uint32_t chunk = plan_cut_chunk(n_quads);
-    const uint64_t n_chunks = (n_quads + chunk - 1) / chunk;
-    uint32_t *d_walk = nullptr;
-    uint16_t *d_step = nullptr;
-    uint64_t *d_entry = nullptr;
-    unsigned long long *d_meta = nullptr, h_meta[3] = {0, 0, 0};
-    e = hipMalloc(&d_walk, sizeof(uint32_t) * n_chunks * PLN_CUT_SPAN);
-    if (e == hipSuccess) e = hipMalloc(&d_step, sizeof(uint16_t) * n_quads);
-    if (e == hipSuccess) e = hipMalloc(&d_entry, sizeof(uint64_t) * 2 * n_chunks);
-    if (e == hipSuccess) e = hipMalloc(&d_meta, sizeof(h_meta));
-    if (e == hipSuccess) e = hipMemset(d_meta, 0, sizeof(h_meta));
+    free(h_quad);
+  } else {
+    uint16_t *d_step = reinterpret_cast<uint16_t *>(scratch + o_step);
+    uint64_t *d_ent0 = reinterpret_cast<uint64_t *>(scratch + o_ent), *d_ent1 = d_ent0 + 2 * n_chunks, *d_ent2 = d_ent1 + 2 * n_maps1;
+    uint64_t *d_map1 = reinterpret_cast<uint64_t *>(scratch + o_map1), *d_map2 = reinterpret_cast<uint64_t *>(scratch + o_map2);
+    uint32_t *d_walk = reinterpret_cast<uint32_t *>(scratch + o_walk);
+    pln_tile *d_desc = reinterpret_cast<pln_tile *>(scratch + o_walk);
     if (e == hipSuccess) {
-      const uint64_t wb = (n_chunks * PLN_CUT_SPAN + 255) / 256;
-      hipLaunchKernelGGL(plan_cut_step_kernel, dim3((unsigned)((n_chunks + 255) / 256)), dim3(256), 0, 0, d_quad, n_quads, n_chunks, chunk, d_step);
-      hipLaunchKernelGGL(plan_cut_walk_kernel, dim3((unsigned)wb), dim3(256), 0, 0, d_step, n_quads, n_chunks, chunk, d_walk);
-      hipLaunchKernelGGL(plan_cut_chain_kernel, dim3(1), dim3(1), 0, 0, d_walk, n_chunks, chunk, d_entry, d_entry + n_chunks, d_meta);
+      auto blocks = [](uint64_t threads) { return dim3((unsigned)((threads + 255) / 256)); };
+      hipLaunchKernelGGL(plan_cut_len_kernel, dim3((unsigned)((n_quads + PLN_CUT_LEN_SPAN - 1) / PLN_CUT_LEN_SPAN)), dim3(256), 0, 0, d_quad,
+                         n_quads, d_step);
+      hipLaunchKernelGGL(plan_cut_walk_kernel, blocks(n_chunks * PLN_CUT_SPAN), dim3(256), 0, 0, d_step, n_quads, n_chunks, d_walk);
+      hipLaunchKernelGGL(plan_cut_compose_kernel<uint32_t>, blocks(n_maps1 * PLN_CUT_SPAN), dim3(256), 0, 0, d_walk, n_chunks, n_maps1, d_map1);
+      hipLaunchKernelGGL(plan_cut_compose_kernel<uint64_t>, blocks(n_maps2 * PLN_CUT_SPAN), dim3(256), 0, 0, d_map1, n_maps1, n_maps2, d_map2);
+      hipLaunchKernelGGL(plan_cut_descend_kernel<uint64_t>, dim3(1), dim3(256), 0, 0, d_map2, n_maps2, n_maps2, (const uint64_t *)nullptr,
+                         (uint64_t)1, d_ent2, d_meta);
+      hipLaunchKernelGGL(plan_cut_descend_kernel<uint64_t>, blocks(n_maps2), dim3(256), 0, 0, d_map1, n_maps1, (uint64_t)PLN_CUT_FAN, d_ent2,
+                         n_maps2, d_ent1, d_meta);
+      hipLaunchKernelGGL(plan_cut_descend_kernel<uint32_t>, blocks(n_maps1), dim3(256), 0, 0, d_walk, n_chunks, (uint64_t)PLN_CUT_FAN, d_ent1,
+                         n_maps1, d_ent0, d_meta);
+      hipLaunchKernelGGL(plan_cut_starts_kernel, blocks(n_chunks), dim3(256), 0, 0, d_step, n_quads, n_chunks, d_ent0, d_desc);
+      hipLaunchKernelGGL(plan_cut_desc_kernel, dim3((unsigned)((max_tiles + 3) / 4)), dim3(256), 0, 0, d_quad, d_step, n_quads, n_rows, ncol,
+                         d_meta, d_desc);
+      hipLaunchKernelGGL(plan_cut_offsets_kernel, dim3(1), dim3(1024), 0, 0, d_desc, p->hist, d_meta);
       e = hipGetLastError();
     }
-    if (e == hipSuccess) e = hipMemcpy(h_meta, d_meta, sizeof(unsigned long long), hipMemcpyDeviceToHost);
-    n_tiles = h_meta[0];
-    if (e == hipSuccess) e = hipMalloc(&p->tiles, sizeof(pln_tile) * (n_tiles + PLN_DESC_PAD));
-    if (e == hipSuccess) e = hipMemset(p->tiles, 0, sizeof(pln_tile) * (n_tiles + PLN_DESC_PAD));
-    if (e == hipSuccess) {
-      hipLaunchKernelGGL(plan_cut_write_kernel, dim3((unsigned)((n_chunks + 255) / 256)), dim3(256), 0, 0, d_quad, n_quads, n_rows, ncol,
-                         n_chunks, chunk, d_entry, d_entry + n_chunks, p->tiles);
-      hipLaunchKernelGGL(plan_cut_offsets_kernel, dim3(1), dim3(1024), 0, 0, p->tiles, n_tiles, d_meta);
-      e = hipGetLastError();
-    }
-    if (e == hipSuccess) e = hipMemcpy(h_meta, d_meta, sizeof(h_meta), hipMemcpyDeviceToHost);
-    if (e == hipSuccess && h_meta[2]) e = hipErrorOutOfMemory;
-    off16 = h_meta[1];
-    (void)hipFree(d_walk);
-    (void)hipFree(d_step);
-    (void)hipFree(d_entry);
-    (void)hipFree(d_meta);
-  }
-  (void)hipFree(d_quad);
+    if (e == hipSuccess) e = hipMemcpy(h_hdr, d_hdr, sizeof(h_hdr), hipMemcpyDeviceToHost);
+    if (e == hipSuccess && h_hdr[HDR_META + 2]) e = hipErrorOutOfMemory;
+    n_tiles = h_hdr[HDR_META];
+    off16 = h_hdr[HDR_META + 1];
+  }
+  const unsigned long long *h_cnt = h_hdr + HDR_CNT;
+  for (int k = 0; k < 3; ++k) p->count_total[k] = p->count_bound[k] = (double)h_hdr[HDR_CNT + 6 + k];
   p->n_tiles = n_tiles;
   const uint64_t stream_bytes = off16 * 16 + 1024;
-  for (int k = 0; k < 3; ++k) p->n_heavy[k] = h_cnt[k];
-  if (host_cut) {
-    if (e == hipSuccess) e = hipMalloc(&p->tiles, sizeof(pln_tile) * (tiles.size() + PLN_DESC_PAD));
-    if (e == hipSuccess) e = hipMemset(p->tiles, 0, sizeof(pln_tile) * (tiles.size() + PLN_DESC_PAD));
-    if (e == hipSuccess) e = hipMemcpy(p->tiles, tiles.data(), sizeof(pln_tile) * tiles.size(), hipMemcpyHostToDevice);
-  }
+  const uint64_t live_bytes = ncol == 5 ? sizeof(uint16_t) * PLN_LIVE_STRIDE * (n_tiles + 1) : 0;
+  if (e == hipSuccess) e = hipMalloc(&p->tiles, sizeof(pln_tile) * (n_tiles + PLN_DESC_PAD));
   if (e == hipSuccess) e = hipMalloc(&p->stream, stream_bytes);
-  if (e == hipSuccess) e = hipMemset(p->stream, 0, stream_bytes);
   if (e == hipSuccess && h_cnt[0]) e = hipMalloc(&p->heavy_col, sizeof(pln_heavy_col) * h_cnt[0]);
   if (e == hipSuccess && h_cnt[1]) e = hipMalloc(&p->heavy_row, sizeof(pln_heavy_row) * h_cnt[1]);
   if (e == hipSuccess && h_cnt[2]) e = hipMalloc(&p->heavy_stop, sizeof(uint64_t) * h_cnt[2]);
+  if (e == hipSuccess && live_bytes) e = hipMalloc(&p->live, live_bytes);
+  if (e == hipSuccess) e = hipMemsetAsync(p->tiles + n_tiles, 0, sizeof(pln_tile) * PLN_DESC_PAD, 0);
+  if (e == hipSuccess && n_tiles)
+    e = host_cut ? hipMemcpy(p->tiles, tiles.data(), sizeof(pln_tile) * n_tiles, hipMemcpyHostToDevice)
+                 : hipMemcpyAsync(p->tiles, scratch + o_walk, sizeof(pln_tile) * n_tiles, hipMemcpyDeviceToDevice, 0);
+  if (e == hipSuccess) e = hipMemsetAsync(p->stream + off16 * 16, 0, 1024, 0);
+  if (e == hipSuccess && live_bytes) e = hipMemsetAsync(p->live + n_tiles * PLN_LIVE_STRIDE, 0, sizeof(uint16_t) * PLN_LIVE_STRIDE, 0);
   if (e == hipSuccess) {
-    const uint64_t nt = n_tiles;
-    const int grid = grid_capped(nt, (uint64_t)ws->num_cu * 2);
-    hipLaunchKernelGGL(plan_fill_kernel, dim3(grid), dim3(1024), 0, 0, counts, n_rows, ncol, p->tiles, nt, p->stream,
-                       p->heavy_col, p->heavy_row, p->heavy_stop, d_cnt + 3);
+    const int grid = grid_capped(n_tiles, (uint64_t)ws->num_cu * PLN_FILL_BLOCKS_PER_CU);
+    hipLaunchKernelGGL(plan_fill_kernel, dim3(grid), dim3(PLN_FILL_THREADS), 0, 0, counts, n_rows, ncol, p->tiles, n_tiles, p->stream,
+                       p->heavy_col, p->heavy_row, p->heavy_stop, d_cnt + 3, p->live);
     e = hipGetLastError();
   }
-  const uint64_t live_bytes = ncol == 5 ? sizeof(uint16_t) * PLN_LIVE_STRIDE * (n_tiles + 1) : 0;
-  if (e == hipSuccess && live_bytes) e = hipMalloc(&p->live, live_bytes);
-  if (e == hipSuccess && live_bytes) e = hipMemset(p->live, 0, live_bytes);
-  if (e == hipSuccess && live_bytes) {
-    const uint64_t nt = n_tiles;
-    const int grid = grid_capped(nt, (uint64_t)ws->num_cu * 2);
-    hipLaunchKernelGGL(plan_live_kernel, dim3(grid), dim3(1024), 0, 0, p->tiles, nt, p->stream, p->live);
-    e = hipGetLastError();
-  }
-  if (e == hipSuccess) e = hipDeviceSynchronize();
   unsigned long long h_used[3] = {0, 0, 0};
   if (e == hipSuccess) e = hipMemcpy(h_used, d_cnt + 3, sizeof(h_used), hipMemcpyDeviceToHost);
   for (int k = 0; k < 3; ++k) p->n_heavy[k] = h_used[k];
@@ -401,14 +422,11 @@
     if (cst != BEAR_OK) e = cst == BEAR_ERR_NOMEM ? hipErrorOutOfMemory : hipErrorUnknown;
   }
   p->n_live_rows = n_rows;
-  if (e == hipSuccess && ncol == 5) {
-    unsigned long long h_hist[SRT_NKEY];
-    e = hipMemcpy(h_hist, p->hist, sizeof(h_hist), hipMemcpyDeviceToHost);
+  if (ncol == 5) {
     unsigned long long live_rows = h_cnt[1];
-    for (int k = 0; k < SRT_NKEY; ++k) live_rows += h_hist[k];
+    for (int k = 0; k < SRT_NKEY; ++k) live_rows += h_hdr[HDR_META + 3 + k];
     p->n_live_rows = live_rows;
   }
-  (void)hipFree(d_cnt);
   if (e != hipSuccess) {
     g_last_hip_error = (int)e;
     plan_free(p);
diff --git a/bear_amd/csrc/kernels_plan.h b/bear_amd/csrc/kernels_plan.h
--- a/bear_amd/csrc/kernels_plan.h
+++ b/bear_amd/csrc/kernels_plan.h
@@ -70,53 +70,83 @@
     if (s_big[k]) atomicAdd(&hist[2 * SRT_NKEY + k], (unsigned long long)s_big[k]);
 }
 
-#define PLN_CUT_CHUNK_MAX 8192
-static inline uint32_t plan_cut_chunk(uint64_t n_quads) { return n_quads <= 50000000ull ? 2048u : (uint32_t)PLN_CUT_CHUNK_MAX; }
 #define PLN_CUT_SPAN (PLN_RMAX / PLN_QUAD)
-
-__device__ __forceinline__ uint64_t plan_cut_one(const uint8_t *__restrict__ quad, uint64_t n_quads, uint64_t q0, uint32_t *items,
-                                                 uint32_t *hcol, uint32_t *hrow) {
-  uint32_t it = 0, hc = 0, hr = 0, rows = 0;
-  uint64_t q = q0;
-  while (q < n_quads && rows + PLN_QUAD <= PLN_RMAX && it + quad[q] <= PLN_NI_CUT) {
-    it += quad[q];
-    if (hcol) {
-      hc += quad[n_quads + q];
-      hr += quad[2 * n_quads + q];
-    }
-    rows += PLN_QUAD;
-    ++q;
-  }
-  *items = it;
-  if (hcol) {
-    *hcol = hc;
-    *hrow = hr;
-  }
-  return q;
-}
-__global__ __launch_bounds__(256) void plan_cut_step_kernel(const uint8_t *__restrict__ quad, uint64_t n_quads, uint64_t n_chunks,
-                                                            uint32_t chunk, uint16_t *__restrict__ step) {
-  const uint64_t k = (uint64_t)blockIdx.x * 256 + threadIdx.x;
-  if (k >= n_chunks) return;
-  const uint64_t q0 = k * chunk, q_end = q0 + chunk < n_quads ? q0 + chunk : n_quads;
-  uint64_t r = q0;
-  uint32_t items = 0;
-  for (uint64_t q = q0; q < q_end; ++q) {
-    if (r < q) {
-      r = q;
-      items = 0;
-    }
-    while (r < n_quads && (uint32_t)(r - q + 1) * PLN_QUAD <= PLN_RMAX && items + quad[r] <= PLN_NI_CUT) items += quad[r++];
-    step[q] = (uint16_t)(r - q);
-    items -= quad[q];
+#define PLN_CUT_LEN_SPAN 2048
+#define PLN_CUT_CHUNK 4096
+#define PLN_CUT_FAN 32
+#define PLN_CUT_MINLEN ((PLN_NI_CUT / (5 * PLN_QUAD)) < PLN_CUT_SPAN ? (PLN_NI_CUT / (5 * PLN_QUAD)) : PLN_CUT_SPAN)
+static_assert(PLN_NI_CUT >= 5 * PLN_QUAD && PLN_NI_CUT <= PLN_NI, "a tile takes at least one group");
+static_assert(PLN_CUT_SPAN < PLN_CUT_CHUNK && PLN_CUT_SPAN < 65536 && PLN_CUT_CHUNK / PLN_CUT_MINLEN + 1 < 65536,
+              "maps: 16 bits of exit offset (a tile is shorter than a chunk), tiles started above them");
+static inline uint64_t plan_cut_max_tiles(uint64_t n_quads) { return n_quads / PLN_CUT_MINLEN + 1; }
+
+__device__ __forceinline__ uint32_t plan_wave_scan(uint32_t v, uint32_t lane) {
+#pragma unroll
+  for (int off = 1; off < 64; off <<= 1) {
+    const uint32_t o = (uint32_t)__shfl_up((int)v, off, 64);
+    if (lane >= (uint32_t)off) v += o;
+  }
+  return v;
+}
+template <int WAVES>
+__device__ __forceinline__ uint32_t plan_block_scan(uint32_t v, uint32_t *part, uint32_t *total) {
+  const uint32_t lane = threadIdx.x & 63u, wave = threadIdx.x >> 6;
+  const uint32_t incl = plan_wave_scan(v, lane);
+  if (lane == 63u) part[wave] = incl;
+  srt_sync();
+  uint32_t before = 0, all = 0;
+#pragma unroll
+  for (int w = 0; w < WAVES; ++w) {
+    const uint32_t s = part[w];
+    before += (uint32_t)w < wave ? s : 0u;
+    all += s;
+  }
+  *total = all;
+  return before + incl - v;
+}
+
+__global__ __launch_bounds__(256) void plan_cut_len_kernel(const uint8_t *__restrict__ quad, uint64_t n_quads, uint16_t *__restrict__ step) {
+  constexpr uint32_t NP = PLN_CUT_LEN_SPAN + PLN_CUT_SPAN;
+  constexpr uint32_t PER = (NP + 255) / 256;
+  __shared__ uint32_t pre[256 * PER + 1];
+  __shared__ uint32_t part[4];
+  const uint32_t tid = threadIdx.x;
+  const uint64_t q0 = (uint64_t)blockIdx.x * PLN_CUT_LEN_SPAN;
+  uint32_t v[PER], sum = 0;
+#pragma unroll
+  for (uint32_t k = 0; k < PER; ++k) {
+    const uint32_t i = tid * PER + k;
+    v[k] = (i < NP && q0 + i < n_quads) ? quad[q0 + i] : 0u;
+    sum += v[k];
+  }
+  uint32_t total;
+  uint32_t run = plan_block_scan<4>(sum, part, &total);
+#pragma unroll
+  for (uint32_t k = 0; k < PER; ++k) {
+    pre[tid * PER + k] = run;
+    run += v[k];
+  }
+  if (tid == 255) pre[256 * PER] = run;
+  __syncthreads();
+  for (uint32_t i = tid; i < PLN_CUT_LEN_SPAN && q0 + i < n_quads; i += 256) {
+    const uint64_t left = n_quads - (q0 + i);
+    const uint32_t most = left < PLN_CUT_SPAN ? (uint32_t)left : (uint32_t)PLN_CUT_SPAN;
+    const uint32_t limit = pre[i] + PLN_NI_CUT;
+    uint32_t lo = 1, hi = most;
+    while (lo < hi) {
+      const uint32_t mid = (lo + hi + 1) >> 1;
+      if (pre[i + mid] <= limit) lo = mid;
+      else hi = mid - 1;
+    }
+    step[q0 + i] = (uint16_t)lo;
   }
 }
 __global__ __launch_bounds__(256) void plan_cut_walk_kernel(const uint16_t *__restrict__ step, uint64_t n_quads, uint64_t n_chunks,
-                                                            uint32_t chunk, uint32_t *__restrict__ walk) {
+                                                            uint32_t *__restrict__ walk) {
   const uint64_t id = (uint64_t)blockIdx.x * 256 + threadIdx.x;
   if (id >= n_chunks * PLN_CUT_SPAN) return;
-  const uint64_t k = id / PLN_CUT_SPAN, j = id - k * PLN_CUT_SPAN, end = (k + 1) * chunk;
-  uint64_t q = k * chunk + j;
+  const uint64_t k = id / PLN_CUT_SPAN, j = id - k * PLN_CUT_SPAN, end = (k + 1) * PLN_CUT_CHUNK;
+  uint64_t q = k * PLN_CUT_CHUNK + j;
   uint32_t cnt = 0;
   while (q < end && q < n_quads) {
     q += step[q];
@@ -124,176 +154,248 @@
   }
   walk[id] = (uint32_t)(q >= end ? q - end : 0) | (cnt << 16);
 }
-static_assert(PLN_CUT_CHUNK_MAX < 65536 && PLN_CUT_SPAN < 65536 && PLN_CUT_SPAN <= 2048, "walk table: 16-bit fields; a tile is shorter than a chunk");
-__global__ void plan_cut_chain_kernel(const uint32_t *__restrict__ walk, uint64_t n_chunks, uint32_t chunk, uint64_t *__restrict__ entry,
-                                      uint64_t *__restrict__ base, unsigned long long *__restrict__ meta) {
-  if (blockIdx.x || threadIdx.x) return;
-  uint64_t j = 0, tiles = 0;
-  for (uint64_t k = 0; k < n_chunks; ++k) {
-    entry[k] = k * chunk + j;
-    base[k] = tiles;
-    const uint32_t w = walk[k * PLN_CUT_SPAN + j];
+template <typename TIN>
+__global__ __launch_bounds__(256) void plan_cut_compose_kernel(const TIN *__restrict__ in, uint64_t n_in, uint64_t n_out,
+                                                               uint64_t *__restrict__ out) {
+  const uint64_t id = (uint64_t)blockIdx.x * 256 + threadIdx.x;
+  if (id >= n_out * PLN_CUT_SPAN) return;
+  const uint64_t g = id / PLN_CUT_SPAN;
+  const uint64_t k_end = (g + 1) * PLN_CUT_FAN < n_in ? (g + 1) * PLN_CUT_FAN : n_in;
+  uint64_t j = id - g * PLN_CUT_SPAN, tiles = 0;
+  for (uint64_t k = g * PLN_CUT_FAN; k < k_end; ++k) {
+    const uint64_t w = in[k * PLN_CUT_SPAN + j];
     tiles += w >> 16;
     j = w & 0xffffu;
   }
-  meta[0] = tiles;
-}
-__global__ __launch_bounds__(256) void plan_cut_write_kernel(const uint8_t *__restrict__ quad, uint64_t n_quads, uint64_t n_rows, int ncol,
-                                                             uint64_t n_chunks, uint32_t chunk, const uint64_t *__restrict__ entry,
-                                                             const uint64_t *__restrict__ base, pln_tile *__restrict__ tiles) {
+  out[id] = j | (tiles << 16);
+}
+template <typename T>
+__global__ __launch_bounds__(256) void plan_cut_descend_kernel(const T *__restrict__ fine, uint64_t n_fine, uint64_t fan,
+                                                               const uint64_t *__restrict__ coarse, uint64_t n_coarse,
+                                                               uint64_t *__restrict__ ent, unsigned long long *__restrict__ meta) {
+  const uint64_t g = (uint64_t)blockIdx.x * 256 + threadIdx.x;
+  if (g >= n_coarse) return;
+  uint64_t j = coarse ? coarse[2 * g] : 0, t = coarse ? coarse[2 * g + 1] : 0;
+  const uint64_t k_end = (g + 1) * fan < n_fine ? (g + 1) * fan : n_fine;
+  for (uint64_t k = g * fan; k < k_end; ++k) {
+    ent[2 * k] = j;
+    ent[2 * k + 1] = t;
+    const uint64_t w = fine[k * PLN_CUT_SPAN + j];
+    t += w >> 16;
+    j = w & 0xffffu;
+  }
+  if (!coarse) meta[0] = t;
+}
+__global__ __launch_bounds__(256) void plan_cut_starts_kernel(const uint16_t *__restrict__ step, uint64_t n_quads, uint64_t n_chunks,
+                                                              const uint64_t *__restrict__ ent, pln_tile *__restrict__ tiles) {
   const uint64_t k = (uint64_t)blockIdx.x * 256 + threadIdx.x;
   if (k >= n_chunks) return;
-  const uint64_t end = (k + 1) * chunk;
-  uint64_t q = entry[k], t = base[k];
+  const uint64_t end = (k + 1) * PLN_CUT_CHUNK;
+  uint64_t q = k * PLN_CUT_CHUNK + ent[2 * k], t = ent[2 * k + 1];
   while (q < end && q < n_quads) {
-    uint32_t items, hcol, hrow;
-    const uint64_t q1 = plan_cut_one(quad, n_quads, q, &items, &hcol, &hrow);
-    pln_tile ti;
-    ti.row0 = q * PLN_QUAD;
-    uint32_t rows = (uint32_t)(q1 - q) * PLN_QUAD;
-    if (ti.row0 + rows > n_rows) rows = (uint32_t)(n_rows - ti.row0);
-    const uint32_t hc = hcol < PLN_HCAP ? hcol : PLN_HCAP;
-    const uint32_t hr = ncol == 5 ? (hrow < PLN_HCAP ? hrow : PLN_HCAP) : 0u;
-    ti.rows_items = (rows << 16) | items;
-    ti.off16 = 0;
-    ti.hc_hr = (hc << 16) | hr;
-    ti.blk16 = pln_block_layout(rows, items, hc, hr).end / 16;
-    ti.pad = 0;
-    tiles[t++] = ti;
-    q = q1;
-  }
-}
-__global__ __launch_bounds__(1024) void plan_cut_offsets_kernel(pln_tile *__restrict__ tiles, uint64_t n_tiles,
+    tiles[t++].row0 = q * PLN_QUAD;
+    q += step[q];
+  }
+}
+__global__ __launch_bounds__(256) void plan_cut_desc_kernel(const uint8_t *__restrict__ quad, const uint16_t *__restrict__ step,
+                                                            uint64_t n_quads, uint64_t n_rows, int ncol,
+                                                            const unsigned long long *__restrict__ meta, pln_tile *__restrict__ tiles) {
+  const uint64_t t = (uint64_t)blockIdx.x * 4 + (threadIdx.x >> 6);
+  const uint32_t lane = threadIdx.x & 63u;
+  if (t >= meta[0]) return;
+  const uint64_t row0 = tiles[t].row0, q = row0 / PLN_QUAD;
+  const uint32_t len = step[q];
+  uint32_t items = 0, hcol = 0, hrow = 0;
+  for (uint32_t i = lane; i < len; i += 64) {
+    items += quad[q + i];
+    hcol += quad[n_quads + q + i];
+    hrow += quad[2 * n_quads + q + i];
+  }
+#pragma unroll
+  for (int off = 32; off > 0; off >>= 1) {
+    items += (uint32_t)__shfl_xor((int)items, off, 64);
+    hcol += (uint32_t)__shfl_xor((int)hcol, off, 64);
+    hrow += (uint32_t)__shfl_xor((int)hrow, off, 64);
+  }
+  if (lane != 0) return;
+  pln_tile ti;
+  ti.row0 = row0;
+  uint32_t rows = len * PLN_QUAD;
+  if (row0 + rows > n_rows) rows = (uint32_t)(n_rows - row0);
+  const uint32_t hc = hcol < PLN_HCAP ? hcol : PLN_HCAP;
+  const uint32_t hr = ncol == 5 ? (hrow < PLN_HCAP ? hrow : PLN_HCAP) : 0u;
+  ti.rows_items = (rows << 16) | items;
+  ti.off16 = 0;
+  ti.hc_hr = (hc << 16) | hr;
+  ti.blk16 = pln_block_layout(rows, items, hc, hr).end / 16;
+  ti.pad = 0;
+  tiles[t] = ti;
+}
+__global__ __launch_bounds__(1024) void plan_cut_offsets_kernel(pln_tile *__restrict__ tiles, const unsigned long long *__restrict__ hist,
                                                                 unsigned long long *__restrict__ meta) {
-  __shared__ unsigned long long part[1024];
-  const uint64_t per = (n_tiles + 1023) / 1024, lo = per * threadIdx.x, hi = lo + per < n_tiles ? lo + per : n_tiles;
-  unsigned long long s = 0;
-  for (uint64_t t = lo; t < hi; ++t) s += tiles[t].blk16;
-  part[threadIdx.x] = s;
-  __syncthreads();
-  if (threadIdx.x == 0) {
-    unsigned long long run = 0;
-    for (int k = 0; k < 1024; ++k) {
-      const unsigned long long v = part[k];
-      part[k] = run;
-      run += v;
-    }
+  constexpr uint32_t PER = 8;
+  __shared__ uint32_t part[16];
+  const uint32_t tid = threadIdx.x;
+  const uint64_t n_tiles = meta[0];
+  unsigned long long run = 0;
+  for (uint64_t base = 0; base < n_tiles; base += 1024 * PER) {
+    const uint64_t t0 = base + (uint64_t)tid * PER;
+    uint32_t v[PER], sum = 0;
+#pragma unroll
+    for (uint32_t k = 0; k < PER; ++k) {
+      v[k] = t0 + k < n_tiles ? tiles[t0 + k].blk16 : 0u;
+      sum += v[k];
+    }
+    uint32_t total;
+    unsigned long long off = run + plan_block_scan<16>(sum, part, &total);
+#pragma unroll
+    for (uint32_t k = 0; k < PER; ++k) {
+      if (t0 + k < n_tiles) tiles[t0 + k].off16 = (uint32_t)off;
+      off += v[k];
+    }
+    run += total;
+    __syncthreads();
+  }
+  if (tid == 0) {
     meta[1] = run;
     meta[2] = run > 0xffffffffull ? 1ull : 0ull;
   }
-  __syncthreads();
-  unsigned long long off = part[threadIdx.x];
-  for (uint64_t t = lo; t < hi; ++t) {
-    tiles[t].off16 = (uint32_t)off;
-    off += tiles[t].blk16;
-  }
-}
-
-__global__ __launch_bounds__(1024) void plan_fill_kernel(const uint32_t *__restrict__ counts, uint64_t n_rows, int ncol,
-                                                         const pln_tile *__restrict__ tiles, uint64_t n_tiles,
-                                                         unsigned char *__restrict__ stream,
-                                                         pln_heavy_col *__restrict__ heavy_col,
-                                                         pln_heavy_row *__restrict__ heavy_row,
-                                                         uint64_t *__restrict__ heavy_stop,
-                                                         unsigned long long *__restrict__ cursors) {
-  constexpr int RPT = (PLN_RMAX + 1023) / 1024;
+  if (tid < SRT_NKEY) meta[3 + tid] = hist[tid];
+}
+
+#define PLN_FILL_THREADS 256
+#define PLN_FILL_BLOCKS_PER_CU 3
+#define PLN_FILL_RPT ((PLN_RMAX + PLN_FILL_THREADS - 1) / PLN_FILL_THREADS)
+#define PLN_FILL_VEC ((PLN_RMAX * 5 / 4 + PLN_FILL_THREADS - 1) / PLN_FILL_THREADS)
+static_assert(PLN_RMAX % 4 == 0 && PLN_BLOCK_MAX % 16 == 0 && (PLN_LIVE_STRIDE * 2) % 16 == 0, "whole 16-byte pieces");
+static_assert(SRT_NHIST == PLN_FILL_THREADS && SRT_CL < 256 && PLN_NI <= (1 << 16), "one histogram bin per thread; count | rank << 8 in a word");
+
+typedef uint32_t plan_u32x4 __attribute__((ext_vector_type(4)));
+struct plan_fill_rows {
+  plan_u32x4 v[PLN_FILL_VEC];
+};
+__device__ __forceinline__ plan_fill_rows plan_fill_fetch(const uint32_t *__restrict__ counts, uint64_t row0, uint32_t rows) {
+  const plan_u32x4 *src = reinterpret_cast<const plan_u32x4 *>(counts + row0 * 5);
+  const uint32_t n_vec = rows * 5u / 4u;
+  plan_fill_rows pre;
+#pragma unroll
+  for (int k = 0; k < PLN_FILL_VEC; ++k) {
+    const uint32_t i = threadIdx.x + PLN_FILL_THREADS * k;
+    pre.v[k] = src[i < n_vec ? i : 0u];
+  }
+  return pre;
+}
+
+__global__ __launch_bounds__(PLN_FILL_THREADS) void plan_fill_kernel(const uint32_t *__restrict__ counts, uint64_t n_rows, int ncol,
+                                                                     const pln_tile *__restrict__ tiles, uint64_t n_tiles,
+                                                                     unsigned char *__restrict__ stream,
+                                                                     pln_heavy_col *__restrict__ heavy_col,
+                                                                     pln_heavy_row *__restrict__ heavy_row,
+                                                                     uint64_t *__restrict__ heavy_stop,
+                                                                     unsigned long long *__restrict__ cursors,
+                                                                     uint16_t *__restrict__ live) {
+  constexpr int RPT = PLN_FILL_RPT;
+  __shared__ __attribute__((aligned(16))) uint32_t s_cnt[PLN_RMAX * 5];
+  __shared__ __attribute__((aligned(16))) unsigned char s_blk[PLN_BLOCK_MAX];
+  __shared__ __attribute__((aligned(16))) uint16_t s_live[PLN_LIVE_STRIDE];
   __shared__ uint32_t hist[SRT_NHIST];
   __shared__ uint32_t offs[SRT_NHIST];
-  __shared__ uint32_t scan[16];
-  __shared__ uint16_t sorted[PLN_NI + 64];
+  __shared__ uint32_t part[4];
   __shared__ uint32_t s_hc, s_hr;
 #ifdef BEAR_DET_BUILD
   __shared__ uint32_t comp[PLN_NI];
-  static_assert((PLN_NI & (PLN_NI - 1)) == 0 && PLN_NI <= 2048, "bitonic sort over the tile's items: PLN_NI / 2 pairs, at most one per thread");
+  static_assert((PLN_NI & (PLN_NI - 1)) == 0, "bitonic sort over the tile's items");
+  static_assert(PLN_HCAP <= PLN_FILL_THREADS, "the in-tile lists are ranked one entry per thread");
   __shared__ unsigned long long hkey[PLN_HCAP], htmp[PLN_HCAP];
+  __shared__ uint32_t part_det[4];
 #endif
   const uint32_t tid = threadIdx.x, rep = tid & (SRT_REP - 1);
+  pln_tile ti, ti_next;
+  plan_fill_rows pre;
+  memset(&ti_next, 0, sizeof(ti_next));
+  if (blockIdx.x >= n_tiles) return;
+  ti = tiles[blockIdx.x];
+  pre = plan_fill_fetch(counts, ti.row0, ti.rows_items >> 16);
+  if ((uint64_t)blockIdx.x + gridDim.x < n_tiles) ti_next = tiles[(uint64_t)blockIdx.x + gridDim.x];
   for (uint64_t t = blockIdx.x; t < n_tiles; t += gridDim.x) {
-    const pln_tile ti = tiles[t];
     const uint32_t rows = ti.rows_items >> 16, n_light = ti.rows_items & 0xffffu;
     const uint32_t hc_cap = ti.hc_hr >> 16, hr_cap = ti.hc_hr & 0xffffu;
+    const uint64_t row0 = ti.row0;
+    const uint32_t off16 = ti.off16;
     const pln_layout L = pln_block_layout(rows, n_light, hc_cap, hr_cap);
-    unsigned char *blk = stream + (size_t)ti.off16 * 16;
-    uint16_t *E = reinterpret_cast<uint16_t *>(blk);
-    uint8_t *nrow = blk + L.nrow;
-    uint16_t *items = reinterpret_cast<uint16_t *>(blk + L.items);
-    uint16_t *hoff = reinterpret_cast<uint16_t *>(blk + L.hoff);
-    uint32_t *hcnt = reinterpret_cast<uint32_t *>(blk + L.hcnt);
-    uint16_t *hrow = reinterpret_cast<uint16_t *>(blk + L.hrow);
-    double *hn = reinterpret_cast<double *>(blk + L.hn);
-    if (tid < SRT_NHIST) hist[tid] = 0;
+    uint16_t *E = reinterpret_cast<uint16_t *>(s_blk);
+    uint8_t *nrow = s_blk + L.nrow;
+    uint16_t *items = reinterpret_cast<uint16_t *>(s_blk + L.items);
+    uint16_t *hoff = reinterpret_cast<uint16_t *>(s_blk + L.hoff);
+    uint32_t *hcnt = reinterpret_cast<uint32_t *>(s_blk + L.hcnt);
+    uint16_t *hrow = reinterpret_cast<uint16_t *>(s_blk + L.hrow);
+    double *hn = reinterpret_cast<double *>(s_blk + L.hn);
+    {
+      const uint32_t n_vec = rows * 5u / 4u, n_word = rows * 5u;
+      plan_u32x4 *dst = reinterpret_cast<plan_u32x4 *>(s_cnt);
+#pragma unroll
+      for (int k = 0; k < PLN_FILL_VEC; ++k) {
+        const uint32_t i = tid + PLN_FILL_THREADS * k;
+        if (i < n_vec) dst[i] = pre.v[k];
+      }
+      if (n_vec * 4u + tid < n_word) s_cnt[n_vec * 4u + tid] = counts[row0 * 5 + n_vec * 4u + tid];
+    }
+    hist[tid] = 0;
+    for (uint32_t i = L.hoff / 16 + tid; i < L.end / 16; i += PLN_FILL_THREADS) reinterpret_cast<uint4 *>(s_blk)[i] = make_uint4(0, 0, 0, 0);
     if (tid == 0) {
       s_hc = 0;
       s_hr = 0;
     }
-    __syncthreads();
+    ti = ti_next;
+    pre = plan_fill_fetch(counts, ti.row0, ti.rows_items >> 16);
+    if (t + 2 * (uint64_t)gridDim.x < n_tiles) ti_next = tiles[t + 2 * (uint64_t)gridDim.x];
+    srt_sync();
+    const uint32_t lr0 = tid * RPT;
 #ifdef BEAR_DET_BUILD
-    uint32_t det_hc[RPT], det_hr[RPT];
+    uint32_t det_hc, det_hr;
     {
-      uint32_t base_c = 0, base_r = 0;
-#pragma unroll
+      uint32_t nc = 0, nr = 0;
       for (int k = 0; k < RPT; ++k) {
-        const uint32_t lr = tid + 1024u * k;
-        uint32_t nc = 0, nr = 0;
+        const uint32_t lr = lr0 + k;
         if (lr < rows) {
           double n = 0.0;
           for (int b = 0; b < 5; ++b) {
-            const uint32_t cv = counts[(ti.row0 + lr) * 5 + b];
+            const uint32_t cv = s_cnt[lr * 5 + b];
             n += (double)cv;
             nc += (b < ncol && cv > SRT_CL) ? 1u : 0u;
           }
-          nr = n > (double)SRT_CL ? 1u : 0u;
+          nr += n > (double)SRT_CL ? 1u : 0u;
         }
-        const uint32_t packed = nc | (nr << 16);
-        const int lane = tid & 63, wave = tid >> 6;
-        uint32_t incl = packed;
-#pragma unroll
-        for (int off = 1; off < 64; off <<= 1) {
-          const uint32_t o = (uint32_t)__shfl_up((int)incl, off, 64);
-          if (lane >= off) incl += o;
+      }
+      uint32_t total;
+      const uint32_t excl = plan_block_scan<4>(nc | (nr << 16), part_det, &total);
+      det_hc = excl & 0xffffu;
+      det_hr = excl >> 16;
+      if (tid == 0) {
+        s_hc = total & 0xffffu;
+        s_hr = total >> 16;
+      }
+    }
+    static_assert(PLN_RMAX * 5 < 65536, "packed scan of the large-count cells and rows");
+#endif
+    uint32_t n_live = 0;
+    for (int k = 0; k < RPT; ++k) {
+      const uint32_t lr = lr0 + k;
+      if (lr < rows) {
+        const uint64_t r = row0 + lr;
+        uint32_t c[5];
+        double n = 0.0;
+#pragma unroll
+        for (int b = 0; b < 5; ++b) {
+          c[b] = s_cnt[lr * 5 + b];
+          n += (double)c[b];
         }
-        __syncthreads();
-        if (lane == 63) scan[wave] = incl;
-        __syncthreads();
-        uint32_t before = 0, total = 0;
-        for (int w = 0; w < 16; ++w) {
-          if (w < wave) before += scan[w];
-          total += scan[w];
-        }
-        const uint32_t excl = before + incl - packed;
-        det_hc[k] = base_c + (excl & 0xffffu);
-        det_hr[k] = base_r + (excl >> 16);
-        base_c += total & 0xffffu;
-        base_r += total >> 16;
-      }
-      __syncthreads();
-      if (tid == 0) {
-        s_hc = base_c;
-        s_hr = base_r;
-      }
-    }
-#endif
-    uint32_t c[RPT][5], rank[RPT][5];
-#pragma unroll
-    for (int k = 0; k < RPT; ++k) {
-      const uint32_t lr = tid + 1024u * k;
-#pragma unroll
-      for (int b = 0; b < 5; ++b) {
-        c[k][b] = 0;
-        rank[k][b] = 0;
-      }
-      if (lr < rows) {
-        const uint64_t r = ti.row0 + lr;
-        double n = 0.0;
-#pragma unroll
-        for (int b = 0; b < 5; ++b) {
-          c[k][b] = counts[r * 5 + b];
-          n += (double)c[k][b];
-        }
-        nrow[lr] = n < 1.0 ? (uint8_t)0 : (n <= (double)SRT_CL ? (uint8_t)n : (uint8_t)255);
+        const uint8_t nb = n < 1.0 ? (uint8_t)0 : (n <= (double)SRT_CL ? (uint8_t)n : (uint8_t)255);
+        nrow[lr] = nb;
+        n_live += nb != 0 ? 1u : 0u;
         if (n > (double)SRT_CL) {
 #ifdef BEAR_DET_BUILD
-          const uint32_t k2 = hr_cap ? det_hr[k] : 0xffffffffu;
+          const uint32_t k2 = hr_cap ? det_hr++ : 0xffffffffu;
 #else
           const uint32_t k2 = hr_cap ? atomicAdd(&s_hr, 1u) : 0xffffffffu;
 #endif
@@ -306,70 +408,75 @@
             heavy_row[q].n = n;
           }
         }
-        if (ncol == 4 && c[k][4] > SRT_CL) heavy_stop[atomicAdd(&cursors[2], 1ull)] = c[k][4];
+        if (ncol == 4 && c[4] > SRT_CL) heavy_stop[atomicAdd(&cursors[2], 1ull)] = c[4];
 #pragma unroll
         for (int b = 0; b < 5; ++b) {
-          if (b >= ncol) c[k][b] = 0;
-          if (c[k][b] > SRT_CL) {
+          uint32_t cb = b < ncol ? c[b] : 0u, word = 0;
+          if (cb > SRT_CL) {
 #ifdef BEAR_DET_BUILD
-            const uint32_t k2 = hc_cap ? det_hc[k]++ : 0xffffffffu;
+            const uint32_t k2 = hc_cap ? det_hc++ : 0xffffffffu;
 #else
             const uint32_t k2 = hc_cap ? atomicAdd(&s_hc, 1u) : 0xffffffffu;
 #endif
             if (k2 < hc_cap) {
               hoff[k2] = (uint16_t)(lr * 5 + b);
-              hcnt[k2] = c[k][b];
+              hcnt[k2] = cb;
             } else {
               const unsigned long long q = atomicAdd(&cursors[0], 1ull);
               heavy_col[q].off = r * 5 + b;
-              heavy_col[q].c = c[k][b];
+              heavy_col[q].c = cb;
             }
-            c[k][b] = 0;
+            cb = 0;
           }
-          if (c[k][b] != 0) rank[k][b] = atomicAdd(&hist[(c[k][b] - 1) * SRT_REP + rep], 1u);
+          if (cb != 0) word = cb | (atomicAdd(&hist[(cb - 1) * SRT_REP + rep], 1u) << 8);
+          s_cnt[lr * 5 + b] = word;
         }
       } else if (lr < ((rows + 15u) & ~15u)) {
         nrow[lr] = 0;
       }
     }
-    __syncthreads();
-    {
-      const uint32_t v = tid < SRT_NHIST ? hist[tid] : 0u;
-      const int lane = tid & 63, wave = tid >> 6;
-      uint32_t incl = v;
-#pragma unroll
-      for (int off = 1; off < 64; off <<= 1) {
-        uint32_t o = (uint32_t)__shfl_up((int)incl, off, 64);
-        if (lane >= off) incl += o;
-      }
-      if (lane == 63) scan[wave] = incl;
-      __syncthreads();
-      uint32_t base = 0;
-      for (int w = 0; w < wave; ++w) base += scan[w];
-      if (tid < SRT_NHIST) offs[tid] = base + incl - v;
-    }
-    __syncthreads();
+    srt_sync();
+    uint32_t total;
+    const uint32_t excl = plan_block_scan<4>(hist[tid] | (n_live << 16), part, &total);
+    offs[tid] = excl & 0xffffu;
+    srt_sync();
     if (tid < 30) E[tid] = (uint16_t)(tid < SRT_CL ? offs[tid * SRT_REP] : n_light);
     if (tid == 30) E[30] = (uint16_t)hc_cap;
     if (tid == 31) E[31] = (uint16_t)hr_cap;
-#pragma unroll
-    for (int k = 0; k < RPT; ++k)
-#pragma unroll
-      for (int b = 0; b < 5; ++b)
-        if (c[k][b] != 0) sorted[offs[(c[k][b] - 1) * SRT_REP + rep] + rank[k][b]] = (uint16_t)((tid + 1024u * k) * 5 + b);
-    __syncthreads();
+    for (int k = 0; k < RPT; ++k) {
+      const uint32_t lr = lr0 + k;
+      if (lr >= rows) break;
+#pragma unroll
+      for (int b = 0; b < 5; ++b) {
+        const uint32_t word = s_cnt[lr * 5 + b];
+        if (word) items[offs[((word & 0xffu) - 1) * SRT_REP + rep] + (word >> 8)] = (uint16_t)(lr * 5 + b);
+      }
+    }
+    const uint32_t padded = (n_light + 63u) & ~63u;
+    if (n_light + tid < padded) items[n_light + tid] = (uint16_t)PLN_SENTINEL;
+    if (live) {
+      const uint32_t all_live = total >> 16;
+      uint32_t at = 1 + (excl >> 16);
+      if (tid == 0) s_live[0] = (uint16_t)all_live;
+      for (int k = 0; k < RPT; ++k) {
+        const uint32_t lr = lr0 + k;
+        if (lr < rows && nrow[lr] != 0) s_live[at++] = (uint16_t)lr;
+      }
+      for (uint32_t i = 1 + all_live + tid; i < PLN_LIVE_STRIDE; i += PLN_FILL_THREADS) s_live[i] = 0;
+    }
+    srt_sync();
 #ifdef BEAR_DET_BUILD
     {
-      for (uint32_t i = tid; i < PLN_NI; i += 1024) {
+      for (uint32_t i = tid; i < PLN_NI; i += PLN_FILL_THREADS) {
         uint32_t key = 0;
         for (uint32_t q = 1; q < SRT_CL; ++q) key += offs[q * SRT_REP] <= i ? 1u : 0u;
-        comp[i] = i < n_light ? (key << 16) | sorted[i] : 0xffffffffu;
-      }
-      __syncthreads();
+        comp[i] = i < n_light ? (key << 16) | items[i] : 0xffffffffu;
+      }
+      srt_sync();
       for (uint32_t size = 2; size <= PLN_NI; size <<= 1)
         for (uint32_t stride = size >> 1; stride > 0; stride >>= 1) {
-          const uint32_t lo = 2u * tid - (tid & (stride - 1u)), hi = lo + stride;
-          if (tid < PLN_NI / 2) {
+          for (uint32_t pr = tid; pr < PLN_NI / 2; pr += PLN_FILL_THREADS) {
+            const uint32_t lo = 2u * pr - (pr & (stride - 1u)), hi = lo + stride;
             const bool up = (lo & size) == 0u;
             const uint32_t a = comp[lo], bq = comp[hi];
             if ((a > bq) == up) {
@@ -377,27 +484,26 @@
               comp[hi] = a;
             }
           }
-          __syncthreads();
+          srt_sync();
         }
-      for (uint32_t i = tid; i < n_light; i += 1024) sorted[i] = (uint16_t)(comp[i] & 0xffffu);
-      __syncthreads();
+      for (uint32_t i = tid; i < n_light; i += PLN_FILL_THREADS) items[i] = (uint16_t)(comp[i] & 0xffffu);
       const uint32_t nhc = s_hc < hc_cap ? s_hc : hc_cap, nhr = s_hr < hr_cap ? s_hr : hr_cap;
       if (tid < nhc) hkey[tid] = ((unsigned long long)hoff[tid] << 32) | hcnt[tid];
-      __syncthreads();
+      srt_sync();
       if (tid < nhc) {
         uint32_t r = 0;
         for (uint32_t q = 0; q < nhc; ++q) r += hkey[q] < hkey[tid] ? 1u : 0u;
         htmp[r] = hkey[tid];
       }
-      __syncthreads();
+      srt_sync();
       if (tid < nhc) {
         hoff[tid] = (uint16_t)(htmp[tid] >> 32);
         hcnt[tid] = (uint32_t)htmp[tid];
       }
-      __syncthreads();
+      srt_sync();
       if (tid < nhr) hkey[tid] = ((unsigned long long)hrow[tid] << 48) | tid;
       if (tid < nhr) htmp[tid] = (unsigned long long)__double_as_longlong(hn[tid]);
-      __syncthreads();
+      srt_sync();
       uint32_t r = 0;
       unsigned long long mine = 0ull, myn = 0ull;
       if (tid < nhr) {
@@ -405,51 +511,25 @@
         mine = hkey[tid];
         myn = htmp[tid];
       }
-      __syncthreads();
+      srt_sync();
       if (tid < nhr) {
         hrow[r] = (uint16_t)(mine >> 48);
         hn[r] = __longlong_as_double((long long)myn);
       }
-      __syncthreads();
+      srt_sync();
     }
 #endif
-    const uint32_t padded = (n_light + 63u) & ~63u;
-    for (uint32_t i = tid; i < padded; i += 1024) items[i] = i < n_light ? sorted[i] : (uint16_t)PLN_SENTINEL;
-    __syncthreads();
-  }
-}
-
-__global__ __launch_bounds__(1024) void plan_live_kernel(const pln_tile *__restrict__ tiles, uint64_t n_tiles,
-                                                         const unsigned char *__restrict__ stream, uint16_t *__restrict__ live) {
-  constexpr int RPT = (PLN_RMAX + 1023) / 1024;
-  __shared__ uint32_t cnt[RPT * 16];
-  const uint32_t tid = threadIdx.x, lane = tid & 63, wave = tid >> 6;
-  for (uint64_t t = blockIdx.x; t < n_tiles; t += gridDim.x) {
-    const pln_tile ti = tiles[t];
-    const uint32_t rows = ti.rows_items >> 16;
-    const uint8_t *nrow = stream + (size_t)ti.off16 * 16 + 64;
-    uint16_t *out = live + t * PLN_LIVE_STRIDE;
-    unsigned long long mask[RPT];
-#pragma unroll
-    for (int k = 0; k < RPT; ++k) {
-      const uint32_t lr = tid + 1024u * k;
-      mask[k] = __builtin_amdgcn_ballot_w64(lr < rows && nrow[lr] != 0);
-      if (lane == 0) cnt[k * 16 + wave] = (uint32_t)__builtin_popcountll(mask[k]);
-    }
-    __syncthreads();
-    uint32_t total = 0;
-#pragma unroll
-    for (int k = 0; k < RPT; ++k) {
-      uint32_t base = total;
-      for (int w = 0; w < 16; ++w) {
-        const uint32_t c = cnt[k * 16 + w];
-        if (w < (int)wave) base += c;
-        total += c;
-      }
-      if ((mask[k] >> lane) & 1ull) out[1 + base + (uint32_t)__builtin_popcountll(mask[k] & ((1ull << lane) - 1ull))] = (uint16_t)(tid + 1024u * k);
-    }
-    if (tid == 0) out[0] = (uint16_t)total;
-    __syncthreads();
+    {
+      uint4 *out = reinterpret_cast<uint4 *>(stream + (size_t)off16 * 16);
+      const uint4 *src = reinterpret_cast<const uint4 *>(s_blk);
+      for (uint32_t i = tid; i < L.end / 16; i += PLN_FILL_THREADS) out[i] = src[i];
+      if (live) {
+        uint4 *lout = reinterpret_cast<uint4 *>(live + t * PLN_LIVE_STRIDE);
+        const uint4 *lsrc = reinterpret_cast<const uint4 *>(s_live);
+        for (uint32_t i = tid; i < PLN_LIVE_STRIDE * 2 / 16; i += PLN_FILL_THREADS) lout[i] = lsrc[i];
+      }
+    }
+    srt_sync();
   }
 }
 
```

Result: no change. 142.0 billion, median of 4 (+0.2%).
